# krea-ai/realtime-video

Hardware: AMD Instinct MI355X
Metric: frames/sec at 832x480, 4-step 14B T2V (per-step DiT latency in config) (higher is better)
Workload: dtype bf16

## Files before the change

### include/rtv_hip_cross_fold.h

```cpp
#ifndef RTV_HIP_CROSS_FOLD_H
#define RTV_HIP_CROSS_FOLD_H
#include "rtv_hip.h"

#ifdef __cplusplus
extern "C" {
#endif

int rtv_attn_probs_dup(const void* q, const void* k, void* p, int Lq, int Lkv, int H, int D,
                       int64_t q_row_stride, int64_t k_row_stride, int64_t p_row_stride, int kh, int p_cols,
                       float scale, int dup_key, int dup_count, rtv_stream_t stream);

#define RTV_CROSS_FOLD_KH_MAX 120
int rtv_cross_fold_dims(int num_heads, int text_rows, int* kh, int* k_fold);
int rtv_cross_fold_weight(const void* co_w, int64_t ldw, const void* v, int64_t ldv, void* vo, int64_t ldvo,
                          int num_heads, int rows, int kh, int k_fold, rtv_stream_t stream);

#ifdef __cplusplus
}
#endif
#endif
```

### realtime_video_amd/causal_model.py

```python
import collections
import ctypes
import math
import os
import types

import torch

from . import _lib, lora, ops
from .rope import rope_cos_sin_table

c_vp = ctypes.c_void_p
_IncompatibleKeys = collections.namedtuple("_IncompatibleKeys", ["missing_keys", "unexpected_keys"])


_Cfg = _lib.STRUCTS["rtv_dit_config"]
_LayerW = _lib.STRUCTS["rtv_dit_layer_weights"]
_Weights = _lib.STRUCTS["rtv_dit_weights"]
_Step = _lib.STRUCTS["rtv_dit_step"]
_Fp8Shadow = _lib.ATTN_FP8_STRUCTS["rtv_attn_fp8_shadow"]
_LAYER_FIELDS = tuple(n for n, _ in _LayerW._fields_)
_TOP_FIELDS = tuple(n for n, t in _Weights._fields_ if t is c_vp)

_FP8_TOP = ("text0_w", "text2_w", "time0_w", "time2_w", "tproj_w", "head_w")
_FP8_LAYER = ("qkv_w", "o_w", "cq_w", "ck_w", "cv_w", "co_w", "ffn0_w", "ffn2_w")

PROJ_LN, PROJ_Q, PROJ_KV = 1, 2, 4


def _cross_fold_max_cols(num_heads):
    lib, kh, kf = _lib.load(), ctypes.c_int(0), ctypes.c_int(0)
    rows = 1
    while lib.rtv_cross_fold_dims(int(num_heads), rows + 8, ctypes.byref(kh), ctypes.byref(kf)):
        rows += 8
    lib.rtv_cross_fold_dims(int(num_heads), rows, ctypes.byref(kh), ctypes.byref(kf))
    return kf.value


class BlockCausalMask:

    def __init__(self, num_frames, frame_seqlen, num_frame_per_block, local_attn_size=-1):
        if local_attn_size != -1:
            raise NotImplementedError("local-window block masks are not used by the inference path")
        self.num_frames, self.frame_seqlen = num_frames, frame_seqlen
        self.num_frame_per_block = num_frame_per_block
        self.block_tokens = frame_seqlen * num_frame_per_block

    def __repr__(self):
        return f"BlockCausalMask(frames={self.num_frames}, block_tokens={self.block_tokens})"


class _SelfAttnHandle:

    def __init__(self, local_attn_size, sink_size):
        self.local_attn_size = local_attn_size
        self.sink_size = sink_size
        self.num_frame_per_block = 1
        self.fused_projections = True
        self.max_attention_size = 32760 if local_attn_size == -1 else local_attn_size * 1560

    def fuse_projections(self):
        self.fused_projections = True


def cache_row_map(cache, sink_tokens=None):
    n = int(cache["local_end_index"])
    r = torch.arange(n)
    lo, size, start = (int(cache.get(k, 0)) for k in ("ring_lo", "ring_size", "ring_start"))
    if size > 0:
        r = torch.where(r >= lo, lo + (r - lo + start) % size, r)
    return r


class CausalWanModel:
    def __init__(self, model_type="t2v", patch_size=(1, 2, 2), text_len=512, in_dim=16, dim=2048, ffn_dim=8192,
                 freq_dim=256, text_dim=4096, out_dim=16, num_heads=16, num_layers=32, local_attn_size=-1,
                 sink_size=0, qk_norm=True, cross_attn_norm=True, eps=1e-6, device="cuda"):
        if model_type != "t2v" or tuple(patch_size) != (1, 2, 2) or not qk_norm or not cross_attn_norm:
            raise NotImplementedError("the MI355X hot path implements the t2v causal model (patch 1x2x2, qk_norm, cross_attn_norm)")
        if dim % num_heads or dim // num_heads != 128:
            raise ValueError("head_dim must be 128")
        self.model_type, self.patch_size = model_type, tuple(patch_size)
        self.text_len, self.in_dim, self.dim, self.ffn_dim = text_len, in_dim, dim, ffn_dim
        self.freq_dim, self.text_dim, self.out_dim = freq_dim, text_dim, out_dim
        self.num_heads, self.num_layers, self.eps = num_heads, num_layers, eps
        self.local_attn_size, self.sink_size = local_attn_size, sink_size
        self.device = torch.device(device)
        self.config = types.SimpleNamespace(num_heads=num_heads, dim=dim, num_layers=num_layers, ffn_dim=ffn_dim)
        self.blocks = [types.SimpleNamespace(self_attn=_SelfAttnHandle(local_attn_size, sink_size))
                       for _ in range(num_layers)]
        self.block_mask = None
        self.num_frame_per_block = 1
        self.independent_first_frame = False
        self.gemm_tile_cfg = 0
        self.context_parallel = None
        self._tensors = {}
        self._w = None
        self._ws = {}
        self.fold_text_padding = True
        self.fold_cross_v = os.environ.get("RTV_FOLD_CROSS_V", "1") != "0"
        self.use_hip_graphs = False
        self._graphs = {}
        self._weights_version = 0
        self._cfg = _Cfg(dim, ffn_dim, num_heads, num_layers, freq_dim, text_dim, text_len, in_dim, out_dim, eps, 0, 0)
        self._lora = {}
        self._lora_base = {}
        self._fp8_attn = None
        self._fp8_attn_epoch = 0
        self._fp8_attn_amax = None
        self.lora_version = 0

    def eval(self):
        return self

    def to(self, *args, **kwargs):
        for a in list(args) + list(kwargs.values()):
            if isinstance(a, torch.dtype) and a != torch.bfloat16:
                raise NotImplementedError(f"the MI355X DiT computes in bf16 (asked for {a})")
            if isinstance(a, (str, torch.device, int)) and not isinstance(a, bool):
                dev = torch.device("cuda", a) if isinstance(a, int) else torch.device(a)
                if dev.type != self.device.type or (dev.index is not None and self.device.index is not None
                                                    and dev.index != self.device.index):
                    raise NotImplementedError(f"weights live on {self.device}; construct the model with device={dev!s} instead")
        return self

    def requires_grad_(self, flag=False):
        return self

    def parameters(self):
        return iter(self._tensors.values())

    def state_dict_shapes(self, fused=False):
        d, f = self.dim, self.ffn_dim
        sh = {"patch_embedding.weight": (d, self.in_dim) + self.patch_size, "patch_embedding.bias": (d,),
              "text_embedding.0.weight": (d, self.text_dim), "text_embedding.0.bias": (d,),
              "text_embedding.2.weight": (d, d), "text_embedding.2.bias": (d,),
              "time_embedding.0.weight": (d, self.freq_dim), "time_embedding.0.bias": (d,),
              "time_embedding.2.weight": (d, d), "time_embedding.2.bias": (d,),
              "time_projection.1.weight": (6 * d, d), "time_projection.1.bias": (6 * d,),
              "head.head.weight": (self.out_dim * 4, d), "head.head.bias": (self.out_dim * 4,), "head.modulation": (1, 2, d)}
        for i in range(self.num_layers):
            p = f"blocks.{i}"
            for a in ("self_attn", "cross_attn"):
                for m in ("q", "k", "v", "o"):
                    sh[f"{p}.{a}.{m}.weight"], sh[f"{p}.{a}.{m}.bias"] = (d, d), (d,)
                sh[f"{p}.{a}.norm_q.weight"], sh[f"{p}.{a}.norm_k.weight"] = (d,), (d,)
            if fused:
                sh[f"{p}.self_attn.to_qkv.weight"], sh[f"{p}.self_attn.to_qkv.bias"] = (3 * d, d), (3 * d,)
            sh[f"{p}.norm3.weight"], sh[f"{p}.norm3.bias"] = (d,), (d,)
            sh[f"{p}.ffn.0.weight"], sh[f"{p}.ffn.0.bias"] = (f, d), (f,)
            sh[f"{p}.ffn.2.weight"], sh[f"{p}.ffn.2.bias"] = (d, f), (d,)
            sh[f"{p}.modulation"] = (1, 6, d)
        return sh

    def load_state_dict(self, sd, strict=True, assign=False):
        dev, bf = self.device, torch.bfloat16
        sd = {(k[len("model."):] if k.startswith("model.") else k): v for k, v in sd.items()}
        want = self.state_dict_shapes(fused=True)
        problems, missing, unexpected = [], [], sorted(k for k in sd if k not in want)
        fused_layers = set()
        for i in range(self.num_layers):
            sa = f"blocks.{i}.self_attn"
            if sa + ".to_qkv.weight" in sd and sa + ".to_qkv.bias" in sd:
                fused_layers.add(i)
        for k, shp in want.items():
            layer_fused = ".self_attn." in k and int(k.split(".")[1]) in fused_layers
            is_qkv = ".self_attn." in k and k.split(".")[3] in ("q", "k", "v")
            is_fused_key = ".to_qkv." in k
            if k not in sd:
                if (is_fused_key and not layer_fused) or (is_qkv and layer_fused):
                    continue
                missing.append(k)
            elif tuple(sd[k].shape) != tuple(shp):
                problems.append(f"size mismatch for {k}: copying a param with shape {tuple(sd[k].shape)} from checkpoint, "
                                f"the shape in current model is {tuple(shp)}.")
        if missing:
            problems.insert(0, "Missing key(s) in state_dict: " + ", ".join(repr(k) for k in missing[:12])
                            + (f" ... ({len(missing)} in total)" if len(missing) > 12 else "") + ".")
        if unexpected and strict:
            problems.insert(1 if missing else 0, "Unexpected key(s) in state_dict: " + ", ".join(repr(k) for k in unexpected[:12])
                            + (f" ... ({len(unexpected)} in total)" if len(unexpected) > 12 else "") + ".")
        if problems and (strict or missing or any(p.startswith("size") for p in problems)):
            raise RuntimeError("Error(s) in loading state_dict for CausalWanModel:\n\t" + "\n\t".join(problems))
# ... 340 lines not shown
            rolled = l_end - evicted - sink_tokens
            if ring and rolled <= 0:
                ring_start = 0
            elif ring:
                if ring_size == 0 or ring_start == 0:
                    ring_lo, ring_size = sink_tokens, kv_size - sink_tokens
                elif (ring_lo, ring_size) != (sink_tokens, kv_size - sink_tokens):
                    raise RuntimeError("the attention sink changed under a rotated rolling cache")
                ring_start = (ring_start + evicted) % ring_size
            else:
                shift_copy = (sink_tokens, evicted, rolled)
            local_end = l_end + current_end - g_end - evicted
        else:
            local_end = l_end + current_end - g_end
        if not ring and ring_start:
            raise RuntimeError("this KV cache is rotated (ring_start != 0): reset it before using it under context parallelism")
        local_start = local_end - num_new
        if local_start < 0 or local_end > kv_size:
            raise RuntimeError(f"KV cache window [{local_start}, {local_end}) outside cache of {kv_size} rows")
        lo = max(0, local_end - sa.max_attention_size)
        if ring_start == 0:
            ring_lo = ring_size = 0

        def commit():
            if shift_copy is not None:
                s0, ev, ro = shift_copy
                for c in kv_cache:
                    for n in ("k", "v"):
                        c[n][:, s0:s0 + ro] = c[n][:, s0 + ev:s0 + ev + ro].clone()
            for c in kv_cache:
                c["global_end_index"] = current_end
                c["local_end_index"] = local_end
                c["ring_lo"], c["ring_size"], c["ring_start"] = ring_lo, ring_size, ring_start
        return local_start, lo, local_end, current_start // frame_seqlen, 0, (ring_lo, ring_size, ring_start), commit

    def _forward_inference(self, x, t, context, seq_len=None, clip_fea=None, y=None, kv_cache=None,
                           crossattn_cache=None, current_start=0, cache_start=0, kv_cache_only=False):
        if self._w is None:
            raise RuntimeError("weights not loaded")
        if kv_cache is None or crossattn_cache is None:
            raise NotImplementedError("the hot path is the KV-cached inference forward (causal_model.py:825-954)")
        if clip_fea is not None or y is not None:
            raise NotImplementedError("i2v conditioning is out of scope")
        xs = list(x) if not torch.is_tensor(x) else [x[i] for i in range(x.shape[0])]
        B = len(xs)
        if B != 1:
            raise NotImplementedError("batch size 1 (the streaming server path); run sessions as replicas")
        u = xs[0]
        if not u.is_cuda:
            raise RuntimeError("realtime_video_amd.CausalWanModel needs GPU tensors (no CPU fallback)")
        C, F, Hh, Ww = u.shape
        gh, gw = Hh // 2, Ww // 2
        fs = gh * gw
        M = F * fs
        if seq_len is not None and M > seq_len:
            raise AssertionError("sequence longer than seq_len")
        u = u.to(torch.bfloat16).contiguous()
        tt = t.reshape(-1).to(device=u.device, dtype=torch.float32).contiguous()
        if tt.numel() != F:
            raise ValueError("t must hold one timestep per latent frame")
        need_cross = not all(bool(c["is_init"]) and int(c.get("lora_version", 0)) == self.lora_version for c in crossattn_cache)
        ctx = None
        if need_cross:
            cu = context[0] if not torch.is_tensor(context) else context[0]
            ctx = torch.zeros(self.text_len, self.text_dim, dtype=torch.bfloat16, device=u.device)
            ctx[:cu.shape[0]] = cu.to(torch.bfloat16)
            nz = torch.nonzero(ctx.abs().amax(dim=1) > 0)
            n_real = int(nz[-1]) + 1 if nz.numel() else 0
            for c in crossattn_cache:
                c["text_rows"] = n_real
        cp = self.context_parallel
        use_cp = cp is not None and (cp.world > 1 or getattr(cp, "force_single_rank", False))
        kv_only = bool(kv_cache_only) and not need_cross
        text_rows = int(crossattn_cache[0].get("text_rows", 0)) if getattr(self, "fold_text_padding", True) else 0
        if text_rows <= 0 or any(int(c.get("text_rows", 0)) != text_rows for c in crossattn_cache):
            text_rows = 0
        fold_k = 0
        if 0 < text_rows < self.text_len - 1 and getattr(self, "fold_cross_v", True) and not self._cfg.use_fp8:
            kh_, kf_ = ctypes.c_int(0), ctypes.c_int(0)
            if _lib.load().rtv_cross_fold_dims(self.num_heads, text_rows, ctypes.byref(kh_), ctypes.byref(kf_)):
                fold_k = kf_.value
            if fold_k and not need_cross and any(c.get("vo_for") != (text_rows, self.lora_version) for c in crossattn_cache):
                fold_k = 0
        if fold_k:
            for c in crossattn_cache:
                if "vo" not in c:
                    c["vo"] = torch.zeros(self.dim * _cross_fold_max_cols(self.num_heads), dtype=torch.bfloat16, device=u.device)
        row0, lo, hi, start_frame, causal_block, (ring_lo, ring_size, ring_shift), commit = \
            self._cache_window(kv_cache, M, current_start, fs, ring=not use_cp)
        L = self.num_layers
        rs = kv_cache[0]["k"].stride(1)
        for c in kv_cache:
            for n in ("k", "v"):
                if c[n].stride(3) != 1 or c[n].stride(2) != c[n].shape[3] or c[n].stride(1) != rs:
                    raise ValueError("KV cache tensors must be [B, kv_size, H, 128] views with dense [H, 128] rows "
                                     "and one common row stride")

        fp8_shadow, fp8_keep = self._fp8_attention_shadow(kv_cache, use_cp)
        forward = ("rtv_dit_forward",) if fp8_shadow is None else ("rtv_dit_forward_attn_fp8", ctypes.byref(fp8_shadow))
        fp8_key = (self._fp8_attn[:2] + (kv_cache[0]["k8"].data_ptr(), kv_cache[-1]["v8t"].data_ptr())) if fp8_shadow is not None else None

        def ptr_array(tensors):
            arr = (c_vp * L)(*[t_.data_ptr() for t_ in tensors])
            return arr, ctypes.cast(arr, ctypes.POINTER(c_vp))

        kk_keep, kk = ptr_array([c["k"] for c in kv_cache])
        kv_keep, kv = ptr_array([c["v"] for c in kv_cache])
        ck_keep, ck = ptr_array([c["k"] for c in crossattn_cache])
        cv_list = [c["v"] for c in crossattn_cache] + ([c["vo"] for c in crossattn_cache] if fold_k else [])
        cv_keep = (c_vp * len(cv_list))(*[t_.data_ptr() for t_ in cv_list])
        cv = ctypes.cast(cv_keep, ctypes.POINTER(c_vp))
        out = (torch.zeros if kv_only else torch.empty)((self.out_dim, F, Hh, Ww), dtype=torch.bfloat16, device=u.device)
        stream = c_vp(torch.cuda.current_stream().cuda_stream)
        cfg_p, w_p = ctypes.byref(self._cfg), ctypes.byref(self._w)

        def make(rank_rows, slot, kk=kk, kv=kv):
            ws = self._workspace(F, gh, gw, slot)
            ws_ptr = (ws.data_ptr() + 255) & ~255
            st = _Step(u.data_ptr(), tt.data_ptr(), ctx.data_ptr() if ctx is not None else None, out.data_ptr(),
                       F, gh, gw, kk, kv, rs, ck, cv, int(need_cross), row0, lo, hi,
                       start_frame, causal_block, int(self.gemm_tile_cfg), rank_rows[0], rank_rows[1],
                       ring_lo, ring_size, ring_shift, int(text_rows), int(kv_only),
                       int(getattr(cp, "attn_kv_splits", 1)) if use_cp else 1, fold_k)
            return st, (c_vp(ws_ptr), ctypes.c_size_t(ws.numel() - (ws_ptr - ws.data_ptr())), stream)

        splits = int(getattr(cp, "attn_kv_splits", 1)) if use_cp else 1
        if splits > self._cfg.max_attn_kv_splits:
            self._cfg.max_attn_kv_splits = splits
            self._ws.clear()
            self._graphs.clear()
            self._weights_version += 1
        if self.gemm_tile_cfg in (0, 5):
            ops.ensure_gemm_workspace(u.device)
        if use_cp:
            commit()
        if not use_cp:
            graph_key = None
            if self.use_hip_graphs and not need_cross:
                graph_key = (F, gh, gw, row0, lo, hi, start_frame, causal_block, ring_lo, ring_size, ring_shift, kv_only, text_rows, fold_k,
                             int(self.gemm_tile_cfg), rs, self._weights_version,
                             kv_cache[0]["k"].data_ptr(), kv_cache[-1]["v"].data_ptr(), crossattn_cache[0]["k"].data_ptr(), fp8_key)
                ent = self._graphs.get(graph_key)
                if isinstance(ent, dict):
                    ent["u"].copy_(u)
                    ent["t"].copy_(tt)
                    ent["graph"].replay()
                    commit()
                    return ent["out"].clone().unsqueeze(0)
            if graph_key is not None and self._graphs.get(graph_key) == "seen":
                ent = {"u": u.clone(), "t": tt.clone(), "out": out, "keep": (kk_keep, kv_keep, ck_keep, cv_keep, fp8_keep)}
                u, tt = ent["u"], ent["t"]
                g = torch.cuda.CUDAGraph()
                if not hasattr(self, "_capture_stream"):
                    self._capture_stream = torch.cuda.Stream(device=u.device)
                ops.ensure_gemm_workspace(u.device, self._capture_stream.cuda_stream)
                with torch.cuda.graph(g, stream=self._capture_stream):
                    stream = c_vp(torch.cuda.current_stream().cuda_stream)
                    st, wsa = make((0, 0), 0)
                    _lib.call(forward[0], cfg_p, w_p, ctypes.byref(st), *forward[1:], *wsa)
                ent["graph"], ent["step"] = g, st
                self._graphs[graph_key] = ent
                g.replay()
                commit()
                return out.clone().unsqueeze(0)
            if graph_key is not None:
                self._graphs[graph_key] = "seen"
            st, wsa = make((0, 0), 0)
            _lib.call(forward[0], cfg_p, w_p, ctypes.byref(st), *forward[1:], *wsa)
            commit()
        else:
            graph_key = None
            if self.use_hip_graphs and not need_cross and not getattr(cp, "_gloo", False):
                graph_key = ("cp", id(cp), bool(getattr(cp, "overlap", True)), cp.world, cp.head_exchange(self.num_heads), F, gh, gw, row0, lo, hi, start_frame, causal_block, kv_only,
                             text_rows, fold_k, int(self.gemm_tile_cfg), rs, self._weights_version, splits,
                             kv_cache[0]["k"].data_ptr(), kv_cache[-1]["v"].data_ptr(), crossattn_cache[0]["k"].data_ptr())
                ent = self._graphs.get(graph_key)
                if isinstance(ent, dict):
                    ent["u"].copy_(u)
                    ent["t"].copy_(tt)
                    ent["graph"].replay()
                    return ent["out"].clone().unsqueeze(0)

            def run_cp():
                self.cp_forwards_issued = getattr(self, "cp_forwards_issued", 0) + 1
                from .parallel import shard_rows, wait_in_order
                W, H = cp.world, self.num_heads
                heads = cp.head_exchange(H)
                keep = []
                if heads:
                    hn = H // W
                    if kv_cache[0]["k"].shape[2] not in (hn, H):
                        raise ValueError(f"KV cache must hold {hn} (this rank's) or {H} heads, not {kv_cache[0]['k'].shape[2]}")
                    parts = []
                    for i, r in enumerate(cp.local_ranks()):
                        h0 = 0 if kv_cache[0]["k"].shape[2] == hn else r * hn
                        ka, kp = ptr_array([c["k"][0, :, h0:h0 + hn] for c in kv_cache])
                        va, vp = ptr_array([c["v"][0, :, h0:h0 + hn] for c in kv_cache])
                        keep.append((ka, va))
                        parts.append(make(shard_rows(M, W, r), i, kp, vp))
                    bufs = [(r, self._exchange_buffers(M, W, i, u.device)) for i, r in enumerate(cp.local_ranks())]
                else:
                    parts = [make(shard_rows(M, W, r), i) for i, r in enumerate(cp.local_ranks())]
                for st, wsa in parts:
                    _lib.call("rtv_dit_begin", cfg_p, w_p, ctypes.byref(st), *wsa)
                null = c_vp(0)
                for l in range(L):
                    last_kv_only = kv_only and l == L - 1
                    if not heads:
                        for st, wsa in parts:
                            _lib.call("rtv_dit_layer_proj", cfg_p, w_p, ctypes.byref(st), l, PROJ_LN | PROJ_KV, 0, null, null, *wsa)
                        pend = cp.gather_kv(kv_cache[l]["k"][0], kv_cache[l]["v"][0], row0, M, async_op=True)
                        if last_kv_only:
                            pend.wait()
                            break
                        for st, wsa in parts:
                            _lib.call("rtv_dit_layer_proj", cfg_p, w_p, ctypes.byref(st), l, PROJ_Q, 0, null, null, *wsa)
                        pend.wait()
                        for st, wsa in parts:
                            _lib.call("rtv_dit_layer_rest", cfg_p, w_p, ctypes.byref(st), l, *wsa)
                        continue
                    if last_kv_only:
                        for (st, wsa), (_, b) in zip(parts, bufs):
                            _lib.call("rtv_dit_layer_proj", cfg_p, w_p, ctypes.byref(st), l, PROJ_LN | PROJ_KV, W, null,
                                      c_vp(b["kv_send"].data_ptr()), *wsa)
                        cp.exchange_kv(bufs, kv_cache[l]["k"][0], kv_cache[l]["v"][0], row0, M)
                        break
                    for (st, wsa), (_, b) in zip(parts, bufs):
                        _lib.call("rtv_dit_layer_proj", cfg_p, w_p, ctypes.byref(st), l, PROJ_LN | PROJ_Q, W,
                                  c_vp(b["q_send"].data_ptr()), null, *wsa)
                    pend_q = cp.exchange_q(bufs, async_op=True)
                    for (st, wsa), (_, b) in zip(parts, bufs):
                        _lib.call("rtv_dit_layer_proj", cfg_p, w_p, ctypes.byref(st), l, PROJ_KV, W, null,
                                  c_vp(b["kv_send"].data_ptr()), *wsa)
                    pend_kv = cp.exchange_kv(bufs, kv_cache[l]["k"][0], kv_cache[l]["v"][0], row0, M, async_op=True)
                    wait_in_order(pend_q, pend_kv)
                    for (st, wsa), (_, b) in zip(parts, bufs):
                        _lib.call("rtv_dit_layer_attn_hp", cfg_p, w_p, ctypes.byref(st), l, W, c_vp(b["q_all"].data_ptr()),
                                  c_vp(b["o_all"].data_ptr()), *wsa)
                    cp.exchange_o(bufs)
                    for (st, wsa), (_, b) in zip(parts, bufs):
                        _lib.call("rtv_dit_layer_rest_hp", cfg_p, w_p, ctypes.byref(st), l, W, c_vp(b["o_recv"].data_ptr()), *wsa)
                if not kv_only:
                    hrow = torch.empty((M, self.out_dim * 4), dtype=torch.bfloat16, device=u.device)
                    for st, wsa in parts:
                        _lib.call("rtv_dit_head", cfg_p, w_p, ctypes.byref(st), c_vp(hrow.data_ptr()), *wsa)
                    cp.all_gather_rows_(hrow, kind="head_rows")
                    _lib.call("rtv_dit_finish", cfg_p, ctypes.byref(parts[0][0]), c_vp(hrow.data_ptr()), stream)

            if graph_key is not None and self._graphs.get(graph_key) == "seen":
                ent = {"u": u.clone(), "t": tt.clone(), "out": out, "keep": (kk_keep, kv_keep, ck_keep, cv_keep)}
                u, tt = ent["u"], ent["t"]
                g = torch.cuda.CUDAGraph()
                if not hasattr(self, "_capture_stream"):
                    self._capture_stream = torch.cuda.Stream(device=u.device)
                ops.ensure_gemm_workspace(u.device, self._capture_stream.cuda_stream)
                with torch.cuda.graph(g, stream=self._capture_stream, capture_error_mode="thread_local"):
                    stream = c_vp(torch.cuda.current_stream().cuda_stream)
# ... 20 lines not shown
```

### realtime_video_amd/csrc/attn_fwd.hip

```cpp
#include "attn_common.h"

namespace rtv {

#ifdef RTV_ATTN_TRACE
__device__ unsigned* g_attn_trace = nullptr;
#define ATT_STAMP(i)                                                                    \
  do {                                                                                  \
    if (tr_on && j >= 20 && j < 24) {                                                   \
      __builtin_amdgcn_sched_barrier(0);                                                \
      const unsigned t_ = (unsigned)__builtin_readcyclecounter();                       \
      if (lane == 0) tr_dst[(j - 20) * 6 + (i)] = t_;                                   \
      __builtin_amdgcn_sched_barrier(0);                                                \
    }                                                                                   \
  } while (0)
#else
#define ATT_STAMP(i)
#endif

template <bool F16>
__global__ __launch_bounds__(256) void attn_combine_kernel(const float* __restrict__ part_o, const float* __restrict__ part_ml,
                                                           uint16_t* __restrict__ o, int S, int B, int H, int Lq, int64_t o_bs,
                                                           int64_t o_rs) {
  const int64_t nrows = (int64_t)B * H * Lq;
  const int64_t row = (int64_t)blockIdx.x * 16 + (threadIdx.x >> 4);
// ... 510 lines not shown
          int kv = j * ATT_KT + kbk * 32 + (r & 3) + 8 * (r >> 2) + 4 * g;
          if (kv >= kv_lim) sacc[kbk][r] = -INFINITY;
        }
    }
    {
      float mx = sacc[0][0];
#pragma unroll
      for (int r = 1; r < 16; ++r) mx = fmaxf(mx, sacc[0][r]);
#pragma unroll
      for (int r = 0; r < 16; ++r) mx = fmaxf(mx, sacc[1][r]);
      mx = xor32_max(mx);
      const float m_cand = fmaxf(m_run, mx * c);
      const bool need = m_cand - m_run > RESCALE_SLACK;
      if (__builtin_amdgcn_ballot_w64(need) != 0) {
        const float m_new = need ? m_cand : m_run;
        const float alpha = __builtin_amdgcn_exp2f(m_run - m_new);
        m_run = m_new;
        l_run *= alpha;
#pragma unroll
        for (int db = 0; db < 4; ++db)
#pragma unroll
          for (int r = 0; r < 16; ++r) oacc[db][r] *= alpha;
      }
      static_for<0, 4>([&](auto ic) { exp_step(IntC<0>{}, ic); });
    }
    asm volatile("" : "+v"(pf[0][0]), "+v"(ps2));
    asm volatile("s_waitcnt vmcnt(4)" ::: "memory");
    ATT_STAMP8(5);
    PP_BARRIER();
    ATT_STAMP8(6);
    lds_wait_frags(frag);
    static_for<0, 16>([&](auto ic) {
      constexpr int i = decltype(ic)::value, kbk = i >> 3, s_ = (i >> 2) & 1, db = i & 3;
      oacc[db] = mfma32<F16>(frag[(kbk * 2 + s_) * 4 + db], pf[kbk][s_], oacc[db]);
      if constexpr (i < 12) {
        constexpr int f = i + 4;
        exp_step(IntC<(f >> 3)>{}, IntC<(f & 7)>{});
      }
      __builtin_amdgcn_sched_barrier(0);
    });
    l_run += ps2[0] + ps2[1];
    ps2 = f32x2{0.f, 0.f};
    asm volatile("" : "+v"(l_run));
    ATT_STAMP8(7);
    PP_BARRIER();
  }
  if (!grp) PP_BARRIER();
#undef PP_BARRIER

#ifdef RTV_ATTN_TRACE
  if (tr_on && lane < 32 && ntiles >= 24) tr_dst[lane] = tr_lds[lane];
#endif
  const float l_tot = l_run + __shfl_xor(l_run, 32, 64);
  if (p.kv_splits > 1) {
    store_partial(p, bh, q_row, g, oacc, m_run, l_tot);
    return;
  }
  const float inv = 1.0f / l_tot;
  if (q_row < p.Lq) {
    uint16_t* op = ob + (size_t)q_row * p.o_rs + 4 * g;
#pragma unroll
    for (int db = 0; db < 4; ++db)
#pragma unroll
      for (int i = 0; i < 4; ++i) {
        u32x2 w;
        w[0] = pack2<F16>(oacc[db][4 * i + 0] * inv, oacc[db][4 * i + 1] * inv);
        w[1] = pack2<F16>(oacc[db][4 * i + 2] * inv, oacc[db][4 * i + 3] * inv);
        *(u32x2*)(op + db * 32 + i * 8) = w;
      }
  }
}

struct ProbsParams {
  const uint16_t* q;
  const uint16_t* k;
  uint16_t* p;
  int Lq, Lkv, H;
  int64_t q_rs, k_rs, p_rs;
  int kh, p_cols;
  float scale_log2e;
  int dup_key;
  float dup_log2;
  int tiles_per_wg;
};
constexpr int PROBS_NW = 4;
constexpr int PROBS_ROWS = PROBS_NW * ATT_QW;

template <int NKB>
__global__ __launch_bounds__(PROBS_NW * 64) void attn_probs_kernel(ProbsParams p) {
  constexpr int KEYS = NKB * 32;
  constexpr int SLAB_LD = KEYS * 2 + 16;
  extern __shared__ __attribute__((aligned(16))) char smem[];
  char* const sK = smem;
  const int tid = threadIdx.x;
  const int lane = tid & 63;
  const int wave = __builtin_amdgcn_readfirstlane(tid >> 6);
  const int l31 = lane & 31, g = lane >> 5;
  char* const slab = smem + KEYS * 256 + wave * (ATT_QW * SLAB_LD);
  const int h = blockIdx.y;
  const uint16_t* qb = p.q + (size_t)h * ATT_D;
  const uint16_t* kb = p.k + (size_t)h * ATT_D;
  uint16_t* pb = p.p + (size_t)h * p.kh;

  for (int id = tid; id < KEYS * 16; id += PROBS_NW * 64) {
    const int r = id >> 4, c = id & 15;
    u32x4 v = {0u, 0u, 0u, 0u};
    if (r < p.Lkv) v = *(const u32x4*)(kb + (int64_t)r * p.k_rs + c * 8);
    *(u32x4*)(sK + r * 256 + ((c ^ (r & 15)) << 4)) = v;
  }
  __syncthreads();
  const char* k_rd[8];
#pragma unroll
  for (int dc = 0; dc < 8; ++dc) k_rd[dc] = sK + l31 * 256 + (((dc * 2 + g) ^ (l31 & 15)) << 4);

  const float c = p.scale_log2e;
  const int ppr = p.kh >> 3;
  const int tail0 = p.H * p.kh, tail_pieces = h == p.H - 1 ? (p.p_cols - tail0) >> 3 : 0;
  const int tile0 = blockIdx.x * p.tiles_per_wg;
  for (int ti = 0; ti < p.tiles_per_wg; ++ti) {
    const int row0 = (tile0 + ti) * PROBS_ROWS + wave * ATT_QW;
    if (row0 >= p.Lq) break;
    const int q_row_c = min(row0 + l31, p.Lq - 1);
    u32x4 qf[8];
    {
      const uint16_t* qp = qb + (size_t)q_row_c * p.q_rs + g * 8;
#pragma unroll
      for (int dc = 0; dc < 8; ++dc) qf[dc] = *(const u32x4*)(qp + dc * 16);
    }
    f32x16 s[NKB];
#pragma unroll
    for (int kbk = 0; kbk < NKB; ++kbk)
#pragma unroll
      for (int r = 0; r < 16; ++r) s[kbk][r] = 0.f;
#pragma unroll
    for (int dc = 0; dc < 8; ++dc)
#pragma unroll
      for (int kbk = 0; kbk < NKB; ++kbk) {
        const u32x4 kf = *(const u32x4*)(k_rd[dc] + kbk * 32 * 256);
        s[kbk] = mfma32<false>(kf, qf[dc], s[kbk]);
      }
    float mx = -INFINITY;
#pragma unroll
    for (int kbk = 0; kbk < NKB; ++kbk)
#pragma unroll
      for (int r = 0; r < 16; ++r) {
        const int key = kbk * 32 + (r & 3) + 8 * (r >> 2) + 4 * g;
        float x = s[kbk][r] * c;
        if (key == p.dup_key) x += p.dup_log2;
        if (key >= p.Lkv) x = -INFINITY;
        s[kbk][r] = x;
        mx = fmaxf(mx, x);
      }
    mx = fmaxf(mx, __shfl_xor(mx, 32, 64));
    float l = 0.f;
#pragma unroll
    for (int kbk = 0; kbk < NKB; ++kbk)
#pragma unroll
      for (int r = 0; r < 16; ++r) {
        const float e = __builtin_amdgcn_exp2f(s[kbk][r] - mx);
        s[kbk][r] = e;
        l += e;
      }
    l += __shfl_xor(l, 32, 64);
    const float inv = 1.0f / l;
#pragma unroll
    for (int kbk = 0; kbk < NKB; ++kbk)
#pragma unroll
      for (int i = 0; i < 4; ++i) {
        u32x2 w;
        w[0] = pack2<false>(s[kbk][4 * i + 0] * inv, s[kbk][4 * i + 1] * inv);
        w[1] = pack2<false>(s[kbk][4 * i + 2] * inv, s[kbk][4 * i + 3] * inv);
        *(u32x2*)(slab + l31 * SLAB_LD + (kbk * 32 + 8 * i + 4 * g) * 2) = w;
      }
    __builtin_amdgcn_fence(__ATOMIC_RELEASE, "workgroup");
    __builtin_amdgcn_wave_barrier();
    const int rows_here = min(ATT_QW, p.Lq - row0);
    for (int id = lane; id < rows_here * ppr; id += 64) {
      const int r = id / ppr, pc = id - r * ppr;
      const u32x4 v = *(const u32x4*)(slab + r * SLAB_LD + pc * 16);
      *(u32x4*)(pb + (int64_t)(row0 + r) * p.p_rs + pc * 8) = v;
    }
    for (int id = lane; id < rows_here * tail_pieces; id += 64) {
      const int r = id / tail_pieces, pc = id - r * tail_pieces;
      *(u32x4*)(p.p + (int64_t)(row0 + r) * p.p_rs + tail0 + pc * 8) = u32x4{0u, 0u, 0u, 0u};
    }
    __builtin_amdgcn_fence(__ATOMIC_ACQUIRE, "workgroup");
    __builtin_amdgcn_wave_barrier();
  }
}

}

using namespace rtv;

#ifdef RTV_ATTN_TRACE
extern "C" int rtv_attn_debug_trace(unsigned* buf) {
  return hipMemcpyToSymbol(HIP_SYMBOL(rtv::g_attn_trace), &buf, sizeof(buf)) == hipSuccess ? 0 : -1;
}
#endif

static std::atomic<int> g_attn_waves{0};
static std::atomic<bool> g_attn_lockstep{false};
static std::atomic<bool> g_attn_force_pp{false};
static std::atomic<bool> g_attn_skip_idle{true};
static std::atomic<int> g_attn_w4{-2};
constexpr int W4_DEFAULT = 600;
namespace rtv {
int launch_attn_w4(const AttnParams& p, bool f16, int variant, dim3 grid, hipStream_t stream);
}

extern "C" int rtv_attn_set_skip_idle(int on) {
  g_attn_skip_idle = on != 0;
  return 0;
}

extern "C" int rtv_attn_set_waves(int waves) {
  if (waves != 0 && waves != 4 && waves != 8 && waves != 81 && waves != 82 && !(waves >= 840 && waves <= 1639))
    return set_error(-1, "attn_set_waves: 0 (auto), 4, 8, 81 (256 rows, lockstep schedule), 82 (256 rows, four-phase schedule) or "
                         "840 + v (256 rows, one wave per SIMD, kernel variant v: attn_w4.hip)");
  g_attn_lockstep = waves == 81;
  g_attn_force_pp = waves == 82;
  g_attn_w4 = waves >= 840 ? waves - 840 : (waves == 81 || waves == 82 ? -1 : -2);
  g_attn_waves = waves > 8 ? 8 : waves;
  return 0;
}

extern "C" int rtv_attn_fwd(const void* q, const void* k, const void* v, void* o, int B, int Lq, int Lkv,
                            int H, int D, int64_t q_batch_stride, int64_t q_row_stride,
                            int64_t k_batch_stride, int64_t k_row_stride, int64_t v_batch_stride,
                            int64_t v_row_stride, int64_t o_batch_stride, int64_t o_row_stride, float scale,
                            int causal_block, int q_offset, int dtype, rtv_stream_t stream) {
  return rtv_attn_fwd_win(q, k, v, o, B, Lq, Lkv, 0, 0, H, D, q_batch_stride, q_row_stride, k_batch_stride, k_row_stride,
                          v_batch_stride, v_row_stride, o_batch_stride, o_row_stride, scale, causal_block, q_offset, dtype,
                          stream);
}

static int attn_fwd_impl(const void* q, const void* k, const void* v, void* o, int B, int Lq, int Lkv0, int Lkv1,
                         int seg1_row, int H, int D, int64_t q_batch_stride, int64_t q_row_stride,
                         int64_t k_batch_stride, int64_t k_row_stride, int64_t v_batch_stride,
                         int64_t v_row_stride, int64_t o_batch_stride, int64_t o_row_stride, float scale,
                         int causal_block, int q_offset, int dtype, rtv_stream_t stream, int dup_key, int dup_count,
                         int kv_splits = 1, void* split_ws = nullptr, size_t split_ws_bytes = 0);

extern "C" int rtv_attn_fwd_win(const void* q, const void* k, const void* v, void* o, int B, int Lq, int Lkv0, int Lkv1,
                                int seg1_row, int H, int D, int64_t q_batch_stride, int64_t q_row_stride,
                                int64_t k_batch_stride, int64_t k_row_stride, int64_t v_batch_stride,
                                int64_t v_row_stride, int64_t o_batch_stride, int64_t o_row_stride, float scale,
                                int causal_block, int q_offset, int dtype, rtv_stream_t stream) {
  return attn_fwd_impl(q, k, v, o, B, Lq, Lkv0, Lkv1, seg1_row, H, D, q_batch_stride, q_row_stride, k_batch_stride, k_row_stride,
                       v_batch_stride, v_row_stride, o_batch_stride, o_row_stride, scale, causal_block, q_offset, dtype, stream,
                       -1, 0);
}

extern "C" int rtv_attn_fwd_dup(const void* q, const void* k, const void* v, void* o, int B, int Lq, int Lkv, int H, int D,
                                int64_t q_batch_stride, int64_t q_row_stride, int64_t k_batch_stride, int64_t k_row_stride,
                                int64_t v_batch_stride, int64_t v_row_stride, int64_t o_batch_stride, int64_t o_row_stride,
                                float scale, int dup_key, int dup_count, int dtype, rtv_stream_t stream) {
  if (dup_key < 0 || dup_key >= Lkv || dup_count < 1) return set_error(-1, "attn_fwd_dup: dup_key must be a key of the window, dup_count >= 1");
  return attn_fwd_impl(q, k, v, o, B, Lq, Lkv, 0, 0, H, D, q_batch_stride, q_row_stride, k_batch_stride, k_row_stride,
                       v_batch_stride, v_row_stride, o_batch_stride, o_row_stride, scale, 0, 0, dtype, stream,
                       dup_count > 1 ? dup_key : -1, dup_count);
}

template <int NKB>
static int launch_attn_probs(const ProbsParams& p, dim3 grid, hipStream_t stream) {
  static LdsAttr lds_attr;
  const int lds = NKB * 32 * 256 + PROBS_NW * ATT_QW * (NKB * 64 + 16);
  if (int st = ensure_dynamic_lds((const void*)attn_probs_kernel<NKB>, lds, &lds_attr, "attn_probs")) return st;
  hipLaunchKernelGGL((attn_probs_kernel<NKB>), grid, dim3(PROBS_NW * 64), lds, stream, p);
  return check_launch("attn_probs");
}

extern "C" int rtv_attn_probs_dup(const void* q, const void* k, void* p, int Lq, int Lkv, int H, int D, int64_t q_row_stride,
                                  int64_t k_row_stride, int64_t p_row_stride, int kh, int p_cols, float scale, int dup_key,
                                  int dup_count, rtv_stream_t stream) {
  if (D != ATT_D) return set_error(-1, "attn_probs: head_dim must be 128");
  if (H <= 0 || Lq <= 0) return 0;
  if (Lkv <= 0 || Lkv > 128) return set_error(-1, "attn_probs: the key window must hold 1..128 keys");
  if (kh <= 0 || (kh & 7) || kh < Lkv || kh > 128) return set_error(-1, "attn_probs: kh must be a multiple of 8 in [Lkv, 128]");
  if ((p_cols & 7) || (int64_t)H * kh > p_cols || p_cols > p_row_stride)
    return set_error(-1, "attn_probs: need H * kh <= p_cols <= p_row_stride, p_cols a multiple of 8");
  if ((q_row_stride | k_row_stride | p_row_stride) & 7 || q_row_stride < (int64_t)H * ATT_D || k_row_stride < (int64_t)H * ATT_D)
    return set_error(-1, "attn_probs: strides must be multiples of 8 elements (16-byte rows) and hold H heads");
  if (((uintptr_t)q | (uintptr_t)k | (uintptr_t)p) & 15) return set_error(-1, "attn_probs: base pointers must be 16-byte aligned");
  if (dup_key < 0 || dup_key >= Lkv || dup_count < 1) return set_error(-1, "attn_probs: dup_key must be a key of the window, dup_count >= 1");
  ProbsParams pp;
  pp.q = (const uint16_t*)q;
  pp.k = (const uint16_t*)k;
  pp.p = (uint16_t*)p;
  pp.Lq = Lq;
  pp.Lkv = Lkv;
  pp.H = H;
  pp.q_rs = q_row_stride;
  pp.k_rs = k_row_stride;
  pp.p_rs = p_row_stride;
  pp.kh = kh;
  pp.p_cols = p_cols;
  pp.scale_log2e = scale * 1.4426950408889634f;
  pp.dup_key = dup_count > 1 ? dup_key : -1;
  pp.dup_log2 = dup_count > 1 ? log2f((float)dup_count) : 0.f;
  const int cus = device_num_cus() > 0 ? device_num_cus() : 256;
  const int n_tiles = (Lq + PROBS_ROWS - 1) / PROBS_ROWS;
  int tpw = (int)(((int64_t)n_tiles * H) / (2 * (int64_t)cus));
  tpw = tpw < 1 ? 1 : (tpw > 8 ? 8 : tpw);
  pp.tiles_per_wg = tpw;
  const dim3 grid((n_tiles + tpw - 1) / tpw, H);
  ProfScope prof(PROF_ATTN, (hipStream_t)stream, 2.0 * H * (double)Lq * Lkv * ATT_D);
  note_kernel(DK_ATTN_PROBS);
  const int nkb = (kh + 31) / 32;
  switch (nkb) {
    case 1: return launch_attn_probs<1>(pp, grid, (hipStream_t)stream);
    case 2: return launch_attn_probs<2>(pp, grid, (hipStream_t)stream);
    case 3: return launch_attn_probs<3>(pp, grid, (hipStream_t)stream);
    default: return launch_attn_probs<4>(pp, grid, (hipStream_t)stream);
  }
}

extern "C" size_t rtv_attn_split_workspace_bytes(int B, int Lq, int H, int kv_splits) {
  if (B <= 0 || Lq <= 0 || H <= 0 || kv_splits < 2) return 0;
  return (size_t)kv_splits * B * H * Lq * (ATT_D + 2) * sizeof(float);
}

extern "C" int rtv_attn_fwd_split(const void* q, const void* k, const void* v, void* o, int B, int Lq, int Lkv0, int Lkv1,
                                  int seg1_row, int H, int D, int64_t q_batch_stride, int64_t q_row_stride,
                                  int64_t k_batch_stride, int64_t k_row_stride, int64_t v_batch_stride,
                                  int64_t v_row_stride, int64_t o_batch_stride, int64_t o_row_stride, float scale,
                                  int causal_block, int q_offset, int kv_splits, void* workspace, size_t workspace_bytes,
                                  int dtype, rtv_stream_t stream) {
  if (kv_splits < 1 || kv_splits > 16) return set_error(-1, "attn_fwd_split: kv_splits must be 1..16");
  return attn_fwd_impl(q, k, v, o, B, Lq, Lkv0, Lkv1, seg1_row, H, D, q_batch_stride, q_row_stride, k_batch_stride, k_row_stride,
                       v_batch_stride, v_row_stride, o_batch_stride, o_row_stride, scale, causal_block, q_offset, dtype, stream, -1,
                       0, kv_splits, workspace, workspace_bytes);
}

static int attn_fwd_impl(const void* q, const void* k, const void* v, void* o, int B, int Lq, int Lkv0, int Lkv1,
                         int seg1_row, int H, int D, int64_t q_batch_stride, int64_t q_row_stride,
                         int64_t k_batch_stride, int64_t k_row_stride, int64_t v_batch_stride,
                         int64_t v_row_stride, int64_t o_batch_stride, int64_t o_row_stride, float scale,
                         int causal_block, int q_offset, int dtype, rtv_stream_t stream, int dup_key, int dup_count,
                         int kv_splits, void* split_ws, size_t split_ws_bytes) {
  if (Lkv0 < 0 || Lkv1 < 0) return set_error(-1, "attn_fwd: negative segment length");
  if (Lkv1 > 0 && causal_block > 0) return set_error(-1, "attn_fwd: the block-causal mask needs a one-segment window");
  const int Lkv = Lkv0 + Lkv1;
  if (D != ATT_D) return set_error(-1, "attn_fwd: head_dim must be 128");
  if (B <= 0 || H <= 0 || Lq <= 0) return 0;
  if (Lkv <= 0) return set_error(-1, "attn_fwd: Lkv must be positive");
  if ((q_row_stride | k_row_stride | v_row_stride | o_row_stride | q_batch_stride | k_batch_stride |
       v_batch_stride | o_batch_stride) & 7)
    return set_error(-1, "attn_fwd: strides must be multiples of 8 elements (16-byte rows)");
  if (((uintptr_t)q | (uintptr_t)k | (uintptr_t)v | (uintptr_t)o) & 15)
    return set_error(-1, "attn_fwd: base pointers must be 16-byte aligned");
  if (causal_block < 0 || q_offset < 0) return set_error(-1, "attn_fwd: negative mask parameters");
  if (dtype != RTV_DTYPE_BF16 && dtype != RTV_DTYPE_F16) return set_error(-1, "attn_fwd: dtype");
  AttnParams p;
  p.q = (const uint16_t*)q;
  p.k = (const uint16_t*)k;
  p.v = (const uint16_t*)v;
  p.o = (uint16_t*)o;
  p.B = B;
  p.Lq = Lq;
  p.Lkv = Lkv;
  p.H = H;
  p.q_bs = q_batch_stride;
  p.q_rs = q_row_stride;
  p.k_bs = k_batch_stride;
  p.k_rs = k_row_stride;
  p.v_bs = v_batch_stride;
  p.v_rs = v_row_stride;
  p.o_bs = o_batch_stride;
  p.o_rs = o_row_stride;
  p.scale_log2e = scale * 1.4426950408889634f;
  p.dup_key = dup_key;
  p.dup_bias = dup_key >= 0 ? log2f((float)dup_count) / p.scale_log2e : 0.f;
  if (kv_splits > (Lkv + ATT_KT - 1) / ATT_KT) kv_splits = (Lkv + ATT_KT - 1) / ATT_KT;
  if (kv_splits < 1) kv_splits = 1;
  p.kv_splits = kv_splits;
  p.part_o = nullptr;
  p.part_ml = nullptr;
  if (kv_splits > 1) {
    if (dup_key >= 0) return set_error(-1, "attn_fwd: no KV split of a window with a counted key");
    const size_t rows = (size_t)kv_splits * B * H * Lq;
    if (!split_ws || ((uintptr_t)split_ws & 15) || split_ws_bytes < rows * (ATT_D + 2) * sizeof(float))
      return set_error(-1, "attn_fwd: split workspace missing, misaligned or too small (rtv_attn_split_workspace_bytes)");
    p.part_o = (float*)split_ws;
    p.part_ml = p.part_o + rows * ATT_D;
  }
  p.causal_block = causal_block;
  p.q_offset = q_offset;
  p.n0 = Lkv1 > 0 ? Lkv0 : Lkv;
  p.delta = Lkv1 > 0 ? seg1_row - Lkv0 : 0;
  int waves = g_attn_waves;
  const int cus = device_num_cus() > 0 ? device_num_cus() : 256;
  if (waves == 0) waves = ((int64_t)B * H * ((Lq + 255) / 256) * kv_splits < (int64_t)cus * 5 / 8 || Lkv <= 512) ? 4 : 8;
  const int qt_rows = ATT_QW * waves;
  p.n_qtiles = (Lq + qt_rows - 1) / qt_rows;
  const int lds = 4 * ATT_TILE_BYTES;
  const bool f16 = dtype == RTV_DTYPE_F16;
  const void* kerns[4] = {(const void*)attn_fwd_kernel<false, 8>, (const void*)attn_fwd_kernel<true, 8>,
// ... 75 lines not shown
```

### realtime_video_amd/csrc/dit_forward.hip

```cpp
#include <atomic>

#include "../../include/rtv_hip_attn_fp8.h"
#include "rtv_common.h"
#include "rtv_internal.h"

namespace rtv {

__global__ void silu_kernel(const bf16_t* __restrict__ x, bf16_t* __restrict__ out, int64_t n) {
  for (int64_t i = (int64_t)blockIdx.x * blockDim.x + threadIdx.x; i < n; i += (int64_t)gridDim.x * blockDim.x)
    out[i] = f32_to_bf16(silu(bf16_to_f32(x[i])));
}

constexpr int FOLD_ROWS = 64, FOLD_LD = 130;
__global__ __launch_bounds__(256) void cross_fold_weight_kernel(const bf16_t* __restrict__ w, int64_t ldw, const bf16_t* __restrict__ v,
                                                               int64_t ldv, bf16_t* __restrict__ vo, int64_t ldvo, int H, int rows, int kh,
                                                               int k_fold) {
  __shared__ __attribute__((aligned(16))) bf16_t sW[FOLD_ROWS * FOLD_LD];
  __shared__ __attribute__((aligned(16))) bf16_t sV[128 * FOLD_LD];
  const int tid = threadIdx.x, lane = tid & 63, wave = tid >> 6;
  const int n0 = blockIdx.x * FOLD_ROWS, h = blockIdx.y;
  for (int id = tid; id < FOLD_ROWS * 64; id += 256) {
    const int r = id >> 6, c = (id & 63) * 2;
    *(uint32_t*)(sW + r * FOLD_LD + c) = *(const uint32_t*)(w + (int64_t)(n0 + r) * ldw + h * 128 + c);
  }
  for (int id = tid; id < rows * 64; id += 256) {
    const int r = id >> 6, c = (id & 63) * 2;
    *(uint32_t*)(sV + r * FOLD_LD + c) = *(const uint32_t*)(v + (int64_t)r * ldv + h * 128 + c);
  }
  __syncthreads();
  for (int ts = 0; ts < kh; ts += 64) {
    const int t = ts + lane;
    float acc[16];
#pragma unroll
    for (int i = 0; i < 16; ++i) acc[i] = 0.f;
    if (t < rows) {
      const bf16_t* vr = sV + t * FOLD_LD;
      const bf16_t* wr = sW + wave * 16 * FOLD_LD;
      for (int dd = 0; dd < 128; dd += 2) {
        const uint32_t v2 = *(const uint32_t*)(vr + dd);
        const float v0 = __uint_as_float(v2 << 16), v1 = __uint_as_float(v2 & 0xffff0000u);
#pragma unroll
        for (int i = 0; i < 16; ++i) {
          const uint32_t w2 = *(const uint32_t*)(wr + i * FOLD_LD + dd);
          acc[i] = fmaf(__uint_as_float(w2 << 16), v0, acc[i]);
          acc[i] = fmaf(__uint_as_float(w2 & 0xffff0000u), v1, acc[i]);
        }
      }
    }
    if (t < kh) {
#pragma unroll
      for (int i = 0; i < 16; ++i) vo[(int64_t)(n0 + wave * 16 + i) * ldvo + h * kh + t] = f32_to_bf16(acc[i]);
    }
  }
  if (h == H - 1) {
    const int tail0 = H * kh;
    for (int t = tail0 + lane; t < k_fold; t += 64)
#pragma unroll
      for (int i = 0; i < 16; ++i) vo[(int64_t)(n0 + wave * 16 + i) * ldvo + t] = 0;
  }
}

struct Workspace {
  char* base;
  size_t off, cap;
  bool ok;
  void* take(size_t bytes) {
    size_t a = (off + 255) & ~(size_t)255;
    if (base && a + bytes > cap) ok = false;
    off = a + bytes;
    return base ? base + a : nullptr;
  }
};

struct DitBuffers {
  uint16_t *x, *xn, *qkv, *q, *ao, *h, *prow, *hrow;
  uint16_t *sinus, *te1, *e, *se, *e0, *emod, *ehead, *ctx1, *ctx, *ktmp;
  uint8_t* q8;
  float* frow;
  float* fscale;
  float* attn_part;
  size_t attn_part_bytes;
};

static size_t carve(const rtv_dit_config* c, int F, int gh, int gw, char* base, size_t cap, DitBuffers* b,
                    bool* ok) {
  Workspace ws{base, 0, cap, true};
  const size_t M = (size_t)F * gh * gw, d = c->dim, e = 2;
  DitBuffers t;
  t.x = (uint16_t*)ws.take(M * d * e);
  t.xn = (uint16_t*)ws.take(M * d * e);
  t.qkv = (uint16_t*)ws.take(M * 3 * d * e);
  t.q = (uint16_t*)ws.take(M * d * e);
  t.ao = (uint16_t*)ws.take(M * d * e);
  t.h = (uint16_t*)ws.take(M * (size_t)c->ffn_dim * e);
  t.prow = (uint16_t*)ws.take(M * (size_t)c->in_dim * 4 * e);
  t.hrow = (uint16_t*)ws.take(M * (size_t)c->out_dim * 4 * e);
  t.sinus = (uint16_t*)ws.take((size_t)F * c->freq_dim * e);
  t.te1 = (uint16_t*)ws.take((size_t)F * d * e);
  t.e = (uint16_t*)ws.take((size_t)F * d * e);
  t.se = (uint16_t*)ws.take((size_t)F * d * e);
  t.e0 = (uint16_t*)ws.take((size_t)F * 6 * d * e);
  t.emod = (uint16_t*)ws.take((size_t)c->num_layers * F * 6 * d * e);
  t.ehead = (uint16_t*)ws.take((size_t)F * 2 * d * e);
  t.ctx1 = (uint16_t*)ws.take((size_t)c->text_len * d * e);
  t.ctx = (uint16_t*)ws.take((size_t)c->text_len * d * e);
  t.ktmp = (uint16_t*)ws.take((size_t)c->text_len * d * e);
  {
    size_t rows = M > (size_t)c->text_len ? M : (size_t)c->text_len, k = d;
    if ((size_t)c->ffn_dim > k) k = c->ffn_dim;
    if ((size_t)c->text_dim > k) k = c->text_dim;
    if ((size_t)c->freq_dim > k) k = c->freq_dim;
    t.q8 = (uint8_t*)ws.take(c->use_fp8 ? rows * k : 0);
    t.frow = (float*)ws.take(c->use_fp8 == 2 ? rows * sizeof(float) : 0);
    t.fscale = (float*)ws.take(256);
  }
  t.attn_part_bytes = c->max_attn_kv_splits > 1 ? M * (size_t)c->num_heads * (128 + 2) * sizeof(float) : 0;
  t.attn_part = (float*)ws.take(t.attn_part_bytes);
  if (b) *b = t;
  if (ok) *ok = ws.ok;
  return ws.off;
}

struct Ctx {
  const rtv_dit_config* cfg;
  const rtv_dit_weights* w;
  const rtv_dit_step* st;
  DitBuffers b;
  rtv_stream_t stream;
  int d, H, L, ffn, hd, F, gh, gw, fs, M, r0, rc, tc;
  const rtv_attn_fp8_shadow* fp8;
  int fold_kh, fold_k;
};

static int make_ctx(const rtv_dit_config* cfg, const rtv_dit_weights* w, const rtv_dit_step* st, void* workspace,
                    size_t workspace_bytes, rtv_stream_t stream, Ctx* c) {
  if (!cfg || !w || !st || !workspace) return set_error(-1, "dit: null argument");
  c->cfg = cfg;
  c->w = w;
  c->st = st;
  c->fp8 = nullptr;
  c->stream = stream;
  c->d = cfg->dim;
  c->H = cfg->num_heads;
  c->L = cfg->num_layers;
  c->ffn = cfg->ffn_dim;
  if (c->H <= 0 || c->d % c->H || c->d / c->H != 128) return set_error(-1, "dit: head_dim must be 128");
  c->hd = 128;
  c->F = st->F;
  c->gh = st->gh;
  c->gw = st->gw;
  c->fs = st->gh * st->gw;
  c->M = st->F * c->fs;
  if (c->M <= 0) return set_error(-1, "dit: empty token grid");
  c->r0 = st->row_begin;
  c->rc = st->row_count > 0 ? st->row_count : c->M - st->row_begin;
  if (c->r0 < 0 || c->rc <= 0 || c->r0 + c->rc > c->M) return set_error(-1, "dit: local row range outside the token grid");
  if (st->kv_lo < 0 || st->kv_hi <= st->kv_lo) return set_error(-1, "dit: empty attention window");
  if (st->cache_row0 < 0 || st->cache_row0 + c->M > st->kv_hi)
    return set_error(-1, "dit: the rows written by this call must lie inside the attention window");
  if (st->ring_size < 0 || st->ring_lo < 0 || st->ring_shift < 0 || (st->ring_size > 0 && st->ring_shift >= st->ring_size) ||
      (st->ring_size > 0 && st->kv_hi > st->ring_lo + st->ring_size))
    return set_error(-1, "dit: bad ring window (0 <= ring_shift < ring_size, kv_hi <= ring_lo + ring_size)");
  if (st->ring_size > 0 && st->ring_shift > 0 && st->causal_block > 0)
    return set_error(-1, "dit: the block-causal recompute pass writes an unrotated cache (ring_shift must be 0)");
  if (((uintptr_t)workspace) & 255) return set_error(-1, "dit: workspace must be 256-byte aligned");
  bool ok = true;
  carve(cfg, c->F, c->gh, c->gw, (char*)workspace, workspace_bytes, &c->b, &ok);
  if (!ok) return set_error(-1, "dit: workspace too small (see rtv_dit_workspace_bytes)");
  c->tc = st->gemm_tile_cfg;
  c->fold_kh = c->fold_k = 0;
  if (st->ca_vo_ld > 0 && st->ca_v && !cfg->use_fp8 && st->text_rows > 0 && st->text_rows + 1 < cfg->text_len) {
    int kh = 0, kf = 0;
    if (rtv_cross_fold_dims(c->H, st->text_rows, &kh, &kf) && kf <= c->d) {
      if (st->ca_vo_ld < kf || (st->ca_vo_ld & 7)) return set_error(-1, "dit: ca_vo_ld must be a multiple of 8 and >= k_fold (rtv_cross_fold_dims)");
      c->fold_kh = kh;
      c->fold_k = kf;
    }
  }
  return 0;
}

}

using namespace rtv;

#define RTV_TRY(expr)        \
  do {                       \
    int _s = (expr);         \
    if (_s != 0) return _s;  \
  } while (0)

extern "C" int rtv_silu(const void* x, void* out, int64_t n, rtv_stream_t stream) {
  if (n <= 0) return 0;
  int blocks = (int)((n + 255) / 256);
  if (blocks > 2048) blocks = 2048;
  hipLaunchKernelGGL(silu_kernel, dim3(blocks), dim3(256), 0, (hipStream_t)stream, (const bf16_t*)x,
                     (bf16_t*)out, n);
  return check_launch("silu");
}

extern "C" int rtv_cross_fold_dims(int num_heads, int text_rows, int* kh, int* k_fold) {
  const int khv = text_rows >= 0 ? (text_rows + 1 + 7) & ~7 : 0;
  const int64_t kf = ((int64_t)num_heads * khv + 63) & ~(int64_t)63;
  if (kh) *kh = khv;
  if (k_fold) *k_fold = kf > 0x7fffffff ? 0 : (int)kf;
  return num_heads > 0 && text_rows > 0 && khv <= RTV_CROSS_FOLD_KH_MAX && kf <= 0x7fffffff;
}

extern "C" int rtv_cross_fold_weight(const void* co_w, int64_t ldw, const void* v, int64_t ldv, void* vo, int64_t ldvo, int num_heads,
                                     int rows, int kh, int k_fold, rtv_stream_t stream) {
  if (!co_w || !v || !vo) return set_error(-1, "cross_fold_weight: null argument");
  if (num_heads <= 0 || rows <= 0 || rows > kh || kh > 128 || (kh & 7)) return set_error(-1, "cross_fold_weight: need 0 < rows <= kh <= 128, kh % 8 == 0");
  const int64_t d = (int64_t)num_heads * 128;
  if ((int64_t)num_heads * kh > k_fold || k_fold > ldvo || ldw < d || ldv < d || ((ldw | ldv) & 1))
    return set_error(-1, "cross_fold_weight: need num_heads * kh <= k_fold <= ldvo and rows of num_heads * 128 elements");
  if (((uintptr_t)co_w | (uintptr_t)v) & 3) return set_error(-1, "cross_fold_weight: operands must be 4-byte aligned");
  ProfScope prof(PROF_MISC, (hipStream_t)stream, 2.0 * d * (double)num_heads * rows * 128);
  hipLaunchKernelGGL(cross_fold_weight_kernel, dim3((unsigned)(d / FOLD_ROWS), num_heads), dim3(256), 0, (hipStream_t)stream,
                     (const bf16_t*)co_w, ldw, (const bf16_t*)v, ldv, (bf16_t*)vo, ldvo, num_heads, rows, kh, k_fold);
  return check_launch("cross_fold_weight");
}

extern "C" size_t rtv_dit_workspace_bytes(const rtv_dit_config* cfg, int F, int gh, int gw) {
  if (!cfg || F <= 0 || gh <= 0 || gw <= 0) return 0;
  return carve(cfg, F, gh, gw, nullptr, 0, nullptr, nullptr) + 256;
}

enum { S_TEXT0 = 0, S_TEXT2, S_TIME0, S_TIME2, S_TPROJ, S_HEAD, S_LAYER0 };
enum { S_QKV = 0, S_O, S_CQ, S_CK, S_CV, S_CO, S_FFN0, S_FFN2, S_PER_LAYER };
static bool is_fp8(const Ctx& c, int sidx) { return c.cfg->use_fp8 && sidx >= 0; }

static int quantize_input(Ctx& c, int sidx, const void* a, int M, int K, rtv_stream_t s) {
  if (!is_fp8(c, sidx)) return 0;
  if (c.cfg->use_fp8 == 2) {
    if (!c.w->fp8_row_scales || !c.w->fp8_row_scales[sidx]) return set_error(-1, "dit: use_fp8 == 2 needs rtv_dit_weights.fp8_row_scales");
    return a ? rtv_quantize_fp8_rows(a, K, M, K, c.b.q8, K, c.b.frow, s) : 0;
  }
  if (!c.w->fp8_scales) return set_error(-1, "dit: use_fp8 needs rtv_dit_weights.fp8_scales");
  return rtv_quantize_fp8(a, K, M, K, c.b.q8, K, c.b.fscale, c.b.fscale + 1, s) ? -1 : 0;
}

static int project(Ctx& c, int sidx, const void* a, int K, const void* w, int w_row0, const void* bias, void* out, int ldc, int M, int N,
                   int act, const void* gate, int gate_stride, int rpf, int row_off, const void* res, int cfg, rtv_stream_t s) {
  const bool fp8 = is_fp8(c, sidx);
  const void* wp = (const char*)w + (size_t)w_row0 * K * (fp8 ? 1 : 2);
  const void* bp = bias ? (const uint16_t*)bias + w_row0 : nullptr;
  const int ldr = res ? ldc : 0;
  if (!fp8) return rtv_gemm(a, K, wp, K, out, ldc, M, N, K, bp, act, gate, gate_stride, rpf, row_off, res, ldr, RTV_DTYPE_BF16, cfg, s);
  if (c.cfg->use_fp8 == 2)
    return rtv_gemm_fp8_rows(c.b.q8, K, wp, K, c.b.frow, (const float*)c.w->fp8_row_scales[sidx] + w_row0, out, ldc, M, N, K, bp, act, gate,
                             gate_stride, rpf, row_off, res, ldr, s);
  return rtv_gemm_fp8(c.b.q8, K, wp, K, c.b.fscale, c.w->fp8_scales[sidx], out, ldc, M, N, K, bp, act, gate, gate_stride, rpf, row_off, res,
                      ldr, s);
}

static int linear(Ctx& c, int sidx, const void* a, int K, const void* w, const void* bias, void* out, int M, int N, int act,
                  const void* gate, int gate_stride, int rpf, int row_off, const void* res, int cfg, rtv_stream_t s) {
  RTV_TRY(quantize_input(c, sidx, a, M, K, s));
  return project(c, sidx, a, K, w, 0, bias, out, N, M, N, act, gate, gate_stride, rpf, row_off, res, cfg, s);
}

static int ln_input(Ctx& c, const void* shift, const void* scale, int frame_stride, const void* weight, const void* bias, const void** a) {
  DitBuffers& b = c.b;
  const int rpf = scale ? c.fs : 0, r0 = scale ? c.r0 : 0;
  if (c.cfg->use_fp8 == 2) {
    *a = nullptr;
    return rtv_layernorm_modulate_fp8_rows(b.x, b.q8, c.d, b.frow, c.rc, c.d, c.cfg->eps, shift, scale, frame_stride, rpf, r0, weight, bias,
                                           c.stream);
  }
  *a = b.xn;
  return rtv_layernorm_modulate(b.x, b.xn, c.rc, c.d, c.cfg->eps, shift, scale, frame_stride, rpf, r0, weight, bias, c.stream);
}

static int dit_begin(Ctx& c) {
  const rtv_dit_config* cfg = c.cfg;
  const rtv_dit_weights* w = c.w;
  const rtv_dit_step* st = c.st;
  DitBuffers& b = c.b;
  const int d = c.d, F = c.F, L = c.L, tc = c.tc;
  rtv_stream_t stream = c.stream;
  const int pk = cfg->in_dim * 4;
  RTV_TRY(rtv_patchify(st->x, b.prow, cfg->in_dim, F, c.gh, c.gw, stream));
  RTV_TRY(linear(c, -1, b.prow + (size_t)c.r0 * pk, pk, w->patch_w, w->patch_b, b.x, c.rc, d, 0, nullptr, 0, 0, 0, nullptr, tc, stream));
// ... 137 lines not shown

struct KeyWindow {
  int row0, n0, row1, n1;
};
static KeyWindow key_window(const rtv_dit_step* st) {
  const int lo = st->kv_lo, hi = st->kv_hi, S = st->ring_lo, R = st->ring_size;
  if (R <= 0 || hi <= S) return KeyWindow{lo, hi - lo, 0, 0};
  const int rl = lo > S ? lo : S;
  const int n = hi - rl;
  const int p0 = S + (rl - S + st->ring_shift) % R;
  const int first = (p0 + n <= S + R) ? n : S + R - p0;
  const int sink = lo < S ? S - lo : 0;
  if (first == n) {
    if (sink == 0) return KeyWindow{p0, n, 0, 0};
    if (p0 == S) return KeyWindow{lo, sink + n, 0, 0};
    return KeyWindow{lo, sink, p0, n};
  }
  return KeyWindow{sink ? lo : S, sink + n - first, p0, first};
}

static int sharded_self_attn(Ctx& c, const void* q, const void* k, const void* v, void* o, int rows, int n0, int n1, int seg1_row,
                             int heads, int64_t q_rs, int64_t kv_rs, int64_t o_rs, int q_offset) {
  const rtv_dit_step* st = c.st;
  const float scale = 1.0f / sqrtf((float)c.hd);
  const int S = st->attn_kv_splits;
  const int qo = st->causal_block > 0 ? q_offset : 0;
  if (S > 1 && (S > c.cfg->max_attn_kv_splits || rtv_attn_split_workspace_bytes(1, rows, heads, S) > c.b.attn_part_bytes))
    return set_error(-1, "dit: attn_kv_splits exceeds rtv_dit_config.max_attn_kv_splits / the partials do not fit the workspace "
                         "(splits <= number of shards)");
  if (S > 1)
    return rtv_attn_fwd_split(q, k, v, o, 1, rows, n0, n1, seg1_row, heads, c.hd, 0, q_rs, 0, kv_rs, 0, kv_rs, 0, o_rs, scale,
                              st->causal_block, qo, S, c.b.attn_part, c.b.attn_part_bytes, RTV_DTYPE_BF16, c.stream);
  return rtv_attn_fwd_win(q, k, v, o, 1, rows, n0, n1, seg1_row, heads, c.hd, 0, q_rs, 0, kv_rs, 0, kv_rs, 0, o_rs, scale,
                          st->causal_block, qo, RTV_DTYPE_BF16, c.stream);
}

static int dit_layer_rest(Ctx& c, int l) {
  const rtv_dit_step* st = c.st;
  DitBuffers& b = c.b;
  const int d = c.d, H = c.H, hd = c.hd, rc = c.rc, r0 = c.r0;
  rtv_stream_t stream = c.stream;
  const float scale = 1.0f / sqrtf((float)hd);
  const int64_t rs = st->kv_row_stride;
  const int Lkv = st->kv_hi - st->kv_lo;
  const int q_offset = st->cache_row0 - st->kv_lo + r0;
  uint16_t* kc = (uint16_t*)st->kv_k[l];
  uint16_t* vc = (uint16_t*)st->kv_v[l];
  KeyWindow kw = key_window(st);
  if (c.fp8) {
    const rtv_attn_fp8_shadow* sh = c.fp8;
    RTV_TRY(rtv_attn_fwd_fp8(b.q, sh->k8[l], sh->v8t[l], b.ao, rc, H, sh->cache_rows, kw.row0, kw.n0, kw.row1, kw.n1, d, d, scale,
                             sh->k_scale, sh->v_scale, st->causal_block, st->causal_block > 0 ? q_offset : 0, stream));
  } else if (rc < c.M) {
    RTV_TRY(sharded_self_attn(c, b.q, kc + (size_t)kw.row0 * rs, vc + (size_t)kw.row0 * rs, b.ao, rc, kw.n0, kw.n1,
                              kw.row1 - kw.row0, H, d, rs, d, q_offset));
  } else {
    RTV_TRY(rtv_attn_fwd_win(b.q, kc + (size_t)kw.row0 * rs, vc + (size_t)kw.row0 * rs, b.ao, 1, rc, kw.n0, kw.n1,
                             kw.row1 - kw.row0, H, hd, 0, d, 0, rs, 0, rs, 0, d, scale, st->causal_block,
                             st->causal_block > 0 ? q_offset : 0, RTV_DTYPE_BF16, stream));
  }
  (void)Lkv;
  if (void* qd = g_capture_q.load(std::memory_order_relaxed)) {
    void* od = g_capture_o.load(std::memory_order_relaxed);
    const size_t bytes = (size_t)rc * d * sizeof(uint16_t);
    if (hipMemcpyAsync(qd, b.q, bytes, hipMemcpyDeviceToDevice, (hipStream_t)stream) != hipSuccess ||
        (od && hipMemcpyAsync(od, b.ao, bytes, hipMemcpyDeviceToDevice, (hipStream_t)stream) != hipSuccess))
      return set_error(-1, "dit: self-attention capture copy failed");
  }
  return dit_after_attn(c, l);
}

static int dit_after_attn(Ctx& c, int l) {
  const rtv_dit_layer_weights& lw = c.w->layers[l];
  const rtv_dit_step* st = c.st;
  DitBuffers& b = c.b;
  const int d = c.d, H = c.H, hd = c.hd, fs = c.fs, tc = c.tc, rc = c.rc, r0 = c.r0;
  rtv_stream_t stream = c.stream;
  const float eps = c.cfg->eps;
  const uint16_t* em = b.emod + (size_t)l * c.F * 6 * d;
  const float scale = 1.0f / sqrtf((float)hd);
  RTV_TRY(linear(c, S_LAYER0 + S_PER_LAYER * l + S_O, b.ao, d, lw.o_w, lw.o_b, b.x, rc, d, 0, em + 2 * d, 6 * d, fs, r0, b.x, tc, stream));
  const void* ln_out = nullptr;
  RTV_TRY(ln_input(c, nullptr, nullptr, 0, lw.norm3_w, lw.norm3_b, &ln_out));
  RTV_TRY(linear(c, S_LAYER0 + S_PER_LAYER * l + S_CQ, ln_out, d, lw.cq_w, lw.cq_b, b.qkv, rc, d, 0, nullptr, 0, 0, 0, nullptr, tc, stream));
  RTV_TRY(rtv_rmsnorm(b.qkv, d, b.q, d, rc, d, eps, lw.cnorm_q_w, stream));
  if (c.fold_k) {
    RTV_TRY(rtv_attn_probs_dup(b.q, st->ca_k[l], b.ao, rc, st->text_rows + 1, H, hd, d, d, c.fold_k, c.fold_kh, c.fold_k, scale,
                               st->text_rows, c.cfg->text_len - st->text_rows, stream));
    RTV_TRY(rtv_gemm(b.ao, c.fold_k, st->ca_v[c.L + l], st->ca_vo_ld, b.x, d, rc, d, c.fold_k, lw.co_b, 0, nullptr, 0, 0, 0, b.x, d,
                     RTV_DTYPE_BF16, tc, stream));
  } else {
    if (st->text_rows > 0 && st->text_rows + 1 < c.cfg->text_len)
      RTV_TRY(rtv_attn_fwd_dup(b.q, st->ca_k[l], st->ca_v[l], b.ao, 1, rc, st->text_rows + 1, H, hd, 0, d, 0, d, 0, d, 0, d, scale,
                               st->text_rows, c.cfg->text_len - st->text_rows, RTV_DTYPE_BF16, stream));
    else
      RTV_TRY(rtv_attn_fwd(b.q, st->ca_k[l], st->ca_v[l], b.ao, 1, rc, c.cfg->text_len, H, hd, 0, d, 0, d, 0, d, 0, d,
                           scale, 0, 0, RTV_DTYPE_BF16, stream));
    RTV_TRY(linear(c, S_LAYER0 + S_PER_LAYER * l + S_CO, b.ao, d, lw.co_w, lw.co_b, b.x, rc, d, 0, nullptr, 0, 0, 0, b.x, tc, stream));
  }
  RTV_TRY(ln_input(c, em + 3 * d, em + 4 * d, 6 * d, nullptr, nullptr, &ln_out));
  RTV_TRY(linear(c, S_LAYER0 + S_PER_LAYER * l + S_FFN0, ln_out, d, lw.ffn0_w, lw.ffn0_b, b.h, rc, c.ffn, RTV_ACT_GELU_TANH, nullptr, 0, 0, 0, nullptr, tc, stream));
  RTV_TRY(linear(c, S_LAYER0 + S_PER_LAYER * l + S_FFN2, b.h, c.ffn, lw.ffn2_w, lw.ffn2_b, b.x, rc, d, 0, em + 5 * d, 6 * d, fs, r0, b.x, tc, stream));
  return 0;
}

static int hp_check(Ctx& c, int world) {
  if (world < 1 || c.H % world) return set_error(-1, "dit: head-parallel exchange needs num_heads % world == 0");
  if (c.M % world || c.rc != c.M / world || c.r0 % c.rc)
    return set_error(-1, "dit: head-parallel exchange needs equal token shards (M % world == 0)");
  return 0;
}

static int dit_layer_qkv_hp(Ctx& c, int l, int world, void* q_send, void* kv_send) {
  return dit_layer_proj(c, l, RTV_PROJ_LN | RTV_PROJ_Q | RTV_PROJ_KV, world, q_send, kv_send);
}

static int dit_layer_attn_hp(Ctx& c, int l, int world, const void* q_all, void* o_all) {
  RTV_TRY(hp_check(c, world));
  const rtv_dit_step* st = c.st;
  const int gc = c.d / world, hn = c.H / world;
  const int64_t rs = st->kv_row_stride;
  const int Lkv = st->kv_hi - st->kv_lo;
  const int q_offset = st->cache_row0 - st->kv_lo;
  const uint16_t* kc = (const uint16_t*)st->kv_k[l];
  const uint16_t* vc = (const uint16_t*)st->kv_v[l];
  KeyWindow kw = key_window(st);
  (void)Lkv;
  return sharded_self_attn(c, q_all, kc + (size_t)kw.row0 * rs, vc + (size_t)kw.row0 * rs, o_all, c.M, kw.n0, kw.n1,
                           kw.row1 - kw.row0, hn, gc, rs, gc, q_offset);
}

static int dit_layer_rest_hp(Ctx& c, int l, int world, const void* o_recv) {
  RTV_TRY(hp_check(c, world));
  RTV_TRY(regroup_heads(o_recv, c.b.ao, c.rc, world, c.d / world, c.stream));
  return dit_after_attn(c, l);
}

static int dit_head(Ctx& c, void* head_rows) {
  DitBuffers& b = c.b;
  const int d = c.d, n = c.cfg->out_dim * 4;
  RTV_TRY(rtv_layernorm_modulate(b.x, b.xn, c.rc, d, c.cfg->eps, b.ehead + 0 * d, b.ehead + 1 * d, 2 * d, c.fs, c.r0, nullptr, nullptr, c.stream));
  RTV_TRY(linear(c, S_HEAD, b.xn, d, c.w->head_w, c.w->head_b, (uint16_t*)head_rows + (size_t)c.r0 * n, c.rc, n, 0, nullptr, 0, 0, 0, nullptr, c.tc, c.stream));
  return 0;
}

extern "C" int rtv_dit_begin(const rtv_dit_config* cfg, const rtv_dit_weights* w, const rtv_dit_step* st, void* ws,
                             size_t ws_bytes, rtv_stream_t stream) {
  Ctx c;
  RTV_TRY(make_ctx(cfg, w, st, ws, ws_bytes, stream, &c));
  return dit_begin(c);
}

extern "C" int rtv_dit_layer_qkv(const rtv_dit_config* cfg, const rtv_dit_weights* w, const rtv_dit_step* st, int layer,
                                 void* ws, size_t ws_bytes, rtv_stream_t stream) {
  Ctx c;
  RTV_TRY(make_ctx(cfg, w, st, ws, ws_bytes, stream, &c));
  if (layer < 0 || layer >= c.L) return set_error(-1, "dit: layer out of range");
  return dit_layer_qkv(c, layer);
}

extern "C" int rtv_dit_layer_proj(const rtv_dit_config* cfg, const rtv_dit_weights* w, const rtv_dit_step* st, int layer,
                                  int parts, int world, void* q_send, void* kv_send, void* ws, size_t ws_bytes,
                                  rtv_stream_t stream) {
  Ctx c;
  RTV_TRY(make_ctx(cfg, w, st, ws, ws_bytes, stream, &c));
  if (layer < 0 || layer >= c.L) return set_error(-1, "dit: layer out of range");
  return dit_layer_proj(c, layer, parts, world, q_send, kv_send);
}

extern "C" int rtv_dit_layer_rest(const rtv_dit_config* cfg, const rtv_dit_weights* w, const rtv_dit_step* st, int layer,
                                  void* ws, size_t ws_bytes, rtv_stream_t stream) {
// ... 95 lines not shown
```

### realtime_video_amd/csrc/elementwise.hip

```cpp
#include "ln_row.h"
#include "rtv_common.h"
#include "rtv_internal.h"

namespace rtv {

static std::atomic<int> g_rope_wave{-1};
constexpr int ROPE_WAVE_MIN_ROWS = 2048;

__global__ __launch_bounds__(EW_THREADS) void layernorm_modulate_kernel(
    const bf16_t* __restrict__ x, bf16_t* __restrict__ out, int d, float eps,
    const bf16_t* __restrict__ shift, const bf16_t* __restrict__ scale, int frame_stride,
    int rows_per_frame, int row_offset, const bf16_t* __restrict__ weight, const bf16_t* __restrict__ bias) {
  __shared__ float red[8];
  bf16_t* orow = out + (size_t)blockIdx.x * d;
  layernorm_row(x, d, eps, shift, scale, frame_stride, rows_per_frame, row_offset, weight, bias, red,
                [&](int, int c, const float* o) { *(u32x4*)(orow + c * 8) = pack_bf16x8(o); });
}

__global__ __launch_bounds__(EW_THREADS) void rmsnorm_kernel(const bf16_t* __restrict__ x, int ldx,
                                                             bf16_t* __restrict__ out, int ldo, int d,
                                                             float eps,
                                                             const bf16_t* __restrict__ weight) {
  __shared__ float red[8];
  const int row = blockIdx.x;
  const int nchunks = d >> 3;
  const bf16_t* xr = x + (size_t)row * ldx;
  float v[EW_MAXC][8];
  float s = 0.f;
#pragma unroll
  for (int i = 0; i < EW_MAXC; ++i) {
    int c = threadIdx.x + i * EW_THREADS;
    if (c < nchunks) {
      unpack_bf16x8(*(const u32x4*)(xr + c * 8), v[i]);
#pragma unroll
      for (int j = 0; j < 8; ++j) s += v[i][j] * v[i][j];
    }
  }
  const float r = rsqrtf(block_sum(s, red) / (float)d + eps);
  bf16_t* orow = out + (size_t)row * ldo;
#pragma unroll
  for (int i = 0; i < EW_MAXC; ++i) {
    int c = threadIdx.x + i * EW_THREADS;
    if (c < nchunks) {
      float w8[8], o[8];
      unpack_bf16x8(*(const u32x4*)(weight + c * 8), w8);
#pragma unroll
      for (int j = 0; j < 8; ++j) o[j] = round_bf16(v[i][j] * r) * w8[j];
      *(u32x4*)(orow + c * 8) = pack_bf16x8(o);
    }
  }
}

__device__ __forceinline__ void launder(u32x4& v) {
  uint32_t a = v[0], b = v[1], c = v[2], e = v[3];
  asm volatile("" : "+v"(a), "+v"(b), "+v"(c), "+v"(e));
  v[0] = a;
  v[1] = b;
  v[2] = c;
  v[3] = e;
}

constexpr int ROWS_PER_WG = 4;

struct RopeArgs {
  const bf16_t* qkv;
  bf16_t* q_out;
  bf16_t* k_cache;
  bf16_t* v_cache;
  int64_t cache_row_stride;
  int cache_row0;
  int M, d, hd;
  float eps;
  const bf16_t* wq;
  const bf16_t* wk;
  const float2* rope_cs;
  int gh, gw, start_frame, row_offset;
  int group_cols;
  int64_t q_group_stride, kv_group_stride;
  int ring_lo, ring_size, ring_shift;
  int parts;
};

__device__ __forceinline__ void rope8(float* x, const float2* w) {
#pragma unroll
  for (int t = 0; t < 4; ++t) {
    const float a = x[2 * t], b = x[2 * t + 1];
    x[2 * t] = a * w[t].x - b * w[t].y;
    x[2 * t + 1] = a * w[t].y + b * w[t].x;
  }
}

template <int CPL, bool LANE_CS>
__global__ __launch_bounds__(EW_THREADS) __attribute__((amdgpu_waves_per_eu(CPL <= 10 ? 5 : 3, 8))) void qk_norm_rope_cache_kernel(RopeArgs a) {
  const int lane = threadIdx.x & 63;
  const bool do_q = a.parts & 1, do_kv = a.parts & 2;
  const int nroles = do_kv ? 2 : 1;
  const int wid = __builtin_amdgcn_readfirstlane(blockIdx.x * ROWS_PER_WG + (threadIdx.x >> 6));
  const int row = wid / nroles, role = wid - row * nroles;
  if (row >= a.M) return;
  const int d = a.d;
  const int nchunks = d >> 3;
  const bf16_t* qr = a.qkv + (size_t)row * 3 * d;
  const bf16_t* vr = qr + 2 * d;
  const bool norm = role == 1 || do_q;
  const bf16_t* xr = role == 1 ? qr + d : qr;
  const bf16_t* wx = role == 1 ? a.wk : a.wq;

  const int half = a.hd >> 1;
  const int c1 = half / 3, c0 = half - 2 * c1;
  const int per_frame = a.gh * a.gw;
  const int grow = a.row_offset + row;
  const int f = grow / per_frame;
  const int rem = grow - f * per_frame;
  const int pos_h = rem / a.gw, pos_w = rem - pos_h * a.gw;
  const int pos_f = a.start_frame + f;
  auto load_cs = [&](int col, float2* w) {
    const int pj0 = (col % a.hd) >> 1;
#pragma unroll
    for (int t = 0; t < 4; ++t) {
      const int pj = pj0 + t;
      const int pos = pj < c0 ? pos_f : (pj < c0 + c1 ? pos_h : pos_w);
      w[t] = a.rope_cs[pos * half + pj];
    }
  };
  float2 cs[4];
  if (LANE_CS && norm) load_cs(lane * 8, cs);

  const int gc = a.group_cols;
  size_t kv_row = gc ? (size_t)row : (size_t)(a.cache_row0 + grow);
  if (!gc && a.ring_size > 0 && (int)kv_row >= a.ring_lo)
    kv_row = (size_t)(a.ring_lo + ((int)kv_row - a.ring_lo + a.ring_shift) % a.ring_size);
  bf16_t* xo = role == 1 ? a.k_cache + kv_row * a.cache_row_stride : a.q_out + (size_t)row * (gc ? gc : d);
  const int64_t x_group_stride = role == 1 ? a.kv_group_stride : a.q_group_stride;
// ... 316 lines not shown
    const size_t r = t / G;
    out[i] = in[((size_t)g * rows + r) * gc8 + c];
  }
}

__global__ void pixels_to_rgb8_kernel(const float* __restrict__ px, uint8_t* __restrict__ out, int T, size_t hw) {
  const size_t quads = hw >> 2;
  const size_t total = (size_t)T * quads;
  for (size_t i = (size_t)blockIdx.x * blockDim.x + threadIdx.x; i < total; i += (size_t)gridDim.x * blockDim.x) {
    const size_t t = i / quads, q = i - t * quads;
    const float* base = px + t * 3 * hw + q * 4;
    float4 c[3];
#pragma unroll
    for (int ch = 0; ch < 3; ++ch) c[ch] = *(const float4*)(base + ch * hw);
    uint8_t b[12];
#pragma unroll
    for (int ch = 0; ch < 3; ++ch) {
      const float v[4] = {c[ch].x, c[ch].y, c[ch].z, c[ch].w};
#pragma unroll
      for (int k = 0; k < 4; ++k) {
        float y = __fmul_rn(__fadd_rn(v[k], 1.0f), 0.5f);
        y = fminf(fmaxf(y, 0.0f), 1.0f);
        b[k * 3 + ch] = (uint8_t)(int)__fmul_rn(y, 255.0f);
      }
    }
    uint32_t* o = (uint32_t*)(out + (t * hw + q * 4) * 3);
#pragma unroll
    for (int w = 0; w < 3; ++w)
      o[w] = (uint32_t)b[4 * w] | ((uint32_t)b[4 * w + 1] << 8) | ((uint32_t)b[4 * w + 2] << 16) | ((uint32_t)b[4 * w + 3] << 24);
  }
}

int regroup_heads(const void* in, void* out, int rows, int G, int group_cols, rtv_stream_t stream) {
  if (rows <= 0) return 0;
  if (group_cols % 8) return set_error(-1, "regroup_heads: group_cols % 8 != 0");
  const size_t total = (size_t)rows * G * (group_cols / 8);
  int blocks = (int)((total + 255) / 256);
  if (blocks > 4096) blocks = 4096;
  ProfScope prof(PROF_MISC, (hipStream_t)stream, 2.0 * rows * G * group_cols * 2);
  hipLaunchKernelGGL(regroup_heads_kernel, dim3(blocks), dim3(256), 0, (hipStream_t)stream, (const u32x4*)in, (u32x4*)out,
                     rows, G, group_cols / 8);
  return check_launch("regroup_heads");
}
}

using namespace rtv;

extern "C" {

int rtv_rope_set_wave(int mode) {
  g_rope_wave.store(mode < 0 ? -1 : (mode ? 1 : 0), std::memory_order_relaxed);
  return 0;
}


int rtv_layernorm_modulate(const void* x, void* out, int M, int d, float eps, const void* shift,
                           const void* scale, int frame_stride, int rows_per_frame, int row_offset,
                           const void* weight, const void* bias, rtv_stream_t stream) {
  if (M <= 0) return 0;
  if (d % 8 || d > EW_THREADS * 8 * EW_MAXC) return set_error(-1, "layernorm_modulate: d must be a multiple of 8 and <= 8192");
  if ((shift == nullptr) != (scale == nullptr)) return set_error(-1, "layernorm_modulate: shift and scale go together");
  if ((weight == nullptr) != (bias == nullptr)) return set_error(-1, "layernorm_modulate: weight and bias go together");
  if (weight && scale) return set_error(-1, "layernorm_modulate: affine and modulation are exclusive");
  if (scale && (rows_per_frame <= 0 || frame_stride % 8)) return set_error(-1, "layernorm_modulate: bad frame geometry");
  ProfScope prof(PROF_LN, (hipStream_t)stream, 2.0 * M * d * 2);
  hipLaunchKernelGGL(layernorm_modulate_kernel, dim3(M), dim3(EW_THREADS), 0, (hipStream_t)stream,
                     (const bf16_t*)x, (bf16_t*)out, d, eps, (const bf16_t*)shift, (const bf16_t*)scale,
                     frame_stride, rows_per_frame, row_offset, (const bf16_t*)weight, (const bf16_t*)bias);
  return check_launch("layernorm_modulate");
}

int rtv_rmsnorm(const void* x, int ldx, void* out, int ldo, int M, int d, float eps, const void* weight,
                rtv_stream_t stream) {
  if (M <= 0) return 0;
  if (d % 8 || d > EW_THREADS * 8 * EW_MAXC || ldx % 8 || ldo % 8)
    return set_error(-1, "rmsnorm: d/ld must be multiples of 8, d <= 8192");
  if (!weight) return set_error(-1, "rmsnorm: weight required");
  ProfScope prof(PROF_LN, (hipStream_t)stream, 2.0 * M * d * 2);
  hipLaunchKernelGGL(rmsnorm_kernel, dim3(M), dim3(EW_THREADS), 0, (hipStream_t)stream, (const bf16_t*)x,
                     ldx, (bf16_t*)out, ldo, d, eps, (const bf16_t*)weight);
  return check_launch("rmsnorm");
}

int rtv_pixels_to_rgb8(const void* pixels, void* rgb8, int T, int H, int W, rtv_stream_t stream) {
  if (T <= 0 || H <= 0 || W <= 0) return 0;
  if (!pixels || !rgb8) return set_error(-1, "pixels_to_rgb8: null argument");
  const size_t hw = (size_t)H * W;
  if (hw % 4 || ((uintptr_t)pixels & 15) || ((uintptr_t)rgb8 & 3))
    return set_error(-1, "pixels_to_rgb8: H*W must be a multiple of 4, pixels 16-byte and rgb8 4-byte aligned");
  const size_t total = (size_t)T * (hw / 4);
  int blocks = (int)((total + 255) / 256);
  if (blocks > 8192) blocks = 8192;
  ProfScope prof(PROF_MISC, (hipStream_t)stream, (double)T * hw * 15.0);
  hipLaunchKernelGGL(pixels_to_rgb8_kernel, dim3(blocks), dim3(256), 0, (hipStream_t)stream, (const float*)pixels,
                     (uint8_t*)rgb8, T, hw);
  return check_launch("pixels_to_rgb8");
}

int rtv_qk_norm_rope_cache(const void* qkv, void* q_out, void* k_cache, void* v_cache,
                           int64_t cache_row_stride, int cache_row0, int M, int d, int num_heads, float eps,
                           const void* wq, const void* wk, const void* rope_cs, int F, int gh, int gw,
                           int start_frame, int row_offset, rtv_stream_t stream) {
  return rtv::qk_norm_rope_launch(qkv, q_out, k_cache, v_cache, cache_row_stride, cache_row0, M, d, num_heads, eps, wq, wk,
                                  rope_cs, F, gh, gw, start_frame, row_offset, 0, 0, 0, 0, 0, 0, 3, stream);
}

int rtv_qk_norm_rope_cache_ring(const void* qkv, void* q_out, void* k_cache, void* v_cache,
                                int64_t cache_row_stride, int cache_row0, int M, int d, int num_heads, float eps,
                                const void* wq, const void* wk, const void* rope_cs, int F, int gh, int gw,
                                int start_frame, int row_offset, int ring_lo, int ring_size, int ring_shift,
                                rtv_stream_t stream) {
  return rtv::qk_norm_rope_launch(qkv, q_out, k_cache, v_cache, cache_row_stride, cache_row0, M, d, num_heads, eps, wq, wk,
                                  rope_cs, F, gh, gw, start_frame, row_offset, 0, 0, 0, ring_lo, ring_size, ring_shift, 3, stream);
}

int rtv_modulation_table(const void* modulation, const void* e0, void* emod, int L, int F, int J, int J0,
                         int d, rtv_stream_t stream) {
  if (J0 != J && J0 != 1) return set_error(-1, "modulation_table: J0 must be J or 1");
  size_t total = (size_t)L * F * J * d;
  if (total == 0) return 0;
  int blocks = (int)((total + 255) / 256);
  if (blocks > 4096) blocks = 4096;
  ProfScope prof(PROF_MISC, (hipStream_t)stream, (double)total * 6);
  hipLaunchKernelGGL(modulation_table_kernel, dim3(blocks), dim3(256), 0, (hipStream_t)stream,
                     (const bf16_t*)modulation, (const bf16_t*)e0, (bf16_t*)emod, L, F, J, J0, d);
  return check_launch("modulation_table");
}

int rtv_sinusoidal_embedding(const void* t, void* out, int F, int dim, rtv_stream_t stream) {
  if (dim % 2) return set_error(-1, "sinusoidal_embedding: dim must be even");
  int n = F * (dim / 2);
  if (n <= 0) return 0;
  hipLaunchKernelGGL(sinusoidal_kernel, dim3((n + 127) / 128), dim3(128), 0, (hipStream_t)stream,
                     (const float*)t, (bf16_t*)out, F, dim);
  return check_launch("sinusoidal_embedding");
}

int rtv_patchify(const void* x, void* rows, int C, int F, int gh, int gw, rtv_stream_t stream) {
  size_t total = (size_t)F * gh * gw * C * 4;
  if (total == 0) return 0;
  int blocks = (int)((total + 255) / 256);
  if (blocks > 4096) blocks = 4096;
  hipLaunchKernelGGL(patchify_kernel, dim3(blocks), dim3(256), 0, (hipStream_t)stream, (const bf16_t*)x,
                     (bf16_t*)rows, C, F, gh, gw);
  return check_launch("patchify");
}

int rtv_unpatchify(const void* rows, void* x, int C, int F, int gh, int gw, rtv_stream_t stream) {
  size_t total = (size_t)F * gh * gw * C * 4;
  if (total == 0) return 0;
  int blocks = (int)((total + 255) / 256);
  if (blocks > 4096) blocks = 4096;
  hipLaunchKernelGGL(unpatchify_kernel, dim3(blocks), dim3(256), 0, (hipStream_t)stream,
                     (const bf16_t*)rows, (bf16_t*)x, C, F, gh, gw);
  return check_launch("unpatchify");
}

}
```

### realtime_video_amd/csrc/gemm.hip

```cpp
#include "gemm_core.h"
#include "rtv_internal.h"

namespace rtv {

template <bool F16, int BM, int BN, int BK, int WM, int WN>
__global__ __launch_bounds__(WM* WN * 64) void gemm_kernel(GemmParams p) {
  typedef TileCfg<BM, BN, BK, WM, WN> Cfg;
  static_assert(Cfg::TN == 2 && Cfg::NW * Cfg::TM * 32 * 128 <= 2 * Cfg::STAGE_BYTES, "LDS epilogue geometry");
  extern __shared__ __attribute__((aligned(16))) char smem[];

  const int tid = threadIdx.x;
  const int lane = tid & 63;
  const int wave = __builtin_amdgcn_readfirstlane(tid >> 6);

  const int nwg = p.tiles_m * p.tiles_n;
  int id = xcd_remap(blockIdx.x, nwg);
  constexpr int GROUP_M = 8;
  const int per_group = GROUP_M * p.tiles_n;
  const int group = id / per_group;
  const int first_m = group * GROUP_M;
  const int gm = min(p.tiles_m - first_m, GROUP_M);
  const int in_group = id - group * per_group;
  const int tile_m = first_m + in_group % gm;
  const int tile_n = in_group / gm;
  const int m0 = tile_m * BM, n0 = tile_n * BN;

  const int cpos = lane % Cfg::CH;
  const int rsub = lane / Cfg::CH;
  uint32_t a_off[Cfg::A_INST], b_off[Cfg::B_INST];
#pragma unroll
  for (int i = 0; i < Cfg::A_INST; ++i) {
    int row = (wave * Cfg::A_INST + i) * Cfg::RPI + rsub;
    int gm_row = min(m0 + row, p.M - 1);
    a_off[i] = (uint32_t)gm_row * (uint32_t)p.lda + Cfg::swz(row, cpos) * 8;
  }
#pragma unroll
  for (int i = 0; i < Cfg::B_INST; ++i) {
    int row = (wave * Cfg::B_INST + i) * Cfg::RPI + rsub;
    int gn_row = min(n0 + row, p.N - 1);
    b_off[i] = (uint32_t)gn_row * (uint32_t)p.ldw + Cfg::swz(row, cpos) * 8;
  }

  auto stage = [&](int kt, int buf) {
    char* sA = smem + buf * Cfg::STAGE_BYTES;
    char* sB = sA + Cfg::A_BYTES;
    const uint16_t* Ak = p.A + (size_t)kt * BK;
    const uint16_t* Wk = p.W + (size_t)kt * BK;
#pragma unroll
    for (int i = 0; i < Cfg::A_INST; ++i)
      dma16(Ak + a_off[i], sA + (wave * Cfg::A_INST + i) * 1024);
#pragma unroll
    for (int i = 0; i < Cfg::B_INST; ++i)
      dma16(Wk + b_off[i], sB + (wave * Cfg::B_INST + i) * 1024);
  };

  f32x16 acc[Cfg::TM][Cfg::TN];
#pragma unroll
  for (int mi = 0; mi < Cfg::TM; ++mi)
#pragma unroll
    for (int ni = 0; ni < Cfg::TN; ++ni)
#pragma unroll
      for (int r = 0; r < 16; ++r) acc[mi][ni][r] = 0.f;

  const int wm = wave / WN, wn = wave % WN;
  const int a_row0 = wm * (BM / WM), b_row0 = wn * (BN / WN);

  const int nk = p.K / BK;
  stage(0, 0);
  for (int kt = 0; kt < nk; ++kt) {
    const int buf = kt & 1;
    __syncthreads();
    if (kt + 1 < nk) stage(kt + 1, buf ^ 1);
    const char* sA = smem + buf * Cfg::STAGE_BYTES;
    mma_stage<F16, Cfg, BK>(sA, sA + Cfg::A_BYTES, a_row0, b_row0, lane, acc);
  }

  const bool wide = !((p.ldc | (p.residual ? p.ldr : 0)) & 7) && !(((uintptr_t)p.C | (uintptr_t)p.residual) & 15);
  if (wide) {
    __syncthreads();
    store_tile_lds<F16, Cfg::TM>(p, m0 + a_row0, n0 + b_row0, lane, smem + wave * (Cfg::TM * 32 * 128), acc);
  } else {
    store_tile<F16, Cfg>(p, m0 + a_row0, n0 + b_row0, lane, acc);
  }
}

template <bool F16, int BM, int BN, int BK, int WM, int WN>
static int launch_cfg(GemmParams p, hipStream_t stream) {
  typedef TileCfg<BM, BN, BK, WM, WN> Cfg;
  p.tiles_m = (p.M + BM - 1) / BM;
  p.tiles_n = (p.N + BN - 1) / BN;
  auto kern = gemm_kernel<F16, BM, BN, BK, WM, WN>;
  static LdsAttr lds_attr;
  const int lds = 2 * Cfg::STAGE_BYTES;
  if (int st = ensure_dynamic_lds((const void*)kern, lds, &lds_attr, "gemm")) return st;
  ProfScope prof(F16 ? PROF_CONV : PROF_GEMM, stream, 2.0 * p.M * (double)p.N * p.K);
  note_kernel(BM == 128 && BN == 128 ? DK_GEMM_128x128 : DK_GEMM_OTHER_CFG);
  hipLaunchKernelGGL(kern, dim3(p.tiles_m * p.tiles_n), dim3(Cfg::NT), lds, stream, p);
  return check_launch("gemm");
}

int launch_gemm(const GemmParams& p, int dtype, int tile_cfg, hipStream_t stream) {
  if (p.M <= 0 || p.N <= 0 || p.K <= 0) return set_error(-1, "gemm: empty problem");
  if (p.K % 64 != 0) return set_error(-1, "gemm: K must be a multiple of 64");
  if (p.N % 8 != 0) return set_error(-1, "gemm: N must be a multiple of 8");
  if ((p.lda % 8) || (p.ldw % 8) || (p.ldc % 4) || (p.residual && (p.ldr % 4)))
    return set_error(-1, "gemm: leading dimensions must keep 16-byte (A,W) / 8-byte (C,res) alignment");
  if (p.gate && p.rows_per_frame <= 0) return set_error(-1, "gemm: gate needs rows_per_frame");
  const bool f16 = dtype == RTV_DTYPE_F16;
  if (dtype != RTV_DTYPE_BF16 && dtype != RTV_DTYPE_F16) return set_error(-1, "gemm: dtype");
  if (tile_cfg == 0) {
    const long tiles_n = (p.N + 255) / 256;
    const long rt256 = (p.M + 255) / 256, rt128 = (p.M + 127) / 128;
    const long tiles256 = rt256 * tiles_n, tiles128 = rt128 * tiles_n;
    const long last256 = p.M - (rt256 - 1) * 256;
    const long eff256 = (rt256 - 1) * 256 + (last256 <= 128 ? 128 : 256), pad128 = rt128 * 128;
    const long G = device_num_cus() > 0 ? device_num_cus() : 256;
    const long tail256 = tiles256 % G;
    const bool small_tail = tiles256 > G && tiles256 < 4 * G && tail256 != 0 && tail256 * 4 < G;
    const long rt160 = (p.M + 159) / 160, tiles160 = rt160 * tiles_n, tail160 = tiles160 % G;
    const bool fill160 = tiles160 * 5 >= G * 4 && (tiles160 <= G || tail160 == 0 || tail160 * 4 >= G);
    if (!f16 && p.K >= 1024 && p.M <= 1280 && rt160 * 160 <= eff256 && fill160) return launch_gemm5(p, f16, true, stream);
    if (!f16 && p.K >= 1024 && tiles128 >= 96 && (pad128 * 100 < eff256 * 93 || tiles256 * 8 < G * 5 || small_tail))
      return launch_gemm8m(p, f16, true, stream);
    if (!f16 && ((p.K >= 2048 && tiles256 >= 128) || tiles256 >= 640 || (p.K >= 8192 && tiles256 >= 64)))
      return launch_gemm8(p, f16, true, stream);
    tile_cfg = 1;
  }
  switch (tile_cfg) {
    case 1:
      return f16 ? launch_cfg<true, 128, 128, 64, 2, 2>(p, stream)
                 : launch_cfg<false, 128, 128, 64, 2, 2>(p, stream);
    case 2:
      return f16 ? launch_cfg<true, 256, 128, 64, 4, 2>(p, stream)
                 : launch_cfg<false, 256, 128, 64, 4, 2>(p, stream);
    case 3:
      return f16 ? launch_cfg<true, 256, 256, 64, 2, 4>(p, stream)
                 : launch_cfg<false, 256, 256, 64, 2, 4>(p, stream);
    case 4:
      return launch_gemm8(p, f16, false, stream);
    case 5:
    case 50:
      return launch_gemm8(p, f16, true, stream);
#ifdef RTV_LAB
    case 8:
      return launch_gemm4(p, f16, stream);
    case 81:
    case 82:
    case 83:
    case 84:
    case 85:
    case 86:
    case 87:
    case 89:
    case 90:
    case 91:
      return launch_gemm4(p, f16, stream, tile_cfg - 80);
#endif
    case 9:
      return launch_gemm5(p, f16, true, stream);
    case 19:
      return launch_gemm5(p, f16, false, stream);
    case 6:
      return launch_gemm8m(p, f16, false, stream);
    case 7:
      return launch_gemm8m(p, f16, true, stream);
    default:
      return set_error(-1, "gemm: unknown tile config");
  }
}

}
```

### realtime_video_amd/csrc/gemm8.hip

```cpp
#include <atomic>
#include <mutex>
#include <type_traits>

#include "gemm_core.h"
#include "gemm_split.h"
#include "rtv_internal.h"

#ifndef RTV_G8_MFMA16
#define RTV_G8_MFMA16 1
#endif

namespace rtv {

namespace g8 {
constexpr int BM = 256, BN = 256, BK = 64;
constexpr int HALF_BYTES = 128 * BK * 2;
constexpr int A_OFF = 0;
constexpr int W_OFF = 6 * HALF_BYTES;
constexpr int LDS_BYTES = 10 * HALF_BYTES;
constexpr int THREADS = 512;
__device__ __forceinline__ int swz(int row, int chunk) { return chunk ^ ((row >> 1) & 7); }
}

#ifdef RTV_GEMM_TIMELINE
__device__ unsigned long long* g_timeline = nullptr;
#endif

__device__ __forceinline__ void g8_tile_mn(int tiles_m, int tiles_n, int tile_id, int* mt, int* nt) {
#if RTV_G8_BALANCED_GROUPS
  const int ngrp = (tiles_m + 7) >> 3;
  const int gq = tiles_m / ngrp, gr = tiles_m - gq * ngrp;
  const int big = (gq + 1) * tiles_n;
  int first_m, gm, in_group;
  if (tile_id < gr * big) {
    const int group = tile_id / big;
    gm = gq + 1;
    first_m = group * gm;
    in_group = tile_id - group * big;
  } else {
    const int t = tile_id - gr * big, sm = gq * tiles_n, group = t / sm;
    gm = gq;
    first_m = gr * (gq + 1) + group * gq;
    in_group = t - group * sm;
  }
#else
  constexpr int GROUP_M = 8;
  const int per_group = GROUP_M * tiles_n;
  const int group = tile_id / per_group;
  const int first_m = group * GROUP_M;
  const int gm = min(tiles_m - first_m, GROUP_M);
  const int in_group = tile_id - group * per_group;
#endif
  *mt = first_m + in_group % gm;
  *nt = in_group / gm;
}

template <bool F16>
__device__ __forceinline__ void gemm8m_body(const GemmParams& p, const SplitArgs& sp, int m0, int n0, int tile_id, int seg, int unit,
                                            int kt_begin, int kt_end, bool is_split);

template <bool F16, bool SKIP_IDLE>
__global__ __launch_bounds__(g8::THREADS, 2) void gemm8_kernel(GemmParams p, SplitArgs sp) {
  using namespace g8;
  int bid0 = blockIdx.x;
  if (sp.pair_units) {
    if (bid0 < sp.pair_pad) {
      if (bid0 >= sp.pair_units) return;
#pragma unroll 1
      for (int j = 0; j < 2; ++j) {
        const int tn = 2 * bid0 + j;
        if (tn >= p.tiles_n) break;
        if (j) __syncthreads();
        gemm8m_body<F16>(p, sp, sp.pair_m0, tn * BN, 0, 0, -1, 0, p.K / BK, false);
      }
      return;
    }
    bid0 -= sp.pair_pad;
  }
  if (sp.half_tail) {
    const int nhu = 2 * sp.tail_tiles;
    if (sp.split_first) bid0 = bid0 < nhu ? sp.first_unit + bid0 : bid0 - nhu;
    if (bid0 >= sp.first_unit) {
      const int v = xcd_remap(bid0 - sp.first_unit, nhu);
      const int tile_id = sp.first_unit + (v >> 1);
      int mt, nt;
      g8_tile_mn(p.tiles_m, p.tiles_n, tile_id, &mt, &nt);
      const int m0h = mt * BM + (v & 1) * 128;
      if (m0h >= p.M) return;
      gemm8m_body<F16>(p, sp, m0h, nt * BN, tile_id, 0, -1, 0, p.K / BK, false);
      return;
    }
    sp.S = 1;
// ... 28 lines not shown
      const int row = j * 64 + wave * 8 + rsub;
      const int ch = swz(row, cpos) * 8;
#pragma unroll
      for (int h = 0; h < 2; ++h) {
        const int gm_row = min(m0 + h * 128 + row, p.M - 1);
        const int gn_row = min(n0 + h * 128 + row, p.N - 1);
        src_off[h][j] = ((uint32_t)gm_row * (uint32_t)p.lda + ch) * 2u;
        src_off[2 + h][j] = ((uint32_t)gn_row * (uint32_t)p.ldw + ch) * 2u;
      }
    }
  }
  __amdgpu_buffer_rsrc_t rsrcA = __builtin_amdgcn_make_buffer_rsrc((void*)p.A, 0, 0x7fffffff, 0x00020000);
  __amdgpu_buffer_rsrc_t rsrcW = __builtin_amdgcn_make_buffer_rsrc((void*)p.W, 0, 0x7fffffff, 0x00020000);
  auto stage_piece = [&](int kt, int a3, int h, int j, auto chk) {
    if (decltype(chk)::value && kt >= kt_end) return;
    const int slot = h < 2 ? A_OFF + (a3 * 2 + h) * HALF_BYTES : W_OFF + ((kt & 1) * 2 + (h - 2)) * HALF_BYTES;
    __builtin_amdgcn_raw_ptr_buffer_load_lds(h < 2 ? rsrcA : rsrcW, (RTV_LDS void*)(smem + slot + (j * 64 + wave * 8) * 128), 16,
                                             src_off[h][j], (unsigned)kt * (BK * 2), 0, 0);
  };

  const int b_row0 = (wc & 1) * 64;
#if RTV_G8_MFMA16
  const int l15 = lane & 15, q4 = lane >> 4;
  u32x4 af[4][2];
  u32x4 bfr[4][2];
  auto read_a = [&](int a3, int mq) {
    const char* s = smem + A_OFF + (a3 * 2 + wr) * HALF_BYTES;
#pragma unroll
    for (int mb = 0; mb < 4; ++mb) {
      const int row = mq * 64 + mb * 16 + l15;
#pragma unroll
      for (int ks = 0; ks < 2; ++ks) af[mb][ks] = *(const u32x4*)(s + row * 128 + (swz(row, ks * 4 + q4) << 4));
    }
  };
  auto read_w = [&](int wb) {
    const char* s = smem + W_OFF + (wb * 2 + (wc >> 1)) * HALF_BYTES;
#pragma unroll
    for (int nb = 0; nb < 4; ++nb) {
      const int row = b_row0 + nb * 16 + l15;
#pragma unroll
      for (int ks = 0; ks < 2; ++ks) bfr[nb][ks] = *(const u32x4*)(s + row * 128 + (swz(row, ks * 4 + q4) << 4));
    }
  };

  f32x4 acc[8][4];
#pragma unroll
  for (int mi = 0; mi < 8; ++mi)
#pragma unroll
    for (int ni = 0; ni < 4; ++ni)
#pragma unroll
      for (int r = 0; r < 4; ++r) acc[mi][ni][r] = 0.f;
#else
  u32x4 af[2][4];
  u32x4 bfr[2][4];
  auto read_a = [&](int a3, int mq) {
    const char* s = smem + A_OFF + (a3 * 2 + wr) * HALF_BYTES;
#pragma unroll
    for (int mb = 0; mb < 2; ++mb) {
      const int row = mq * 64 + mb * 32 + l31;
#pragma unroll
      for (int ks = 0; ks < 4; ++ks) af[mb][ks] = *(const u32x4*)(s + row * 128 + (swz(row, ks * 2 + g) << 4));
    }
  };
  auto read_w = [&](int wb) {
    const char* s = smem + W_OFF + (wb * 2 + (wc >> 1)) * HALF_BYTES;
#pragma unroll
    for (int nq = 0; nq < 2; ++nq) {
      const int row = b_row0 + nq * 32 + l31;
#pragma unroll
      for (int ks = 0; ks < 4; ++ks) bfr[nq][ks] = *(const u32x4*)(s + row * 128 + (swz(row, ks * 2 + g) << 4));
    }
  };

  f32x16 acc[4][2];
#pragma unroll
  for (int mi = 0; mi < 4; ++mi)
#pragma unroll
    for (int ni = 0; ni < 2; ++ni)
#pragma unroll
      for (int r = 0; r < 16; ++r) acc[mi][ni][r] = 0.f;
#endif

#define G8_FENCE() __builtin_amdgcn_sched_barrier(0)
#if RTV_G8_MFMA16
#define G8_STORE_LDS(...) store_tile_lds16<F16>(__VA_ARGS__)
#define G8_STORE_DIRECT(CFG, ...) store_tile16<F16>(__VA_ARGS__)
#else
#define G8_STORE_LDS(...) store_tile_lds<F16>(__VA_ARGS__)
#define G8_STORE_DIRECT(CFG, ...) store_tile<F16, CFG>(__VA_ARGS__)
#endif
#define G8_BARRIER()                  \
  do {                                \
    G8_FENCE();                       \
    __builtin_amdgcn_s_barrier();     \
    G8_FENCE();                       \
  } while (0)
#define G8_LDS_DONE()                                   \
  do {                                                  \
    asm volatile("s_waitcnt lgkmcnt(0)" ::: "memory");  \
    G8_FENCE();                                         \
  } while (0)

  const bool idle_rows = SKIP_IDLE && m0 + wr * 128 >= p.M;
  auto mma_half = [&](int mq, int st_kt, int st_a3, int h0, auto chk) {
    __builtin_amdgcn_s_setprio(1);
    int n = 0;
#if RTV_G8_MFMA16
#pragma unroll
    for (int ks = 0; ks < 2; ++ks)
#pragma unroll
      for (int nb = 0; nb < 4; ++nb)
#pragma unroll
        for (int mb = 0; mb < 4; ++mb) {
          acc[mq * 4 + mb][nb] = Mfma16<F16>::run(bfr[nb][ks], af[mb][ks], acc[mq * 4 + mb][nb]);
          ++n;
          if ((n & 7) == 4) {
            G8_FENCE();
            stage_piece(st_kt, st_a3, h0 + (n >> 4), (n >> 3) & 1, chk);
            G8_FENCE();
          }
        }
#else
#pragma unroll
    for (int ks = 0; ks < 4; ++ks)
#pragma unroll
      for (int nq = 0; nq < 2; ++nq)
#pragma unroll
        for (int mb = 0; mb < 2; ++mb) {
          acc[mq * 2 + mb][nq] = Mfma32<F16>::run(bfr[nq][ks], af[mb][ks], acc[mq * 2 + mb][nq]);
          ++n;
          if ((n & 3) == 2) {
            G8_FENCE();
            stage_piece(st_kt, st_a3, h0 + (n >> 3), (n >> 2) & 1, chk);
            G8_FENCE();
          }
        }
#endif
    __builtin_amdgcn_s_setprio(0);
  };

#pragma unroll
  for (int t = 0; t < 2; ++t)
#pragma unroll
    for (int hh = 0; hh < 4; ++hh) {
      const int h = (hh + 2) & 3;
      stage_piece(kt_begin + t, t, h, 0, std::true_type{});
      stage_piece(kt_begin + t, t, h, 1, std::true_type{});
    }
  if (kt_begin + 1 < kt_end) asm volatile("s_waitcnt vmcnt(8)" ::: "memory");
  else asm volatile("s_waitcnt vmcnt(0)" ::: "memory");
  G8_BARRIER();
  if (wr == 1) G8_BARRIER();

  int a3 = 0;
  auto k_tile = [&](const int kt, auto chk) {
    constexpr bool CHK = decltype(chk)::value;
    const int a3n = a3 == 0 ? 2 : a3 - 1;
    read_w(kt & 1);
    read_a(a3, 0);
    G8_LDS_DONE();
    G8_BARRIER();
    mma_half(0, kt + 2, a3n, 0, chk);
    G8_BARRIER();
    read_a(a3, 1);
    if (!CHK || kt + 2 < kt_end) asm volatile("s_waitcnt vmcnt(4)" ::: "memory");
    else asm volatile("s_waitcnt vmcnt(0)" ::: "memory");
    G8_LDS_DONE();
    G8_BARRIER();
    mma_half(1, kt + 2, a3n, 2, chk);
    G8_BARRIER();
    a3 = a3 == 2 ? 0 : a3 + 1;
  };
  auto idle_tile = [&](const int kt) {
    const int a3n = a3 == 0 ? 2 : a3 - 1;
    G8_BARRIER();
#pragma unroll
    for (int i = 0; i < 4; ++i) stage_piece(kt + 2, a3n, i >> 1, i & 1, std::true_type{});
    G8_BARRIER();
    if (kt + 2 < kt_end) asm volatile("s_waitcnt vmcnt(4)" ::: "memory");
    else asm volatile("s_waitcnt vmcnt(0)" ::: "memory");
    G8_BARRIER();
#pragma unroll
    for (int i = 0; i < 4; ++i) stage_piece(kt + 2, a3n, 2 + (i >> 1), i & 1, std::true_type{});
    G8_BARRIER();
    a3 = a3 == 2 ? 0 : a3 + 1;
  };
  int kt = kt_begin;
  if (idle_rows) {
    for (; kt < kt_end; ++kt) idle_tile(kt);
  } else {
    for (; kt + 2 < kt_end; ++kt) k_tile(kt, std::false_type{});
    for (; kt < kt_end; ++kt) k_tile(kt, std::true_type{});
  }
  if (wr == 0) G8_BARRIER();

#ifdef RTV_GEMM_TIMELINE
  tl_t1 = __builtin_amdgcn_s_memrealtime();
  const unsigned long long tl_c1 = __builtin_amdgcn_s_memtime();
  bool reducer = true;
  if (is_split) reducer = split_k_reduce(acc, sp, unit, seg, tile_id, smem, tid, wave, lane);
  if (!reducer) {
    if (g_timeline && tid == 0) {
      unsigned long long* t = g_timeline + (size_t)blockIdx.x * 4;
      t[0] = tl_t0;
      t[1] = tl_t1;
      t[2] = __builtin_amdgcn_s_memrealtime();
      t[3] = ((unsigned long long)(seg + 1) << 32) | (unsigned)tile_id;
    }
    return;
  }
#else
  if (is_split && !split_k_reduce(acc, sp, unit, seg, tile_id, smem, tid, wave, lane)) return;
#endif

  const bool wide = !((p.ldc | (p.residual ? p.ldr : 0)) & 7) && !(((uintptr_t)p.C | (uintptr_t)p.residual) & 15);
  if (wide) {
    if (is_split) __syncthreads();
#ifdef RTV_GEMM_TIMELINE
    unsigned long long tl_mid = 0;
    G8_STORE_LDS(p, m0 + wr * 128, n0 + wc * 64, lane, smem + wave * (128 * 128), acc, &tl_mid);
    if (g_timeline && tid == 0) g_timeline[(size_t)blockIdx.x * 4 + 1] = tl_mid | (1ull << 63);
    tl_t1 = tl_t1 ? tl_t1 : 0;
    if (g_timeline && tid == 0) {
      unsigned long long* t = g_timeline + (size_t)blockIdx.x * 4;
      t[0] = tl_t0;
      t[2] = __builtin_amdgcn_s_memrealtime();
      t[3] = ((unsigned long long)(is_split ? seg + 1 : 0) << 32) | (unsigned)tile_id;
      g_timeline[(size_t)(gridDim.x + blockIdx.x) * 4] = tl_t1;
      g_timeline[(size_t)(gridDim.x + blockIdx.x) * 4 + 1] = tl_c1 - tl_c0;
    }
    return;
#else
    G8_STORE_LDS(p, m0 + wr * 128, n0 + wc * 64, lane, smem + wave * (128 * 128), acc, nullptr);
#endif
  } else {
    G8_STORE_DIRECT(Cfg, p, m0 + wr * 128, n0 + wc * 64, lane, acc);
  }
#ifdef RTV_GEMM_TIMELINE
  if (g_timeline && tid == 0) {
    unsigned long long* t = g_timeline + (size_t)blockIdx.x * 4;
    t[0] = tl_t0;
    t[1] = tl_t1;
    t[2] = __builtin_amdgcn_s_memrealtime();
    t[3] = ((unsigned long long)(is_split ? seg + 1 : 0) << 32) | (unsigned)tile_id | (is_split ? 0x80000000u : 0u);
  }
#endif
}

static std::atomic<bool> g_gemm8_skip_idle{true};
static std::atomic<bool> g_gemm8_half_tail{true};
static std::atomic<bool> g_gemm8_ragged_strips{true};
namespace g8m {
constexpr int BM = 128, BN = 256, BK = 64;
constexpr int HALF_BYTES = 128 * BK * 2;
constexpr int LDS_BYTES = 9 * HALF_BYTES;
}

template <bool F16>
__device__ __forceinline__ void gemm8m_body(const GemmParams& p, const SplitArgs& sp, int m0, int n0, int tile_id, int seg, int unit,
                                            int kt_begin, int kt_end, bool is_split) {
  using namespace g8m;
  extern __shared__ __attribute__((aligned(16))) char smem[];
  const int tid = threadIdx.x;
  const int lane = tid & 63;
  const int wave = __builtin_amdgcn_readfirstlane(tid >> 6);
  const int wr = wave >> 2, wc = wave & 3;
  [[maybe_unused]] const int l31 = lane & 31, g = lane >> 5;

  uint32_t src_off[3][2];
  {
    const int rsub = lane >> 3, cpos = lane & 7;
#pragma unroll
    for (int j = 0; j < 2; ++j) {
      const int row = j * 64 + wave * 8 + rsub;
      const int ch = g8::swz(row, cpos) * 8;
      src_off[0][j] = ((uint32_t)min(m0 + row, p.M - 1) * (uint32_t)p.lda + ch) * 2u;
      src_off[1][j] = ((uint32_t)min(n0 + row, p.N - 1) * (uint32_t)p.ldw + ch) * 2u;
      src_off[2][j] = ((uint32_t)min(n0 + 128 + row, p.N - 1) * (uint32_t)p.ldw + ch) * 2u;
    }
  }
  __amdgpu_buffer_rsrc_t rsrcA = __builtin_amdgcn_make_buffer_rsrc((void*)p.A, 0, 0x7fffffff, 0x00020000);
  __amdgpu_buffer_rsrc_t rsrcW = __builtin_amdgcn_make_buffer_rsrc((void*)p.W, 0, 0x7fffffff, 0x00020000);
  auto stage_piece = [&](int kt, int b3, int h, int j, auto chk) {
    if (decltype(chk)::value && kt >= kt_end) return;
    __builtin_amdgcn_raw_ptr_buffer_load_lds(h == 0 ? rsrcA : rsrcW,
                                             (RTV_LDS void*)(smem + (b3 * 3 + h) * HALF_BYTES + (j * 64 + wave * 8) * 128), 16,
                                             src_off[h][j], (unsigned)kt * (BK * 2), 0, 0);
  };

#if RTV_G8_MFMA16
  const int l15 = lane & 15, q4 = lane >> 4;
  u32x4 af[4][2], bfr[4][2];
  auto read_frags = [&](int b3) {
    const char* sa = smem + (b3 * 3) * HALF_BYTES;
    const char* sw = smem + (b3 * 3 + 1 + (wc >> 1)) * HALF_BYTES;
#pragma unroll
    for (int nb = 0; nb < 4; ++nb) {
      const int row = (wc & 1) * 64 + nb * 16 + l15;
#pragma unroll
      for (int ks = 0; ks < 2; ++ks) bfr[nb][ks] = *(const u32x4*)(sw + row * 128 + (g8::swz(row, ks * 4 + q4) << 4));
    }
#pragma unroll
    for (int mb = 0; mb < 4; ++mb) {
      const int row = wr * 64 + mb * 16 + l15;
#pragma unroll
      for (int ks = 0; ks < 2; ++ks) af[mb][ks] = *(const u32x4*)(sa + row * 128 + (g8::swz(row, ks * 4 + q4) << 4));
    }
  };

  f32x4 acc[4][4];
#pragma unroll
  for (int mi = 0; mi < 4; ++mi)
#pragma unroll
    for (int ni = 0; ni < 4; ++ni)
#pragma unroll
      for (int r = 0; r < 4; ++r) acc[mi][ni][r] = 0.f;
#else
  u32x4 af[2][4], bfr[2][4];
  auto read_frags = [&](int b3) {
    const char* sa = smem + (b3 * 3) * HALF_BYTES;
    const char* sw = smem + (b3 * 3 + 1 + (wc >> 1)) * HALF_BYTES;
#pragma unroll
    for (int nq = 0; nq < 2; ++nq) {
      const int row = (wc & 1) * 64 + nq * 32 + l31;
#pragma unroll
      for (int ks = 0; ks < 4; ++ks) bfr[nq][ks] = *(const u32x4*)(sw + row * 128 + (g8::swz(row, ks * 2 + g) << 4));
    }
#pragma unroll
    for (int mb = 0; mb < 2; ++mb) {
      const int row = wr * 64 + mb * 32 + l31;
#pragma unroll
      for (int ks = 0; ks < 4; ++ks) af[mb][ks] = *(const u32x4*)(sa + row * 128 + (g8::swz(row, ks * 2 + g) << 4));
    }
  };
// ... 18 lines not shown
#pragma unroll
    for (int h = 0; h < 3; ++h) {
      stage_piece(kt_begin + 2, 2, h, 0, std::true_type{});
      stage_piece(kt_begin + 2, 2, h, 1, std::true_type{});
    }
  }
  if (wr == 1) {
    if (kt_begin + 2 < kt_end) asm volatile("s_waitcnt vmcnt(6)" ::: "memory");
    else asm volatile("s_waitcnt vmcnt(0)" ::: "memory");
  } else {
    if (kt_begin + 1 < kt_end) asm volatile("s_waitcnt vmcnt(6)" ::: "memory");
    else asm volatile("s_waitcnt vmcnt(0)" ::: "memory");
  }
  G8_BARRIER();
  if (wr == 1) G8_BARRIER();

  int b3 = 0;
  auto k_tile = [&](const int kt, auto chk) {
    constexpr bool CHK = decltype(chk)::value;
    read_frags(b3);
    G8_LDS_DONE();
    G8_BARRIER();
    const int st_kt = kt + 2 + wr;
    const int st_b = wr ? b3 : (b3 == 0 ? 2 : b3 - 1);
    __builtin_amdgcn_s_setprio(1);
    int n = 0;
#if RTV_G8_MFMA16
#pragma unroll
    for (int ks = 0; ks < 2; ++ks)
#pragma unroll
      for (int nb = 0; nb < 4; ++nb)
#pragma unroll
        for (int mb = 0; mb < 4; ++mb) {
          acc[mb][nb] = Mfma16<F16>::run(bfr[nb][ks], af[mb][ks], acc[mb][nb]);
          ++n;
          if (n == 4 || n == 8 || n == 14 || n == 20 || n == 24 || n == 30) {
            const int pc = n == 4 ? 0 : n == 8 ? 1 : n == 14 ? 2 : n == 20 ? 3 : n == 24 ? 4 : 5;
            G8_FENCE();
            stage_piece(st_kt, st_b, pc >> 1, pc & 1, chk);
            G8_FENCE();
          }
        }
#else
#pragma unroll
    for (int ks = 0; ks < 4; ++ks)
#pragma unroll
      for (int nq = 0; nq < 2; ++nq)
#pragma unroll
        for (int mb = 0; mb < 2; ++mb) {
          acc[mb][nq] = Mfma32<F16>::run(bfr[nq][ks], af[mb][ks], acc[mb][nq]);
          ++n;
          if (n == 2 || n == 4 || n == 7 || n == 10 || n == 12 || n == 15) {
            const int pc = n == 2 ? 0 : n == 4 ? 1 : n == 7 ? 2 : n == 10 ? 3 : n == 12 ? 4 : 5;
            G8_FENCE();
            stage_piece(st_kt, st_b, pc >> 1, pc & 1, chk);
            G8_FENCE();
          }
        }
#endif
    __builtin_amdgcn_s_setprio(0);
    G8_FENCE();
    if (!CHK || st_kt < kt_end) asm volatile("s_waitcnt vmcnt(6)" ::: "memory");
    else asm volatile("s_waitcnt vmcnt(0)" ::: "memory");
    G8_BARRIER();
    b3 = b3 == 2 ? 0 : b3 + 1;
  };
  int kt = kt_begin;
  for (; kt + 3 < kt_end; ++kt) k_tile(kt, std::false_type{});
  for (; kt < kt_end; ++kt) k_tile(kt, std::true_type{});
  if (wr == 0) G8_BARRIER();

  if (is_split && !split_k_reduce(acc, sp, unit, seg, tile_id, smem, tid, wave, lane)) return;

  const bool wide = !((p.ldc | (p.residual ? p.ldr : 0)) & 7) && !(((uintptr_t)p.C | (uintptr_t)p.residual) & 15);
  if (wide) {
    if (is_split) __syncthreads();
    G8_STORE_LDS(p, m0 + wr * 64, n0 + wc * 64, lane, smem + wave * (64 * 128), acc, nullptr);
  } else {
    [[maybe_unused]] typedef TileCfg<128, 256, 64, 2, 4> CfgM;
    G8_STORE_DIRECT(CfgM, p, m0 + wr * 64, n0 + wc * 64, lane, acc);
  }
}

template <bool F16>
__global__ __launch_bounds__(g8::THREADS, 2) void gemm8m_kernel(GemmParams p, SplitArgs sp) {
  using namespace g8m;
  const int nk_total = p.K / BK;
  int tile_id, seg, unit, kt_begin, kt_end;
  const bool is_split = split_unit_of_block(sp, blockIdx.x, nk_total, &tile_id, &unit, &seg, &kt_begin, &kt_end);
  constexpr int GROUP_M = 8;
  const int per_group = GROUP_M * p.tiles_n;
  const int group = tile_id / per_group;
  const int first_m = group * GROUP_M;
  const int gm = min(p.tiles_m - first_m, GROUP_M);
  const int in_group = tile_id - group * per_group;
  gemm8m_body<F16>(p, sp, (first_m + in_group % gm) * BM, (in_group / gm) * BN, tile_id, seg, unit, kt_begin, kt_end, is_split);
}

struct SplitWorkspace {
  int device;
  hipStream_t stream;
  bool any_stream;
  float* slabs;
  int* counters;
};
constexpr int MAX_WORKSPACES = 64;
constexpr int MAX_DEVICES = 64;
static SplitWorkspace g_ws[MAX_WORKSPACES];
static int g_num_ws = 0;
static std::mutex g_ws_mu;

static int attach_workspace(bool any_stream, hipStream_t stream, void* ptr, size_t bytes) {
  int dev = 0;
  if (hipGetDevice(&dev) != hipSuccess) return set_error(-1, "gemm_set_workspace: cannot query the device");
  std::lock_guard<std::mutex> lk(g_ws_mu);
  int slot = -1;
  for (int i = 0; i < g_num_ws; ++i)
    if (g_ws[i].device == dev && g_ws[i].any_stream == any_stream && (any_stream || g_ws[i].stream == stream)) slot = i;
  if (!ptr) {
    if (slot >= 0) g_ws[slot] = g_ws[--g_num_ws];
    return 0;
  }
  if (((uintptr_t)ptr) & 255) return set_error(-1, "gemm_set_workspace: pointer must be 256-byte aligned");
  if (bytes < rtv_gemm_workspace_bytes()) return set_error(-1, "gemm_set_workspace: too small (rtv_gemm_workspace_bytes)");
  if (slot < 0) {
    if (g_num_ws == MAX_WORKSPACES) return set_error(-1, "gemm_set_workspace: too many workspaces attached");
    slot = g_num_ws++;
  }
  SplitWorkspace w{dev, stream, any_stream, (float*)ptr, (int*)((char*)ptr + (size_t)SPLIT_MAX_UNITS * SPLIT_SLAB_FLOATS * 4)};
  if (hipMemset(w.counters, 0, (size_t)SPLIT_MAX_UNITS * sizeof(int)) != hipSuccess) {
    if (slot == g_num_ws - 1) --g_num_ws;
    return set_error(-1, "gemm_set_workspace: cannot zero the arrival counters");
  }
  g_ws[slot] = w;
  return 0;
}

}

using namespace rtv;

#ifdef RTV_GEMM_TIMELINE
extern "C" int rtv_gemm_debug_timeline(unsigned long long* buf) {
  return hipMemcpyToSymbol(HIP_SYMBOL(g_timeline), &buf, sizeof(buf)) == hipSuccess ? 0 : -1;
}
#endif

extern "C" int rtv_gemm_set_half_tail(int on) {
  rtv::g_gemm8_half_tail.store(on != 0, std::memory_order_relaxed);
  return 0;
}

extern "C" int rtv_gemm_set_ragged_strips(int on) {
  rtv::g_gemm8_ragged_strips.store(on != 0, std::memory_order_relaxed);
  return 0;
}

extern "C" int rtv_gemm_set_skip_idle(int on) {
  rtv::g_gemm8_skip_idle.store(on != 0, std::memory_order_relaxed);
  return 0;
}

extern "C" size_t rtv_gemm_workspace_bytes(void) {
  return (size_t)SPLIT_MAX_UNITS * SPLIT_SLAB_FLOATS * 4 + (size_t)SPLIT_MAX_UNITS * 4 + 256;
}

extern "C" int rtv_gemm_set_workspace(void* ptr, size_t bytes) { return attach_workspace(true, nullptr, ptr, bytes); }

extern "C" int rtv_gemm_set_stream_workspace(rtv_stream_t stream, void* ptr, size_t bytes) {
  return attach_workspace(false, (hipStream_t)stream, ptr, bytes);
}

namespace rtv {

int plan_split_k(int T, int nk, bool allow_split, SplitArgs* sp, int* grid, hipStream_t stream, bool allow_half, int extra_units) {
  int dev = 0;
  if (hipGetDevice(&dev) != hipSuccess || dev < 0 || dev >= MAX_DEVICES) return set_error(-1, "gemm: cannot query the device");
  float* slabs = nullptr;
  int* counters = nullptr;
  const int G = device_num_cus();
  if (G <= 0) return set_error(-1, "gemm: cannot query the device");
  {
    std::lock_guard<std::mutex> lk(g_ws_mu);
    for (int i = 0; i < g_num_ws && allow_split; ++i) {
      const SplitWorkspace& w = g_ws[i];
      if (w.device != dev) continue;
      if (!w.any_stream && w.stream == stream) {
        slabs = w.slabs;
        counters = w.counters;
        break;
      }
      if (w.any_stream && !slabs) {
        slabs = w.slabs;
        counters = w.counters;
      }
    }
  }
  *sp = SplitArgs{T, 1, nullptr, nullptr, 0, 0, 0, 0, 0, 0};
  *grid = T;
  const int R = (T + extra_units) % G <= T ? (T + extra_units) % G : 0;
  if (allow_half && g_gemm8_half_tail.load(std::memory_order_relaxed) && R > 0 && T > R && G / R == 2 && nk <= 128) {
    sp->first_unit = T - R;
    sp->tail_tiles = R;
    sp->half_tail = 1;
    *grid = (T - R) + 2 * R;
    return 0;
  }
  if (allow_split && slabs && R > 0) {
    int S = G / R;
    if (S > 8) S = 8;
    if (S > nk / 4) S = nk / 4;
    if (S >= 2 && (size_t)R * S <= (size_t)SPLIT_MAX_UNITS) {
      sp->first_unit = T - R;
      sp->S = S;
      sp->slabs = slabs;
      sp->counters = counters;
      sp->tail_tiles = R;
      sp->split_first = (R * S * 4 <= G) ? 1 : 0;
      *grid = (T - R) + R * S;
    }
  }
  return 0;
}

template <bool F16, bool SKIP_IDLE>
static int launch_gemm8_t(GemmParams p, bool allow_split, hipStream_t stream) {
  p.tiles_m = (p.M + g8::BM - 1) / g8::BM;
  p.tiles_n = (p.N + g8::BN - 1) / g8::BN;
  auto kern = gemm8_kernel<F16, SKIP_IDLE>;
  static LdsAttr lds_attr;
  if (int st = ensure_dynamic_lds((const void*)kern, g8::LDS_BYTES, &lds_attr, "gemm8")) return st;
  SplitArgs sp;
  int grid = 0;
  const int G = device_num_cus();
  const int last_rows = p.M - (p.tiles_m - 1) * g8::BM;
  const int T0 = p.tiles_m * p.tiles_n;
  int pair_units = 0, pair_pad = 0;
  if (allow_split && g_gemm8_ragged_strips.load(std::memory_order_relaxed) && p.tiles_m >= 2 && last_rows <= 128 && G > 0 && T0 > G) {
    const int pu = (p.tiles_n + 1) / 2, pp = (pu + 7) & ~7;
    const int RA = T0 % G;
    if (RA > 0 && RA <= p.tiles_n - pp) {
      pair_units = pu;
      pair_pad = pp;
      p.tiles_m -= 1;
    }
  }
  if (int st = plan_split_k(p.tiles_m * p.tiles_n, p.K / g8::BK, allow_split, &sp, &grid, stream, true, pair_pad))
    return st;
  if (pair_units) {
    sp.pair_units = pair_units;
    sp.pair_pad = pair_pad;
    sp.pair_m0 = p.tiles_m * g8::BM;
    grid += pair_pad;
  }
  ProfScope prof(F16 ? PROF_CONV : PROF_GEMM, stream, 2.0 * p.M * (double)p.N * p.K);
  note_kernel(DK_GEMM8_256x256);
  hipLaunchKernelGGL(kern, dim3(grid), dim3(g8::THREADS), g8::LDS_BYTES, stream, p, sp);
  return check_launch("gemm8");
}

template <bool F16>
static int launch_gemm8m_t(GemmParams p, bool allow_split, hipStream_t stream) {
  p.tiles_m = (p.M + g8m::BM - 1) / g8m::BM;
  p.tiles_n = (p.N + g8m::BN - 1) / g8m::BN;
  auto kern = gemm8m_kernel<F16>;
  static LdsAttr lds_attr;
  if (int st = ensure_dynamic_lds((const void*)kern, g8m::LDS_BYTES, &lds_attr, "gemm8m")) return st;
  SplitArgs sp;
  int grid = 0;
  if (int st = plan_split_k(p.tiles_m * p.tiles_n, p.K / g8m::BK, allow_split, &sp, &grid, stream)) return st;
  ProfScope prof(F16 ? PROF_CONV : PROF_GEMM, stream, 2.0 * p.M * (double)p.N * p.K);
  note_kernel(DK_GEMM8M_128x256);
  hipLaunchKernelGGL(kern, dim3(grid), dim3(g8::THREADS), g8m::LDS_BYTES, stream, p, sp);
  return check_launch("gemm8m");
}

int launch_gemm8m(const GemmParams& p, bool f16, bool split, hipStream_t stream) {
  if ((size_t)p.M * p.lda * 2 > 0x7fffffffull || (size_t)p.N * p.ldw * 2 > 0x7fffffffull)
    return set_error(-1, "gemm8m: operand larger than 2 GiB");
  return f16 ? launch_gemm8m_t<true>(p, split, stream) : launch_gemm8m_t<false>(p, split, stream);
}

int launch_gemm8(const GemmParams& p, bool f16, bool split, hipStream_t stream) {
  if ((size_t)p.M * p.lda * 2 > 0x7fffffffull || (size_t)p.N * p.ldw * 2 > 0x7fffffffull)
    return set_error(-1, "gemm8: operand larger than 2 GiB");
  const int last_rows = p.M - (p.M - 1) / g8::BM * g8::BM;
  if (g_gemm8_skip_idle.load(std::memory_order_relaxed) && !f16 && last_rows <= 128) return launch_gemm8_t<false, true>(p, split, stream);
  return f16 ? launch_gemm8_t<true, false>(p, split, stream) : launch_gemm8_t<false, false>(p, split, stream);
}

}
```

### realtime_video_amd/csrc/rtv_internal.h

```cpp
#pragma once
#include <hip/hip_runtime.h>

#include <atomic>

#include "../../include/rtv_hip.h"
#include "../../include/rtv_hip_cross_fold.h"
#include "../../include/rtv_hip_fp8_rows.h"
#include "../../include/rtv_hip_lab.h"

namespace rtv {

int set_error(int code, const char* msg);
int check_launch(const char* what);

struct LdsAttr {
  std::atomic<uint64_t> done{0};
};
int ensure_dynamic_lds(const void* kernel, int bytes, LdsAttr* state, const char* what);

int device_num_cus();

enum ProfClass { PROF_GEMM = 0, PROF_ATTN, PROF_LN, PROF_ROPE, PROF_CONV, PROF_MISC, PROF_NCLASS };

struct ProfScope {
  ProfScope(int cls, hipStream_t stream, double work);
  ~ProfScope();
  int slot;
  hipStream_t stream;
};

enum DispatchKernel {
  DK_GEMM_128x128 = 0, DK_GEMM_OTHER_CFG, DK_GEMM8_256x256, DK_GEMM8M_128x256, DK_GEMM5_160x256, DK_GEMM_FP8_256x256,
  DK_ATTN_W4, DK_ATTN_FOUR_PHASE, DK_ATTN_LOCKSTEP_256ROW, DK_ATTN_LOCKSTEP_128ROW, DK_ATTN_SPLIT_COMBINE,
  DK_CONV_HALO4P, DK_CONV_HALO4, DK_CONV_HALO, DK_CONV_IGEMM, DK_ATTN_PROBS, DK_COUNT
};
void note_kernel(int id);

struct GemmParams;
int launch_gemm(const GemmParams& p, int dtype, int tile_cfg, hipStream_t stream);
int launch_gemm8(const GemmParams& p, bool f16, bool split_k, hipStream_t stream);
int launch_gemm4(const GemmParams& p, bool f16, hipStream_t stream, int lab = 0);
int launch_gemm8m(const GemmParams& p, bool f16, bool split_k, hipStream_t stream);
int launch_gemm5(const GemmParams& p, bool f16, bool split_k, hipStream_t stream);
int launch_quantize_fp8(const uint16_t* x, int64_t ld, int M, int d, uint8_t* q, int64_t ldq, float* scale_out,
                        unsigned* amax_scratch, hipStream_t stream);
int launch_gemm_fp8(GemmParams p, const uint8_t* A, int lda, const uint8_t* W, int ldw, const float* a_scale, float w_scale,
                    hipStream_t stream);
int launch_gemm_fp8_rows(GemmParams p, const uint8_t* A, int lda, const uint8_t* W, int ldw, const float* a_scales,
                         const float* w_scales, hipStream_t stream);

int qk_norm_rope_check(int64_t cache_row_stride, int cache_row0, int M, int d, int num_heads, int F, int gh, int gw, int start_frame,
                       int row_offset, int group_cols, int64_t q_group_stride, int64_t kv_group_stride, int ring_lo, int ring_size,
                       int ring_shift, int parts);
int qk_norm_rope_launch(const void* qkv, void* q_out, void* k_cache, void* v_cache, int64_t cache_row_stride,
                        int cache_row0, int M, int d, int num_heads, float eps, const void* wq, const void* wk,
                        const void* rope_cs, int F, int gh, int gw, int start_frame, int row_offset, int group_cols,
                        int64_t q_group_stride, int64_t kv_group_stride, int ring_lo, int ring_size, int ring_shift,
                        int parts , rtv_stream_t stream);
int regroup_heads(const void* in, void* out, int rows, int G, int group_cols, rtv_stream_t stream);

int conv3_last_tap(const void* frame, const void* w3, const void* bias, const void* gamma, const void* residual, int res_ld, void* out,
                   int out_ld, int H, int W, int Cin, int Cout, int flags, const void* zeros, hipStream_t stream);

}
```

### realtime_video_amd/csrc/runtime.hip

```cpp
#include <mutex>
#include <string>
#include <vector>

#include "gemm_core.h"
#include "rtv_internal.h"

namespace rtv {

static thread_local std::string g_err;

int set_error(int code, const char* msg) {
  g_err = msg ? msg : "unknown error";
  if (code > 0) {
    g_err += ": ";
    g_err += hipGetErrorString((hipError_t)code);
  }
  return code == 0 ? -1 : code;
}

int ensure_dynamic_lds(const void* kernel, int bytes, LdsAttr* state, const char* what) {
  int dev = 0;
  if (hipGetDevice(&dev) != hipSuccess || dev < 0 || dev >= 64) return set_error(-1, "cannot query the current device");
  const uint64_t bit = 1ull << dev;
  if (state->done.load(std::memory_order_acquire) & bit) return 0;
  hipError_t e = hipFuncSetAttribute(kernel, hipFuncAttributeMaxDynamicSharedMemorySize, bytes);
  if (e != hipSuccess) return set_error((int)e, what);
  state->done.fetch_or(bit, std::memory_order_release);
  return 0;
}

int device_num_cus() {
  static std::atomic<int> cus[64];
  int dev = 0;
  if (hipGetDevice(&dev) != hipSuccess || dev < 0 || dev >= 64) return 0;
  int n = cus[dev].load(std::memory_order_relaxed);
  if (n == 0) {
    hipDeviceProp_t prop;
    if (hipGetDeviceProperties(&prop, dev) != hipSuccess) return 0;
    n = prop.multiProcessorCount;
    cus[dev].store(n, std::memory_order_relaxed);
  }
  return n;
}

static std::atomic<int64_t> g_dispatch[DK_COUNT];
static const char* const g_dispatch_names[DK_COUNT] = {
    "gemm_kernel<128x128>", "gemm_kernel<other tile config>", "gemm8_kernel<256x256 ping-pong>", "gemm8m_kernel<128x256 ping-pong>",
    "gemm5_kernel<160x256 one wave per SIMD>", "gemm_fp8_kernel<256x256>",
    "attn_fwd_w4_kernel<one wave per SIMD>", "attn_fwd_pp_kernel<four-phase>", "attn_fwd_kernel<lockstep, 256 rows>",
    "attn_fwd_kernel<lockstep, 128 rows>", "attn_combine_kernel<kv split>",
    "conv_halo4p_kernel<persistent>", "conv_halo4_kernel", "conv_halo_kernel", "conv_igemm_kernel",
    "attn_probs_kernel<short window, probabilities>"};
void note_kernel(int id) {
  if (id >= 0 && id < DK_COUNT) g_dispatch[id].fetch_add(1, std::memory_order_relaxed);
}

int check_launch(const char* what) {
  hipError_t e = hipGetLastError();
  if (e != hipSuccess) return set_error((int)e, what);
  return 0;
}

struct ProfRec {
  int cls;
  hipEvent_t start, stop;
  double work;
};
static unsigned g_prof_mask = 0;
static int g_prof_stride[PROF_NCLASS] = {1, 1, 1, 1, 1, 1};
static int64_t g_prof_seen[PROF_NCLASS] = {0};
static double g_prof_seen_work[PROF_NCLASS] = {0};
static std::mutex g_prof_mu;
static std::vector<ProfRec> g_prof;
static std::vector<hipEvent_t> g_event_pool;

static hipEvent_t get_event() {
  if (!g_event_pool.empty()) {
    hipEvent_t e = g_event_pool.back();
    g_event_pool.pop_back();
    return e;
  }
  hipEvent_t e;
  hipEventCreate(&e);
  return e;
}

ProfScope::ProfScope(int cls, hipStream_t s, double work) : slot(-1), stream(s) {
  if (!((g_prof_mask >> cls) & 1u)) return;
  std::lock_guard<std::mutex> lk(g_prof_mu);
  g_prof_seen_work[cls] += work;
  if (g_prof_seen[cls]++ % g_prof_stride[cls]) return;
  ProfRec r;
  r.cls = cls;
  r.work = work;
  r.start = get_event();
  r.stop = get_event();
  hipEventRecord(r.start, s);
  g_prof.push_back(r);
  slot = (int)g_prof.size() - 1;
}
ProfScope::~ProfScope() {
  if (slot < 0) return;
  std::lock_guard<std::mutex> lk(g_prof_mu);
  hipEventRecord(g_prof[slot].stop, stream);
}

}

using namespace rtv;

extern "C" {

int rtv_version(void) { return RTV_ABI_VERSION; }

const char* rtv_last_error(void) { return g_err.c_str(); }

int rtv_lab_build(void) {
#ifdef RTV_LAB
  return 1;
#else
  return 0;
#endif
}

int rtv_dispatch_counts(int64_t* counts, int n) {
  for (int i = 0; counts && i < n && i < DK_COUNT; ++i) counts[i] = g_dispatch[i].load(std::memory_order_relaxed);
  return DK_COUNT;
}

const char* rtv_dispatch_name(int id) { return id >= 0 && id < DK_COUNT ? g_dispatch_names[id] : ""; }

int rtv_dispatch_reset(void) {
  for (auto& c : g_dispatch) c.store(0, std::memory_order_relaxed);
  return 0;
}
// ... 17 lines not shown
  return 0;
}

int rtv_prof_set_stride(int cls, int stride) {
  if (cls < 0 || cls >= PROF_NCLASS || stride < 1) return set_error(-1, "prof_set_stride: class 0..5, stride >= 1");
  std::lock_guard<std::mutex> lk(g_prof_mu);
  g_prof_stride[cls] = stride;
  return 0;
}

int rtv_prof_bracket_overhead(int n, rtv_stream_t stream_, double* avg_ms) {
  if (n < 1 || n > 4096 || !avg_ms) return set_error(-1, "prof_bracket_overhead: 1 <= n <= 4096, avg_ms != null");
  hipStream_t stream = (hipStream_t)stream_;
  std::vector<hipEvent_t> ev;
  ev.reserve(2 * (size_t)n);
  auto fail = [&](const char* what) {
    for (auto& e : ev) (void)hipEventDestroy(e);
    return set_error(-1, what);
  };
  for (int i = 0; i < 2 * n; ++i) {
    hipEvent_t e;
    if (hipEventCreate(&e) != hipSuccess) return fail("prof_bracket_overhead: hipEventCreate");
    ev.push_back(e);
  }
  for (int i = 0; i < n; ++i) {
    if (hipEventRecord(ev[2 * i], stream) != hipSuccess || hipEventRecord(ev[2 * i + 1], stream) != hipSuccess)
      return fail("prof_bracket_overhead: hipEventRecord");
  }
  if (hipStreamSynchronize(stream) != hipSuccess) return fail("prof_bracket_overhead: hipStreamSynchronize");
  double tot = 0;
  for (int i = 0; i < n; ++i) {
    float t = 0;
    if (hipEventElapsedTime(&t, ev[2 * i], ev[2 * i + 1]) != hipSuccess) return fail("prof_bracket_overhead: hipEventElapsedTime");
    tot += t;
  }
  for (auto& e : ev) (void)hipEventDestroy(e);
  *avg_ms = tot / n;
  return 0;
}

int rtv_prof_read_seen(int cls, int64_t* launches, double* work) {
  if (cls < 0 || cls >= PROF_NCLASS) return set_error(-1, "prof_read_seen: class 0..5");
  std::lock_guard<std::mutex> lk(g_prof_mu);
  if (launches) *launches = g_prof_seen[cls];
  if (work) *work = g_prof_seen_work[cls];
  return 0;
}

int rtv_prof_read(int cls, double* total_ms, int64_t* launches, double* total_work) {
  std::lock_guard<std::mutex> lk(g_prof_mu);
  double ms = 0, work = 0;
  int64_t n = 0;
  for (auto& r : g_prof) {
    if (r.cls != cls) continue;
    hipError_t e = hipEventSynchronize(r.stop);
    if (e != hipSuccess) return set_error((int)e, "prof_read: hipEventSynchronize");
    float t = 0;
    e = hipEventElapsedTime(&t, r.start, r.stop);
    if (e != hipSuccess) return set_error((int)e, "prof_read: hipEventElapsedTime");
    ms += t;
    work += r.work;
    ++n;
  }
  if (total_ms) *total_ms = ms;
  if (launches) *launches = n;
  if (total_work) *total_work = work;
  return 0;
}

int rtv_gemm(const void* A, int lda, const void* W, int ldw, void* C, int ldc, int M, int N, int K,
             const void* bias, int act, const void* gate, int gate_stride, int rows_per_frame, int row_offset,
             const void* residual, int ldr, int dtype, int tile_cfg, rtv_stream_t stream) {
  if (!A || !W || !C) return set_error(-1, "gemm: null operand");
  if (((uintptr_t)A | (uintptr_t)W) & 15) return set_error(-1, "gemm: A/W must be 16-byte aligned");
  if (((uintptr_t)C | (uintptr_t)bias | (uintptr_t)gate | (uintptr_t)residual) & 7)
    return set_error(-1, "gemm: C/bias/gate/residual must be 8-byte aligned");
  if (gate && (gate_stride % 4)) return set_error(-1, "gemm: gate_stride must be a multiple of 4");
  if (act < 0 || act > 2) return set_error(-1, "gemm: unknown activation");
  const GemmParams p = gemm_params(A, lda, W, ldw, C, ldc, M, N, K, bias, act, gate, gate_stride, rows_per_frame, row_offset, residual,
                                   ldr);
  return launch_gemm(p, dtype, tile_cfg, (hipStream_t)stream);
}

}
```

### realtime_video_amd/ops.py

```python
import ctypes
import math

import torch

from . import _lib

ACT_NONE, ACT_GELU_TANH, ACT_SILU = 0, 1, 2
DT_BF16, DT_F16 = 0, 1
PROF_CLASSES = {"gemm": 0, "attn": 1, "layernorm": 2, "rope": 3, "conv": 4, "misc": 5}


def _ptr(t):
    return ctypes.c_void_p(t.data_ptr()) if t is not None else ctypes.c_void_p(0)


def _stream():
    return ctypes.c_void_p(torch.cuda.current_stream().cuda_stream)


def _dt(t):
    if t.dtype == torch.bfloat16:
        return DT_BF16
    if t.dtype == torch.float16:
        return DT_F16
# ... 45 lines not shown
    sn, swork = ctypes.c_int64(0), ctypes.c_double(0)
    _lib.call("rtv_prof_read_seen", c, ctypes.byref(sn), ctypes.byref(swork))
    scale = swork.value / work.value if work.value > 0 else 1.0
    return {"ms": ms.value, "launches": n.value, "work": work.value, "seen_launches": sn.value, "seen_work": swork.value,
            "ms_class": ms.value * scale}


def attn_set_waves(waves=0):
    _lib.call("rtv_attn_set_waves", int(waves))


def attn_fwd(q, k, v, out=None, scale=None, causal_block=0, q_offset=0):
    _gpu(q, k, v)
    B, Lq, H, D = q.shape
    Lkv = k.shape[1]
    if k.shape != v.shape or k.shape[0] != B or k.shape[2] != H or k.shape[3] != D:
        raise ValueError(f"attention shape mismatch q{tuple(q.shape)} k{tuple(k.shape)} v{tuple(v.shape)}")
    if not (q.dtype == k.dtype == v.dtype):
        raise TypeError("q, k, v must share a dtype")
    for t in (q, k, v):
        if t.stride(3) != 1 or t.stride(2) != D:
            raise ValueError("attention operands need dense [H, D] inner dims (BLHD layout)")
    if out is None:
        out = torch.empty((B, Lq, H, D), dtype=q.dtype, device=q.device)
    if scale is None:
        scale = 1.0 / math.sqrt(D)
    _lib.call("rtv_attn_fwd", _ptr(q), _ptr(k), _ptr(v), _ptr(out), B, Lq, Lkv, H, D,
              q.stride(0), q.stride(1), k.stride(0), k.stride(1), v.stride(0), v.stride(1),
              out.stride(0), out.stride(1), float(scale), int(causal_block), int(q_offset), _dt(q), _stream())
    return out


def attn_fwd_dup(q, k, v, dup_key, dup_count, out=None, scale=None):
    _gpu(q, k, v)
    B, Lq, H, D = q.shape
    Lkv = k.shape[1]
    if k.shape != v.shape or k.shape[0] != B or k.shape[2] != H or k.shape[3] != D:
        raise ValueError(f"attention shape mismatch q{tuple(q.shape)} k{tuple(k.shape)} v{tuple(v.shape)}")
    for t in (q, k, v):
        if t.stride(3) != 1 or t.stride(2) != D:
            raise ValueError("attention operands need dense [H, D] inner dims (BLHD layout)")
    if out is None:
        out = torch.empty((B, Lq, H, D), dtype=q.dtype, device=q.device)
    if scale is None:
        scale = 1.0 / math.sqrt(D)
    _lib.call("rtv_attn_fwd_dup", _ptr(q), _ptr(k), _ptr(v), _ptr(out), B, Lq, Lkv, H, D,
              q.stride(0), q.stride(1), k.stride(0), k.stride(1), v.stride(0), v.stride(1),
              out.stride(0), out.stride(1), float(scale), int(dup_key), int(dup_count), _dt(q), _stream())
    return out


def cross_fold_dims(num_heads, text_rows):
    kh, kf = ctypes.c_int(0), ctypes.c_int(0)
    ok = _lib.load().rtv_cross_fold_dims(int(num_heads), int(text_rows), ctypes.byref(kh), ctypes.byref(kf))
    return bool(ok), kh.value, kf.value


def attn_probs_dup(q, k, dup_key, dup_count, kh, p_cols, out=None, scale=None):
    _gpu(q, k)
    Lq, H, D = q.shape
    Lkv = k.shape[0]
    if q.dtype != torch.bfloat16 or k.dtype != torch.bfloat16:
        raise TypeError("attn_probs_dup is bf16 only")
    for t in (q, k):
        if t.stride(2) != 1 or t.stride(1) != D:
            raise ValueError("attention operands need dense [H, D] inner dims")
    if out is None:
        out = torch.empty((Lq, p_cols), dtype=q.dtype, device=q.device)
    if scale is None:
        scale = 1.0 / math.sqrt(D)
    _lib.call("rtv_attn_probs_dup", _ptr(q), _ptr(k), _ptr(out), Lq, Lkv, H, D, q.stride(0), k.stride(0), out.stride(0),
              int(kh), int(p_cols), float(scale), int(dup_key), int(dup_count), _stream())
    return out


def cross_fold_weight(co_w, v, rows, kh, k_fold, out=None):
    _gpu(co_w, v)
    d = co_w.shape[0]
    if out is None:
        out = torch.empty((d, k_fold), dtype=torch.bfloat16, device=co_w.device)
    _lib.call("rtv_cross_fold_weight", _ptr(co_w), co_w.stride(0), _ptr(v), v.stride(0), _ptr(out), out.stride(0), d // 128,
              int(rows), int(kh), int(k_fold), _stream())
    return out


def attn_fwd_win(q, k_cache, v_cache, seg0, seg1=(0, 0), out=None, scale=None):
    _gpu(q, k_cache, v_cache)
    B, Lq, H, D = q.shape
    (r0, n0), (r1, n1) = seg0, seg1
    rows = k_cache.shape[1]
    if min(r0, n0, r1, n1) < 0 or r0 + n0 > rows or (n1 and r1 + n1 > rows):
        raise ValueError("attn_fwd_win: segment outside the cache")
    for t in (q, k_cache, v_cache):
        if t.stride(3) != 1 or t.stride(2) != D:
            raise ValueError("attention operands need dense [H, D] inner dims (BLHD layout)")
    if out is None:
        out = torch.empty((B, Lq, H, D), dtype=q.dtype, device=q.device)
    if scale is None:
        scale = 1.0 / math.sqrt(D)
    k, v = k_cache[:, r0:], v_cache[:, r0:]
    _lib.call("rtv_attn_fwd_win", _ptr(q), _ptr(k), _ptr(v), _ptr(out), B, Lq, n0, n1,
              (r1 - r0) if n1 else 0, H, D, q.stride(0), q.stride(1), k.stride(0), k.stride(1), v.stride(0), v.stride(1),
              out.stride(0), out.stride(1), float(scale), 0, 0, _dt(q), _stream())
    return out


def attn_fwd_split(q, k_cache, v_cache, seg0, seg1=(0, 0), kv_splits=2, out=None, scale=None, workspace=None, causal_block=0,
                   q_offset=0):
    _gpu(q, k_cache, v_cache)
    B, Lq, H, D = q.shape
    (r0, n0), (r1, n1) = seg0, seg1
    rows = k_cache.shape[1]
    if min(r0, n0, r1, n1) < 0 or r0 + n0 > rows or (n1 and r1 + n1 > rows):
        raise ValueError("attn_fwd_split: segment outside the cache")
    for t in (q, k_cache, v_cache):
        if t.stride(3) != 1 or t.stride(2) != D:
            raise ValueError("attention operands need dense [H, D] inner dims (BLHD layout)")
    if out is None:
        out = torch.empty((B, Lq, H, D), dtype=q.dtype, device=q.device)
    if scale is None:
        scale = 1.0 / math.sqrt(D)
    if workspace is None:
        need = _lib.load().rtv_attn_split_workspace_bytes(B, Lq, H, int(kv_splits))
        workspace = torch.empty(max(need, 16) // 4, dtype=torch.float32, device=q.device)
    k, v = k_cache[:, r0:], v_cache[:, r0:]
    _lib.call("rtv_attn_fwd_split", _ptr(q), _ptr(k), _ptr(v), _ptr(out), B, Lq, n0, n1,
              (r1 - r0) if n1 else 0, H, D, q.stride(0), q.stride(1), k.stride(0), k.stride(1), v.stride(0), v.stride(1),
              out.stride(0), out.stride(1), float(scale), int(causal_block), int(q_offset), int(kv_splits), _ptr(workspace),
              workspace.numel() * workspace.element_size(), _dt(q), _stream())
    return out


def attn_fp8_shadow(cache_rows, H, device):
    return (torch.zeros((cache_rows, H, 128), dtype=torch.uint8, device=device),
            torch.zeros(((cache_rows + 63) // 64, H, 128, 64), dtype=torch.uint8, device=device))


def _check_shadow(k8, v8t, what):
    _gpu(k8, v8t)
    if k8.dtype != torch.uint8 or v8t.dtype != torch.uint8 or k8.dim() != 3 or v8t.dim() != 4 or not (k8.is_contiguous() and v8t.is_contiguous()):
        raise ValueError(f"{what}: k8 / v8t must be dense uint8 tensors [rows, H, 128] / [tiles, H, 128, 64]")
    rows, H, D = k8.shape
    if D != 128 or tuple(v8t.shape) != ((rows + 63) // 64, H, 128, 64):
        raise ValueError(f"{what}: v8t must be [ceil(rows / 64), H, 128, 64] for k8 [rows, H, 128]")
    return rows, H


def attn_quantize_kv(k_cache, v_cache, k8, v8t, row0=0, rows=None, k_scale=1.0, v_scale=1.0, amax=None):
    _gpu(k_cache, v_cache, amax)
    cache_rows, H = _check_shadow(k8, v8t, "attn_quantize_kv")
    for t in (k_cache, v_cache):
        if t.dtype != torch.bfloat16 or t.dim() != 3 or tuple(t.shape) != (cache_rows, H, 128) or t.stride(2) != 1 or t.stride(1) != 128:
            raise ValueError("attn_quantize_kv: caches must be bf16 [rows, H, 128] with dense [H, 128] inner dims, rows as in k8")
    if k_cache.stride(0) != v_cache.stride(0):
        raise ValueError("attn_quantize_kv: K and V need the same row stride")
    if amax is not None and (amax.dtype != torch.float32 or amax.numel() != 2 or not amax.is_contiguous()):
        raise ValueError("attn_quantize_kv: amax must be a dense float32 tensor of 2 elements")
    if rows is None:
        rows = cache_rows - row0
    _lib.call("rtv_attn_quantize_kv", _ptr(k_cache), _ptr(v_cache), k_cache.stride(0), int(row0), int(rows), H, _ptr(k8), _ptr(v8t),
              cache_rows, float(k_scale), float(v_scale), _ptr(amax), _stream())
    return k8, v8t


def attn_fwd_fp8(q, k8, v8t, seg0, seg1=(0, 0), out=None, scale=None, k_scale=1.0, v_scale=1.0, causal_block=0, q_offset=0):
    _gpu(q, out)
# ... 496 lines not shown
```

Baseline: 18.87.

## Fold cross-attention q RMSNorm into the q GEMM epilogue and probs kernel

The cross-attention query path no longer runs a separate RMSNorm kernel. The q projection GEMM now writes per-row sum-of-squares partials in its epilogue. The short-window probs kernel reads the raw q, multiplies in the norm weight from LDS, and applies the rsqrt scale to the softmax logit scale. This removes one full read/write pass over q and one kernel launch per layer, at the cost of a heavier GEMM epilogue and extra register and LDS pressure in the probs kernel. It is enabled by default through an env toggle and only takes effect when the cross-V fold is active.

```diff
diff --git a/include/rtv_hip_cross_fold.h b/include/rtv_hip_cross_fold.h
--- a/include/rtv_hip_cross_fold.h
+++ b/include/rtv_hip_cross_fold.h
@@ -15,6 +15,15 @@
 int rtv_cross_fold_weight(const void* co_w, int64_t ldw, const void* v, int64_t ldv, void* vo, int64_t ldvo,
                           int num_heads, int rows, int kh, int k_fold, rtv_stream_t stream);
 
+int rtv_gemm_rowsq(const void* A, int lda, const void* W, int ldw, void* C, int ldc, int M, int N, int K, const void* bias,
+                   void* partials, int ldp, int tile_cfg, rtv_stream_t stream);
+int rtv_row_sumsq_partials(const void* x, int64_t ldx, void* partials, int ldp, int M, int d, rtv_stream_t stream);
+int rtv_attn_probs_dup_rawq(const void* q, const void* q_norm_w, const void* q_sumsq, int sumsq_ld, float eps, const void* k,
+                            void* p, int Lq, int Lkv, int H, int D, int64_t q_row_stride, int64_t k_row_stride,
+                            int64_t p_row_stride, int kh, int p_cols, float scale, int dup_key, int dup_count,
+                            rtv_stream_t stream);
+int rtv_dit_set_cross_q_fold(int on);
+
 #ifdef __cplusplus
 }
 #endif
diff --git a/realtime_video_amd/causal_model.py b/realtime_video_amd/causal_model.py
--- a/realtime_video_amd/causal_model.py
+++ b/realtime_video_amd/causal_model.py
@@ -98,6 +98,7 @@
         self._ws = {}
         self.fold_text_padding = True
         self.fold_cross_v = os.environ.get("RTV_FOLD_CROSS_V", "1") != "0"
+        self.cross_q_fold = os.environ.get("RTV_CROSS_Q_FOLD", "1") != "0"
         self.use_hip_graphs = False
         self._graphs = {}
         self._weights_version = 0
@@ -604,6 +605,9 @@
                 fold_k = kf_.value
             if fold_k and not need_cross and any(c.get("vo_for") != (text_rows, self.lora_version) for c in crossattn_cache):
                 fold_k = 0
+        q_fold = bool(fold_k) and getattr(self, "cross_q_fold", True)
+        if fold_k and hasattr(_lib.load(), "rtv_dit_set_cross_q_fold"):
+            _lib.load().rtv_dit_set_cross_q_fold(int(q_fold))
         if fold_k:
             for c in crossattn_cache:
                 if "vo" not in c:
@@ -659,7 +663,7 @@
         if not use_cp:
             graph_key = None
             if self.use_hip_graphs and not need_cross:
-                graph_key = (F, gh, gw, row0, lo, hi, start_frame, causal_block, ring_lo, ring_size, ring_shift, kv_only, text_rows, fold_k,
+                graph_key = (F, gh, gw, row0, lo, hi, start_frame, causal_block, ring_lo, ring_size, ring_shift, kv_only, text_rows, fold_k, q_fold,
                              int(self.gemm_tile_cfg), rs, self._weights_version,
                              kv_cache[0]["k"].data_ptr(), kv_cache[-1]["v"].data_ptr(), crossattn_cache[0]["k"].data_ptr(), fp8_key)
                 ent = self._graphs.get(graph_key)
@@ -694,7 +698,7 @@
             graph_key = None
             if self.use_hip_graphs and not need_cross and not getattr(cp, "_gloo", False):
                 graph_key = ("cp", id(cp), bool(getattr(cp, "overlap", True)), cp.world, cp.head_exchange(self.num_heads), F, gh, gw, row0, lo, hi, start_frame, causal_block, kv_only,
-                             text_rows, fold_k, int(self.gemm_tile_cfg), rs, self._weights_version, splits,
+                             text_rows, fold_k, q_fold, int(self.gemm_tile_cfg), rs, self._weights_version, splits,
                              kv_cache[0]["k"].data_ptr(), kv_cache[-1]["v"].data_ptr(), crossattn_cache[0]["k"].data_ptr())
                 ent = self._graphs.get(graph_key)
                 if isinstance(ent, dict):
diff --git a/realtime_video_amd/csrc/attn_fwd.hip b/realtime_video_amd/csrc/attn_fwd.hip
--- a/realtime_video_amd/csrc/attn_fwd.hip
+++ b/realtime_video_amd/csrc/attn_fwd.hip
@@ -616,12 +616,17 @@
   int dup_key;
   float dup_log2;
   int tiles_per_wg;
+  const uint16_t* qw;
+  const float* qsq;
+  int qsq_ld, qsq_n;
+  float d_norm, eps;
 };
 constexpr int PROBS_NW = 4;
 constexpr int PROBS_ROWS = PROBS_NW * ATT_QW;
-
-template <int NKB>
-__global__ __launch_bounds__(PROBS_NW * 64) void attn_probs_kernel(ProbsParams p) {
+constexpr int PROBS_MAX_PARTIALS = 32;
+
+template <int NKB, bool RAWQ = false>
+__global__ __launch_bounds__(PROBS_NW * 64, RAWQ ? (NKB <= 3 ? 4 : 3) : 1) void attn_probs_kernel(ProbsParams p) {
   constexpr int KEYS = NKB * 32;
   constexpr int SLAB_LD = KEYS * 2 + 16;
   extern __shared__ __attribute__((aligned(16))) char smem[];
@@ -636,6 +641,9 @@
   const uint16_t* kb = p.k + (size_t)h * ATT_D;
   uint16_t* pb = p.p + (size_t)h * p.kh;
 
+  if constexpr (RAWQ) {
+    if (tid < 16) *(u32x4*)(smem + KEYS * 256 + PROBS_NW * ATT_QW * SLAB_LD + tid * 16) = *(const u32x4*)(p.qw + (size_t)h * ATT_D + tid * 8);
+  }
   for (int id = tid; id < KEYS * 16; id += PROBS_NW * 64) {
     const int r = id >> 4, c = id & 15;
     u32x4 v = {0u, 0u, 0u, 0u};
@@ -647,7 +655,8 @@
 #pragma unroll
   for (int dc = 0; dc < 8; ++dc) k_rd[dc] = sK + l31 * 256 + (((dc * 2 + g) ^ (l31 & 15)) << 4);
 
-  const float c = p.scale_log2e;
+  [[maybe_unused]] const char* const sW = smem + KEYS * 256 + PROBS_NW * ATT_QW * SLAB_LD;
+  float c = p.scale_log2e;
   const int ppr = p.kh >> 3;
   const int tail0 = p.H * p.kh, tail_pieces = h == p.H - 1 ? (p.p_cols - tail0) >> 3 : 0;
   const int tile0 = blockIdx.x * p.tiles_per_wg;
@@ -655,12 +664,36 @@
     const int row0 = (tile0 + ti) * PROBS_ROWS + wave * ATT_QW;
     if (row0 >= p.Lq) break;
     const int q_row_c = min(row0 + l31, p.Lq - 1);
+    [[maybe_unused]] float pv[PROBS_MAX_PARTIALS / 2];
+    if constexpr (RAWQ) {
+      const float4* sq = (const float4*)(p.qsq + (size_t)q_row_c * p.qsq_ld);
+      const int n4 = (p.qsq_n + 3) >> 2;
+#pragma unroll
+      for (int j = 0; j < PROBS_MAX_PARTIALS / 8; ++j) {
+        const int t0 = 4 * (g * (PROBS_MAX_PARTIALS / 8) + j);
+        const float4 v = sq[min(t0 >> 2, n4 - 1)];
+        pv[4 * j + 0] = t0 + 0 < p.qsq_n ? v.x : 0.f;
+        pv[4 * j + 1] = t0 + 1 < p.qsq_n ? v.y : 0.f;
+        pv[4 * j + 2] = t0 + 2 < p.qsq_n ? v.z : 0.f;
+        pv[4 * j + 3] = t0 + 3 < p.qsq_n ? v.w : 0.f;
+      }
+    }
     u32x4 qf[8];
     {
       const uint16_t* qp = qb + (size_t)q_row_c * p.q_rs + g * 8;
 #pragma unroll
       for (int dc = 0; dc < 8; ++dc) qf[dc] = *(const u32x4*)(qp + dc * 16);
     }
+    if constexpr (RAWQ) {
+#pragma unroll
+      for (int dc = 0; dc < 8; ++dc) {
+        const u32x4 wf = *(const u32x4*)(sW + (dc * 2 + g) * 16);
+#pragma unroll
+        for (int i = 0; i < 4; ++i)
+          qf[dc][i] = pack2<false>(__uint_as_float(qf[dc][i] << 16) * __uint_as_float(wf[i] << 16),
+                                   __uint_as_float(qf[dc][i] & 0xffff0000u) * __uint_as_float(wf[i] & 0xffff0000u));
+      }
+    }
     f32x16 s[NKB];
 #pragma unroll
     for (int kbk = 0; kbk < NKB; ++kbk)
@@ -673,6 +706,17 @@
         const u32x4 kf = *(const u32x4*)(k_rd[dc] + kbk * 32 * 256);
         s[kbk] = mfma32<false>(kf, qf[dc], s[kbk]);
       }
+    if constexpr (RAWQ) {
+      float lo = 0.f;
+#pragma unroll
+      for (int t = 0; t < PROBS_MAX_PARTIALS / 2; ++t) lo += pv[t];
+      float ss = __shfl_xor(lo, 32, 64);
+#pragma unroll
+      for (int t = 0; t < PROBS_MAX_PARTIALS / 2; ++t) ss += pv[t];
+      const float up = __shfl_xor(ss, 32, 64);
+      ss = g ? ss : up;
+      c = p.scale_log2e * rsqrtf(ss / p.d_norm + p.eps);
+    }
     float mx = -INFINITY;
 #pragma unroll
     for (int kbk = 0; kbk < NKB; ++kbk)
@@ -796,18 +840,22 @@
                        dup_count > 1 ? dup_key : -1, dup_count);
 }
 
+template <int NKB, bool RAWQ>
+static int launch_attn_probs_t(const ProbsParams& p, dim3 grid, hipStream_t stream) {
+  static LdsAttr lds_attr;
+  const int lds = NKB * 32 * 256 + PROBS_NW * ATT_QW * (NKB * 64 + 16) + (RAWQ ? 256 : 0);
+  if (int st = ensure_dynamic_lds((const void*)attn_probs_kernel<NKB, RAWQ>, lds, &lds_attr, "attn_probs")) return st;
+  hipLaunchKernelGGL((attn_probs_kernel<NKB, RAWQ>), grid, dim3(PROBS_NW * 64), lds, stream, p);
+  return check_launch("attn_probs");
+}
 template <int NKB>
 static int launch_attn_probs(const ProbsParams& p, dim3 grid, hipStream_t stream) {
-  static LdsAttr lds_attr;
-  const int lds = NKB * 32 * 256 + PROBS_NW * ATT_QW * (NKB * 64 + 16);
-  if (int st = ensure_dynamic_lds((const void*)attn_probs_kernel<NKB>, lds, &lds_attr, "attn_probs")) return st;
-  hipLaunchKernelGGL((attn_probs_kernel<NKB>), grid, dim3(PROBS_NW * 64), lds, stream, p);
-  return check_launch("attn_probs");
-}
-
-extern "C" int rtv_attn_probs_dup(const void* q, const void* k, void* p, int Lq, int Lkv, int H, int D, int64_t q_row_stride,
-                                  int64_t k_row_stride, int64_t p_row_stride, int kh, int p_cols, float scale, int dup_key,
-                                  int dup_count, rtv_stream_t stream) {
+  return p.qw ? launch_attn_probs_t<NKB, true>(p, grid, stream) : launch_attn_probs_t<NKB, false>(p, grid, stream);
+}
+
+static int attn_probs_impl(const void* q, const void* k, void* p, int Lq, int Lkv, int H, int D, int64_t q_row_stride,
+                           int64_t k_row_stride, int64_t p_row_stride, int kh, int p_cols, float scale, int dup_key,
+                           int dup_count, const void* q_w, const void* q_sumsq, int sumsq_ld, float eps, rtv_stream_t stream) {
   if (D != ATT_D) return set_error(-1, "attn_probs: head_dim must be 128");
   if (H <= 0 || Lq <= 0) return 0;
   if (Lkv <= 0 || Lkv > 128) return set_error(-1, "attn_probs: the key window must hold 1..128 keys");
@@ -833,6 +881,14 @@
   pp.scale_log2e = scale * 1.4426950408889634f;
   pp.dup_key = dup_count > 1 ? dup_key : -1;
   pp.dup_log2 = dup_count > 1 ? log2f((float)dup_count) : 0.f;
+  pp.qw = (const uint16_t*)q_w;
+  pp.qsq = (const float*)q_sumsq;
+  pp.qsq_ld = sumsq_ld;
+  pp.qsq_n = (H * ATT_D + 255) / 256;
+  pp.d_norm = (float)(H * ATT_D);
+  pp.eps = eps;
+  if (q_w && (!q_sumsq || sumsq_ld < pp.qsq_n || (sumsq_ld & 3) || pp.qsq_n > PROBS_MAX_PARTIALS || (((uintptr_t)q_w | (uintptr_t)q_sumsq) & 15)))
+    return set_error(-1, "attn_probs_rawq: needs the norm weight, H <= 64 and partials with sumsq_ld >= ceil(H * 128 / 256), sumsq_ld % 4 == 0, both 16-byte aligned");
   const int cus = device_num_cus() > 0 ? device_num_cus() : 256;
   const int n_tiles = (Lq + PROBS_ROWS - 1) / PROBS_ROWS;
   int tpw = (int)(((int64_t)n_tiles * H) / (2 * (int64_t)cus));
@@ -840,7 +896,7 @@
   pp.tiles_per_wg = tpw;
   const dim3 grid((n_tiles + tpw - 1) / tpw, H);
   ProfScope prof(PROF_ATTN, (hipStream_t)stream, 2.0 * H * (double)Lq * Lkv * ATT_D);
-  note_kernel(DK_ATTN_PROBS);
+  note_kernel(q_w ? DK_ATTN_PROBS_RAWQ : DK_ATTN_PROBS);
   const int nkb = (kh + 31) / 32;
   switch (nkb) {
     case 1: return launch_attn_probs<1>(pp, grid, (hipStream_t)stream);
@@ -848,6 +904,22 @@
     case 3: return launch_attn_probs<3>(pp, grid, (hipStream_t)stream);
     default: return launch_attn_probs<4>(pp, grid, (hipStream_t)stream);
   }
+}
+
+extern "C" int rtv_attn_probs_dup(const void* q, const void* k, void* p, int Lq, int Lkv, int H, int D, int64_t q_row_stride,
+                                  int64_t k_row_stride, int64_t p_row_stride, int kh, int p_cols, float scale, int dup_key,
+                                  int dup_count, rtv_stream_t stream) {
+  return attn_probs_impl(q, k, p, Lq, Lkv, H, D, q_row_stride, k_row_stride, p_row_stride, kh, p_cols, scale, dup_key, dup_count, nullptr,
+                         nullptr, 0, 0.f, stream);
+}
+
+extern "C" int rtv_attn_probs_dup_rawq(const void* q, const void* q_norm_w, const void* q_sumsq, int sumsq_ld, float eps, const void* k,
+                                       void* p, int Lq, int Lkv, int H, int D, int64_t q_row_stride, int64_t k_row_stride,
+                                       int64_t p_row_stride, int kh, int p_cols, float scale, int dup_key, int dup_count,
+                                       rtv_stream_t stream) {
+  if (!q_norm_w) return set_error(-1, "attn_probs_rawq: the norm weight is required");
+  return attn_probs_impl(q, k, p, Lq, Lkv, H, D, q_row_stride, k_row_stride, p_row_stride, kh, p_cols, scale, dup_key, dup_count, q_norm_w,
+                         q_sumsq, sumsq_ld, eps, stream);
 }
 
 extern "C" size_t rtv_attn_split_workspace_bytes(int B, int Lq, int H, int kv_splits) {
diff --git a/realtime_video_amd/csrc/dit_forward.hip b/realtime_video_amd/csrc/dit_forward.hip
--- a/realtime_video_amd/csrc/dit_forward.hip
+++ b/realtime_video_amd/csrc/dit_forward.hip
@@ -80,6 +80,7 @@
   float* fscale;
   float* attn_part;
   size_t attn_part_bytes;
+  float* qsq;
 };
 
 static size_t carve(const rtv_dit_config* c, int F, int gh, int gw, char* base, size_t cap, DitBuffers* b,
@@ -116,6 +117,7 @@
   }
   t.attn_part_bytes = c->max_attn_kv_splits > 1 ? M * (size_t)c->num_heads * (128 + 2) * sizeof(float) : 0;
   t.attn_part = (float*)ws.take(t.attn_part_bytes);
+  t.qsq = (float*)ws.take(M * (((d + 255) / 256 + 3) & ~(size_t)3) * sizeof(float));
   if (b) *b = t;
   if (ok) *ok = ws.ok;
   return ws.off;
@@ -199,6 +201,12 @@
   return check_launch("silu");
 }
 
+static std::atomic<bool> g_cross_q_fold{true};
+extern "C" int rtv_dit_set_cross_q_fold(int on) {
+  g_cross_q_fold.store(on != 0, std::memory_order_relaxed);
+  return 0;
+}
+
 extern "C" int rtv_cross_fold_dims(int num_heads, int text_rows, int* kh, int* k_fold) {
   const int khv = text_rows >= 0 ? (text_rows + 1 + 7) & ~7 : 0;
   const int64_t kf = ((int64_t)num_heads * khv + 63) & ~(int64_t)63;
@@ -502,11 +510,21 @@
   RTV_TRY(linear(c, S_LAYER0 + S_PER_LAYER * l + S_O, b.ao, d, lw.o_w, lw.o_b, b.x, rc, d, 0, em + 2 * d, 6 * d, fs, r0, b.x, tc, stream));
   const void* ln_out = nullptr;
   RTV_TRY(ln_input(c, nullptr, nullptr, 0, lw.norm3_w, lw.norm3_b, &ln_out));
-  RTV_TRY(linear(c, S_LAYER0 + S_PER_LAYER * l + S_CQ, ln_out, d, lw.cq_w, lw.cq_b, b.qkv, rc, d, 0, nullptr, 0, 0, 0, nullptr, tc, stream));
-  RTV_TRY(rtv_rmsnorm(b.qkv, d, b.q, d, rc, d, eps, lw.cnorm_q_w, stream));
+  const bool q_fold = c.fold_k && g_cross_q_fold.load(std::memory_order_relaxed);
+  const int ldp = ((d + 255) / 256 + 3) & ~3;
+  if (q_fold) {
+    RTV_TRY(rtv_gemm_rowsq(ln_out, d, lw.cq_w, d, b.qkv, d, rc, d, d, lw.cq_b, b.qsq, ldp, tc, stream));
+  } else {
+    RTV_TRY(linear(c, S_LAYER0 + S_PER_LAYER * l + S_CQ, ln_out, d, lw.cq_w, lw.cq_b, b.qkv, rc, d, 0, nullptr, 0, 0, 0, nullptr, tc, stream));
+    RTV_TRY(rtv_rmsnorm(b.qkv, d, b.q, d, rc, d, eps, lw.cnorm_q_w, stream));
+  }
   if (c.fold_k) {
-    RTV_TRY(rtv_attn_probs_dup(b.q, st->ca_k[l], b.ao, rc, st->text_rows + 1, H, hd, d, d, c.fold_k, c.fold_kh, c.fold_k, scale,
-                               st->text_rows, c.cfg->text_len - st->text_rows, stream));
+    if (q_fold)
+      RTV_TRY(rtv_attn_probs_dup_rawq(b.qkv, lw.cnorm_q_w, b.qsq, ldp, eps, st->ca_k[l], b.ao, rc, st->text_rows + 1, H, hd, d, d, c.fold_k,
+                                      c.fold_kh, c.fold_k, scale, st->text_rows, c.cfg->text_len - st->text_rows, stream));
+    else
+      RTV_TRY(rtv_attn_probs_dup(b.q, st->ca_k[l], b.ao, rc, st->text_rows + 1, H, hd, d, d, c.fold_k, c.fold_kh, c.fold_k, scale,
+                                 st->text_rows, c.cfg->text_len - st->text_rows, stream));
     RTV_TRY(rtv_gemm(b.ao, c.fold_k, st->ca_v[c.L + l], st->ca_vo_ld, b.x, d, rc, d, c.fold_k, lw.co_b, 0, nullptr, 0, 0, 0, b.x, d,
                      RTV_DTYPE_BF16, tc, stream));
   } else {
diff --git a/realtime_video_amd/csrc/elementwise.hip b/realtime_video_amd/csrc/elementwise.hip
--- a/realtime_video_amd/csrc/elementwise.hip
+++ b/realtime_video_amd/csrc/elementwise.hip
@@ -1,3 +1,4 @@
+#include "gemm_rowsq.h"
 #include "ln_row.h"
 #include "rtv_common.h"
 #include "rtv_internal.h"
@@ -49,6 +50,36 @@
       *(u32x4*)(orow + c * 8) = pack_bf16x8(o);
     }
   }
+}
+
+__global__ __launch_bounds__(EW_THREADS) void row_sumsq_kernel(const bf16_t* __restrict__ x, int64_t ldx, float* __restrict__ partials,
+                                                               int ldp, int d) {
+  const int row = blockIdx.x, half = threadIdx.x >> 5, l = threadIdx.x & 31;
+  const bf16_t* xr = x + (size_t)row * ldx;
+  const int ntiles = (d + ROWSQ_TILE - 1) / ROWSQ_TILE;
+  for (int t = half; t < ntiles; t += EW_THREADS / 32) {
+    const int col = t * ROWSQ_TILE + l * 8;
+    u32x4 v = {0u, 0u, 0u, 0u};
+    if (col < d) v = *(const u32x4*)(xr + col);
+    float s = rowsq_group8(v);
+    s += __shfl_xor(s, 1, 64);
+    s += __shfl_xor(s, 2, 64);
+    s += __shfl_xor(s, 4, 64);
+    s += __shfl_xor(s, 8, 64);
+    s += __shfl_xor(s, 16, 64);
+    if (l == 0) partials[(size_t)row * ldp + t] = s;
+  }
+}
+
+int launch_row_sumsq(const void* x, int64_t ldx, float* partials, int ldp, int M, int d, hipStream_t stream) {
+  if (M <= 0) return 0;
+  if (!x || !partials) return set_error(-1, "row_sumsq: null argument");
+  if (d <= 0 || (d & 7) || (ldx & 7) || ldx < d || ((uintptr_t)x & 15) || ((uintptr_t)partials & 3) || ldp < (d + ROWSQ_TILE - 1) / ROWSQ_TILE)
+    return set_error(-1, "row_sumsq: d and ldx must be multiples of 8 (16-byte rows), ldp >= ceil(d / 256)");
+  ProfScope prof(PROF_LN, stream, 1.0 * M * d * 2);
+  note_kernel(DK_ROW_SUMSQ);
+  hipLaunchKernelGGL(row_sumsq_kernel, dim3(M), dim3(EW_THREADS), 0, stream, (const bf16_t*)x, ldx, partials, ldp, d);
+  return check_launch("row_sumsq");
 }
 
 __device__ __forceinline__ void launder(u32x4& v) {
@@ -531,6 +562,10 @@
   return check_launch("rmsnorm");
 }
 
+int rtv_row_sumsq_partials(const void* x, int64_t ldx, void* partials, int ldp, int M, int d, rtv_stream_t stream) {
+  return launch_row_sumsq(x, ldx, (float*)partials, ldp, M, d, (hipStream_t)stream);
+}
+
 int rtv_pixels_to_rgb8(const void* pixels, void* rgb8, int T, int H, int W, rtv_stream_t stream) {
   if (T <= 0 || H <= 0 || W <= 0) return 0;
   if (!pixels || !rgb8) return set_error(-1, "pixels_to_rgb8: null argument");
diff --git a/realtime_video_amd/csrc/gemm.hip b/realtime_video_amd/csrc/gemm.hip
--- a/realtime_video_amd/csrc/gemm.hip
+++ b/realtime_video_amd/csrc/gemm.hip
@@ -99,7 +99,7 @@
   return check_launch("gemm");
 }
 
-int launch_gemm(const GemmParams& p, int dtype, int tile_cfg, hipStream_t stream) {
+static int launch_gemm_pick(const GemmParams& p, int dtype, int tile_cfg, hipStream_t stream, float* rowsq, int ldp, bool* fused) {
   if (p.M <= 0 || p.N <= 0 || p.K <= 0) return set_error(-1, "gemm: empty problem");
   if (p.K % 64 != 0) return set_error(-1, "gemm: K must be a multiple of 64");
   if (p.N % 8 != 0) return set_error(-1, "gemm: N must be a multiple of 8");
@@ -108,6 +108,13 @@
   if (p.gate && p.rows_per_frame <= 0) return set_error(-1, "gemm: gate needs rows_per_frame");
   const bool f16 = dtype == RTV_DTYPE_F16;
   if (dtype != RTV_DTYPE_BF16 && dtype != RTV_DTYPE_F16) return set_error(-1, "gemm: dtype");
+  auto gemm8 = [&](bool split) {
+    if (rowsq && gemm8_rowsq_applies(p, f16, ldp)) {
+      *fused = true;
+      return launch_gemm8_rowsq(p, split, rowsq, ldp, stream);
+    }
+    return launch_gemm8(p, f16, split, stream);
+  };
   if (tile_cfg == 0) {
     const long tiles_n = (p.N + 255) / 256;
     const long rt256 = (p.M + 255) / 256, rt128 = (p.M + 127) / 128;
@@ -123,7 +130,7 @@
     if (!f16 && p.K >= 1024 && tiles128 >= 96 && (pad128 * 100 < eff256 * 93 || tiles256 * 8 < G * 5 || small_tail))
       return launch_gemm8m(p, f16, true, stream);
     if (!f16 && ((p.K >= 2048 && tiles256 >= 128) || tiles256 >= 640 || (p.K >= 8192 && tiles256 >= 64)))
-      return launch_gemm8(p, f16, true, stream);
+      return gemm8(true);
     tile_cfg = 1;
   }
   switch (tile_cfg) {
@@ -137,10 +144,10 @@
       return f16 ? launch_cfg<true, 256, 256, 64, 2, 4>(p, stream)
                  : launch_cfg<false, 256, 256, 64, 2, 4>(p, stream);
     case 4:
-      return launch_gemm8(p, f16, false, stream);
+      return gemm8(false);
     case 5:
     case 50:
-      return launch_gemm8(p, f16, true, stream);
+      return gemm8(true);
 #ifdef RTV_LAB
     case 8:
       return launch_gemm4(p, f16, stream);
@@ -169,4 +176,14 @@
   }
 }
 
+int launch_row_sumsq(const void* x, int64_t ldx, float* partials, int ldp, int M, int d, hipStream_t stream);
+
+int launch_gemm(const GemmParams& p, int dtype, int tile_cfg, hipStream_t stream, float* rowsq, int ldp) {
+  bool fused = false;
+  if (rowsq && (dtype != RTV_DTYPE_BF16 || ldp < (p.N + 255) / 256)) return set_error(-1, "gemm: row partials need bf16 and ldp >= ceil(N / 256)");
+  if (int st = launch_gemm_pick(p, dtype, tile_cfg, stream, rowsq, ldp, &fused)) return st;
+  if (!rowsq || fused) return 0;
+  return launch_row_sumsq(p.C, p.ldc, rowsq, ldp, p.M, p.N, stream);
 }
+
+}
diff --git a/realtime_video_amd/csrc/gemm8.hip b/realtime_video_amd/csrc/gemm8.hip
--- a/realtime_video_amd/csrc/gemm8.hip
+++ b/realtime_video_amd/csrc/gemm8.hip
@@ -8,6 +8,9 @@
 
 #ifndef RTV_G8_MFMA16
 #define RTV_G8_MFMA16 1
+#endif
+#ifndef RTV_G8_ROWSQ
+#define RTV_G8_ROWSQ 0
 #endif
 
 namespace rtv {
@@ -202,7 +205,10 @@
 #endif
 
 #define G8_FENCE() __builtin_amdgcn_sched_barrier(0)
-#if RTV_G8_MFMA16
+#if RTV_G8_ROWSQ
+#define G8_STORE_LDS(...) store_tile_lds16_rowsq<F16>(__VA_ARGS__)
+#define G8_STORE_DIRECT(CFG, ...) ((void)0)
+#elif RTV_G8_MFMA16
 #define G8_STORE_LDS(...) store_tile_lds16<F16>(__VA_ARGS__)
 #define G8_STORE_DIRECT(CFG, ...) store_tile16<F16>(__VA_ARGS__)
 #else
@@ -367,9 +373,13 @@
 #endif
 }
 
-static std::atomic<bool> g_gemm8_skip_idle{true};
-static std::atomic<bool> g_gemm8_half_tail{true};
-static std::atomic<bool> g_gemm8_ragged_strips{true};
+#if RTV_G8_ROWSQ
+extern std::atomic<bool> g_gemm8_skip_idle, g_gemm8_half_tail, g_gemm8_ragged_strips;
+#else
+std::atomic<bool> g_gemm8_skip_idle{true};
+std::atomic<bool> g_gemm8_half_tail{true};
+std::atomic<bool> g_gemm8_ragged_strips{true};
+#endif
 namespace g8m {
 constexpr int BM = 128, BN = 256, BK = 64;
 constexpr int HALF_BYTES = 128 * BK * 2;
@@ -554,6 +564,7 @@
   }
 }
 
+#if !RTV_G8_ROWSQ
 template <bool F16>
 __global__ __launch_bounds__(g8::THREADS, 2) void gemm8m_kernel(GemmParams p, SplitArgs sp) {
   using namespace g8m;
@@ -694,6 +705,7 @@
   }
   return 0;
 }
+#endif
 
 template <bool F16, bool SKIP_IDLE>
 static int launch_gemm8_t(GemmParams p, bool allow_split, hipStream_t stream) {
@@ -726,11 +738,12 @@
     grid += pair_pad;
   }
   ProfScope prof(F16 ? PROF_CONV : PROF_GEMM, stream, 2.0 * p.M * (double)p.N * p.K);
-  note_kernel(DK_GEMM8_256x256);
+  note_kernel(RTV_G8_ROWSQ ? DK_GEMM8_ROWSQ_256x256 : DK_GEMM8_256x256);
   hipLaunchKernelGGL(kern, dim3(grid), dim3(g8::THREADS), g8::LDS_BYTES, stream, p, sp);
   return check_launch("gemm8");
 }
 
+#if !RTV_G8_ROWSQ
 template <bool F16>
 static int launch_gemm8m_t(GemmParams p, bool allow_split, hipStream_t stream) {
   p.tiles_m = (p.M + g8m::BM - 1) / g8m::BM;
@@ -760,5 +773,6 @@
   if (g_gemm8_skip_idle.load(std::memory_order_relaxed) && !f16 && last_rows <= 128) return launch_gemm8_t<false, true>(p, split, stream);
   return f16 ? launch_gemm8_t<true, false>(p, split, stream) : launch_gemm8_t<false, false>(p, split, stream);
 }
-
-}
+#endif
+
+}
diff --git a/realtime_video_amd/csrc/gemm8_rowsq.hip b/realtime_video_amd/csrc/gemm8_rowsq.hip
--- /dev/null
+++ b/realtime_video_amd/csrc/gemm8_rowsq.hip
@@ -0,0 +1,30 @@
+#include "gemm_rowsq.h"
+
+#undef RTV_G8_MFMA16
+#define RTV_G8_MFMA16 1
+#undef RTV_GEMM_TIMELINE
+#define RTV_G8_ROWSQ 1
+#define gemm8_kernel gemm8_rowsq_kernel
+#define gemm8m_body gemm8m_rowsq_body
+#include "gemm8.hip"
+
+namespace rtv {
+
+bool gemm8_rowsq_applies(const GemmParams& p, bool f16, int ldp) {
+  return !f16 && p.act == 0 && !p.gate && !p.residual && p.N % ROWSQ_TILE == 0 && ldp >= p.N / ROWSQ_TILE && !(p.ldc & 7) &&
+         !((uintptr_t)p.C & 15);
+}
+
+int launch_gemm8_rowsq(const GemmParams& p0, bool split, float* partials, int ldp, hipStream_t stream) {
+  if (!partials || !gemm8_rowsq_applies(p0, false, ldp)) return set_error(-1, "gemm8_rowsq: needs a plain bf16 launch with 16-byte output rows, N % 256 == 0");
+  if ((size_t)p0.M * p0.lda * 2 > 0x7fffffffull || (size_t)p0.N * p0.ldw * 2 > 0x7fffffffull)
+    return set_error(-1, "gemm8: operand larger than 2 GiB");
+  GemmParams p = p0;
+  p.gate = (const uint16_t*)partials;
+  p.gate_stride = ldp;
+  const int last_rows = p.M - (p.M - 1) / g8::BM * g8::BM;
+  if (g_gemm8_skip_idle.load(std::memory_order_relaxed) && last_rows <= 128) return launch_gemm8_t<false, true>(p, split, stream);
+  return launch_gemm8_t<false, false>(p, split, stream);
+}
+
+}
diff --git a/realtime_video_amd/csrc/gemm_rowsq.h b/realtime_video_amd/csrc/gemm_rowsq.h
--- /dev/null
+++ b/realtime_video_amd/csrc/gemm_rowsq.h
@@ -0,0 +1,80 @@
+#pragma once
+#include "gemm_core.h"
+
+namespace rtv {
+
+constexpr int ROWSQ_TILE = 256;
+
+__device__ __forceinline__ float rowsq_group8(const u32x4& t) {
+  float s = 0.f;
+#pragma unroll
+  for (int i = 0; i < 4; ++i) {
+    const float lo = __uint_as_float(t[i] << 16), hi = __uint_as_float(t[i] & 0xffff0000u);
+    s += lo * lo;
+    s += hi * hi;
+  }
+  return s;
+}
+
+template <int CTRL>
+__device__ __forceinline__ float lane_swap(float v) {
+  return __builtin_bit_cast(float, __builtin_amdgcn_update_dpp(0, __builtin_bit_cast(int, v), CTRL, 0xf, 0xf, true));
+}
+
+constexpr int ROWSQ_LDS_OFF = 8 * 128 * 128;
+
+template <bool F16, int TMB>
+__device__ __forceinline__ void store_tile_lds16_rowsq(const GemmParams& p, int m_base, int n_base, int lane, char* img,
+                                                       f32x4 (&acc)[TMB][4], unsigned long long*) {
+  static_assert(!F16, "row sum-of-squares partials are defined on bf16 outputs");
+  typedef Mfma32<F16> T;
+  constexpr int ROWS = TMB * 16;
+  const int l15 = lane & 15, q = lane >> 4;
+  u32x2 bq[4];
+#pragma unroll
+  for (int nb = 0; nb < 4; ++nb) {
+    const int ncol = min(n_base + nb * 16 + q * 4, p.N - 4);
+    bq[nb] = p.bias ? *(const u32x2*)(p.bias + ncol) : u32x2{0u, 0u};
+  }
+#pragma unroll
+  for (int mb = 0; mb < TMB; ++mb) {
+    const int row = mb * 16 + l15;
+#pragma unroll
+    for (int nb = 0; nb < 4; ++nb) {
+      u32x2 o;
+      o[0] = T::pack2(acc[mb][nb][0] + T::lo_f32(bq[nb][0]), acc[mb][nb][1] + T::hi_f32(bq[nb][0]));
+      o[1] = T::pack2(acc[mb][nb][2] + T::lo_f32(bq[nb][1]), acc[mb][nb][3] + T::hi_f32(bq[nb][1]));
+      *(u32x2*)(img + row * 128 + (((nb * 4 + q) ^ l15) << 3)) = o;
+    }
+  }
+  asm volatile("s_waitcnt lgkmcnt(0)" ::: "memory");
+  __builtin_amdgcn_sched_barrier(0);
+  const int wave = __builtin_amdgcn_readfirstlane(threadIdx.x >> 6);
+  const int wr = wave >> 2, wc = wave & 3;
+  float* const sums = (float*)(img - wave * (ROWS * 128) + ROWSQ_LDS_OFF);
+  const int rsub = lane >> 3, c = lane & 7;
+  const int n = n_base + c * 8;
+#pragma unroll
+  for (int ps = 0; ps < TMB * 2; ++ps) {
+    const int row = ps * 8 + rsub;
+    const int m = m_base + row;
+    u32x4 t = *(const u32x4*)(img + row * 128 + ((c ^ ((row >> 1) & 7)) << 4));
+    if (row & 1) t = u32x4{t[2], t[3], t[0], t[1]};
+    if (m < p.M) *(u32x4*)(p.C + (size_t)m * p.ldc + n) = t;
+    float s = rowsq_group8(t);
+    s += lane_swap<0xB1>(s);
+    s += lane_swap<0x4E>(s);
+    s += lane_swap<0x141>(s);
+    if (c == 0) sums[wave * ROWS + row] = s;
+  }
+  __syncthreads();
+  const int r = threadIdx.x;
+  if (r < 2 * ROWS) {
+    const float* b = sums + (r / ROWS) * 4 * ROWS + (r % ROWS);
+    const float v = (b[0] + b[ROWS]) + (b[2 * ROWS] + b[3 * ROWS]);
+    const int m = m_base - wr * ROWS + r;
+    if (m < p.M) ((float*)p.gate)[(size_t)m * p.gate_stride + (n_base - wc * 64) / ROWSQ_TILE] = v;
+  }
+}
+
+}
diff --git a/realtime_video_amd/csrc/rtv_internal.h b/realtime_video_amd/csrc/rtv_internal.h
--- a/realtime_video_amd/csrc/rtv_internal.h
+++ b/realtime_video_amd/csrc/rtv_internal.h
@@ -32,12 +32,15 @@
 enum DispatchKernel {
   DK_GEMM_128x128 = 0, DK_GEMM_OTHER_CFG, DK_GEMM8_256x256, DK_GEMM8M_128x256, DK_GEMM5_160x256, DK_GEMM_FP8_256x256,
   DK_ATTN_W4, DK_ATTN_FOUR_PHASE, DK_ATTN_LOCKSTEP_256ROW, DK_ATTN_LOCKSTEP_128ROW, DK_ATTN_SPLIT_COMBINE,
-  DK_CONV_HALO4P, DK_CONV_HALO4, DK_CONV_HALO, DK_CONV_IGEMM, DK_ATTN_PROBS, DK_COUNT
+  DK_CONV_HALO4P, DK_CONV_HALO4, DK_CONV_HALO, DK_CONV_IGEMM, DK_ATTN_PROBS, DK_GEMM8_ROWSQ_256x256, DK_ATTN_PROBS_RAWQ, DK_ROW_SUMSQ,
+  DK_COUNT
 };
 void note_kernel(int id);
 
 struct GemmParams;
-int launch_gemm(const GemmParams& p, int dtype, int tile_cfg, hipStream_t stream);
+int launch_gemm(const GemmParams& p, int dtype, int tile_cfg, hipStream_t stream, float* rowsq = nullptr, int ldp = 0);
+bool gemm8_rowsq_applies(const GemmParams& p, bool f16, int ldp);
+int launch_gemm8_rowsq(const GemmParams& p, bool split_k, float* partials, int ldp, hipStream_t stream);
 int launch_gemm8(const GemmParams& p, bool f16, bool split_k, hipStream_t stream);
 int launch_gemm4(const GemmParams& p, bool f16, hipStream_t stream, int lab = 0);
 int launch_gemm8m(const GemmParams& p, bool f16, bool split_k, hipStream_t stream);
diff --git a/realtime_video_amd/csrc/runtime.hip b/realtime_video_amd/csrc/runtime.hip
--- a/realtime_video_amd/csrc/runtime.hip
+++ b/realtime_video_amd/csrc/runtime.hip
@@ -50,7 +50,8 @@
     "attn_fwd_w4_kernel<one wave per SIMD>", "attn_fwd_pp_kernel<four-phase>", "attn_fwd_kernel<lockstep, 256 rows>",
     "attn_fwd_kernel<lockstep, 128 rows>", "attn_combine_kernel<kv split>",
     "conv_halo4p_kernel<persistent>", "conv_halo4_kernel", "conv_halo_kernel", "conv_igemm_kernel",
-    "attn_probs_kernel<short window, probabilities>"};
+    "attn_probs_kernel<short window, probabilities>", "gemm8_rowsq_kernel<256x256 ping-pong + row sum-of-squares>",
+    "attn_probs_kernel<short window, raw q + norm folded>", "row_sumsq_kernel<partials of stored rows>"};
 void note_kernel(int id) {
   if (id >= 0 && id < DK_COUNT) g_dispatch[id].fetch_add(1, std::memory_order_relaxed);
 }
@@ -234,4 +235,13 @@
   return launch_gemm(p, dtype, tile_cfg, (hipStream_t)stream);
 }
 
-}
+int rtv_gemm_rowsq(const void* A, int lda, const void* W, int ldw, void* C, int ldc, int M, int N, int K, const void* bias,
+                   void* partials, int ldp, int tile_cfg, rtv_stream_t stream) {
+  if (!A || !W || !C || !partials) return set_error(-1, "gemm_rowsq: null operand");
+  if (((uintptr_t)A | (uintptr_t)W | (uintptr_t)C) & 15) return set_error(-1, "gemm_rowsq: A/W/C must be 16-byte aligned");
+  if (((uintptr_t)bias & 7) || ((uintptr_t)partials & 3) || (ldc & 7)) return set_error(-1, "gemm_rowsq: bias 8-byte, partials 4-byte aligned, ldc % 8 == 0");
+  const GemmParams p = gemm_params(A, lda, W, ldw, C, ldc, M, N, K, bias, 0, nullptr, 0, 0, 0, nullptr, 0);
+  return launch_gemm(p, RTV_DTYPE_BF16, tile_cfg, (hipStream_t)stream, (float*)partials, ldp);
+}
+
+}
diff --git a/realtime_video_amd/ops.py b/realtime_video_amd/ops.py
--- a/realtime_video_amd/ops.py
+++ b/realtime_video_amd/ops.py
@@ -151,6 +151,58 @@
     _lib.call("rtv_cross_fold_weight", _ptr(co_w), co_w.stride(0), _ptr(v), v.stride(0), _ptr(out), out.stride(0), d // 128,
               int(rows), int(kh), int(k_fold), _stream())
     return out
+
+
+def _partials_buffer(M, d, device):
+    nt = (d + 255) // 256
+    return torch.empty((M, (nt + 3) // 4 * 4), dtype=torch.float32, device=device)[:, :nt]
+
+
+def gemm_rowsq(a, w, bias=None, tile_cfg=0, out=None, partials=None):
+    _gpu(a, w)
+    M, K = a.shape
+    N = w.shape[0]
+    if out is None:
+        out = torch.empty((M, N), dtype=torch.bfloat16, device=a.device)
+    if partials is None:
+        partials = _partials_buffer(M, N, a.device)
+    if tile_cfg in (0, 5, 7, 50):
+        ensure_gemm_workspace(a.device)
+    _lib.call("rtv_gemm_rowsq", _ptr(a), a.stride(0), _ptr(w), w.stride(0), _ptr(out), out.stride(0), M, N, K,
+              _ptr(bias), _ptr(partials), partials.stride(0), int(tile_cfg), _stream())
+    return out, partials
+
+
+def row_sumsq_partials(x, out=None):
+    _gpu(x)
+    M, d = x.shape
+    if out is None:
+        out = _partials_buffer(M, d, x.device)
+    _lib.call("rtv_row_sumsq_partials", _ptr(x), x.stride(0), _ptr(out), out.stride(0), M, d, _stream())
+    return out
+
+
+def attn_probs_dup_rawq(q, norm_w, sumsq, eps, k, dup_key, dup_count, kh, p_cols, out=None, scale=None):
+    _gpu(q, k, norm_w, sumsq)
+    Lq, H, D = q.shape
+    Lkv = k.shape[0]
+    if q.dtype != torch.bfloat16 or k.dtype != torch.bfloat16 or norm_w.dtype != torch.bfloat16 or sumsq.dtype != torch.float32:
+        raise TypeError("attn_probs_dup_rawq takes bf16 q / k / weight and fp32 partials")
+    for t in (q, k):
+        if t.stride(2) != 1 or t.stride(1) != D:
+            raise ValueError("attention operands need dense [H, D] inner dims")
+    if out is None:
+        out = torch.empty((Lq, p_cols), dtype=q.dtype, device=q.device)
+    if scale is None:
+        scale = 1.0 / math.sqrt(D)
+    _lib.call("rtv_attn_probs_dup_rawq", _ptr(q), _ptr(norm_w), _ptr(sumsq), sumsq.stride(0), float(eps), _ptr(k), _ptr(out), Lq, Lkv,
+              H, D, q.stride(0), k.stride(0), out.stride(0), int(kh), int(p_cols), float(scale), int(dup_key), int(dup_count),
+              _stream())
+    return out
+
+
+def dit_set_cross_q_fold(on=True):
+    _lib.call("rtv_dit_set_cross_q_fold", int(bool(on)))
 
 
 def attn_fwd_win(q, k_cache, v_cache, seg0, seg1=(0, 0), out=None, scale=None):
```

Result: no change. 18.95, median of 6 (+0.4%).
